# ucmmesa/Lidar-Visual-Odometry

Measured on NVIDIA B200. Metric: scan-to-map scans/sec (HDL-64 synthetic), higher is better.
Workload: dtype f32+f64

## Files before the change

lidar-visual-odometry_b200/csrc/lvo_api.cu:

```cuda
#include "lvo_internal.h"
#include "lvo_prims.cuh"
#include "lvo_extract.cuh"
#include "lvo_voxel.cuh"
#include "lvo_knn.cuh"
#include "lvo_solver.cuh"
#include "lvo_odometry.cuh"
#include "lvo_mapping.cuh"
#include "lvo_depth.cuh"
#include "lvo_outputs.cuh"

#include <algorithm>
#include <cmath>
#include <cstring>
#include <new>
#include <type_traits>
#include <nvtx3/nvToolsExt.h>

#define LVO_PROBE_GATE_EXTRACT 1
#define LVO_PROBE_GATE_ODO 2
#define LVO_PROBE_GATE_MAP 4

struct lvo_ctx {
  lvo_config cfg;
  int lanes, P, cap_sharp, cap_lsharp, cap_flat;
  cudaStream_t st = nullptr;
  cudaStream_t own_st = nullptr;
  std::string err;
  std::vector<void*> allocs, pinned;
  LaneState* d_ls = nullptr;
  LaneState* h_ls = nullptr;
  ExtractArgs ex;
  OdoArgs odo;
  MapArgs map;
  SolveArgs solve;
  GridSet gknn;
  GridProblem* d_knn_prob = nullptr;
  int* d_knn_n = nullptr;
  unsigned char* d_raw = nullptr;
  const lvo_cloud_view* pending_next = nullptr;
  unsigned char* d_raw2 = nullptr;
  cudaStream_t copy_st = nullptr;
  cudaEvent_t copy_ev = nullptr, compute_ev = nullptr;
  std::vector<lvo_cloud_view> prefetched;
  std::vector<const unsigned char*> next_in_ptr;
  int opt_stage_timing = 1;
  int raw_cur = 0;
  size_t raw_lane_bytes = 0;
  const unsigned char** d_in_ptr = nullptr; const unsigned char** h_in_ptr = nullptr;
  int* d_in_n = nullptr; int* h_in_n = nullptr;
  float4* d_upload = nullptr;
  int* d_knn_ind = nullptr; float* d_knn_sq = nullptr;
  double* d_trace[2] = {nullptr, nullptr};
  long long launches = 0;
  std::vector<long long> lane_frame;
  std::vector<lvo_lane_config> lane_cfg;
  LaneConfig* d_lcfg = nullptr; LaneConfig* h_lcfg = nullptr;
  std::vector<char> lane_active;
  std::vector<char> lane_map_update;
  std::vector<char> prefetched_active;
  std::vector<int> lane_status;
  std::vector<char> probe_gate;
  bool odo_grids_stale = false;
  cudaEvent_t ev[8];
  LvoStageTimer stage_tm;
  lvo_timings tim;
  bool pending = false, pending_do_map = false, pending_graph = false;
  struct Span { const unsigned char* host; size_t bytes; size_t dev_off; };
  std::vector<Span> spans;
  std::vector<int> span_order;
  cudaGraphExec_t graph_exec[2][2] = {{nullptr, nullptr}, {nullptr, nullptr}};
  long long graph_launches[2][2] = {{0, 0}, {0, 0}};
  int graph_stride = -1, graph_off = -1;
  int opt_graphs = -1;
  struct DepthArena {
    size_t cap_pts = 0, cap_raw = 0, cap_kp = 0; int cap_slots = 0;
    std::vector<void*> dev, pin;
    unsigned char* raw = nullptr;
    unsigned* flag = nullptr;
    float4* dc = nullptr;
    unsigned char* d_in = nullptr;
    unsigned char* h_in = nullptr;
    unsigned* d_res = nullptr;
    unsigned* h_res = nullptr;
    unsigned* dc_off = nullptr; int* ndc = nullptr;
    int* cnt = nullptr;
    GridSet grid;
  } depth;
  struct MapOutArena {
    std::vector<void*> dev, pin;
    MapOutDesc* d_desc = nullptr; MapOutDesc* h_desc = nullptr;
    unsigned* off = nullptr;
    unsigned* d_tot = nullptr; unsigned* h_tot = nullptr;
    size_t cap_pts = 0;
    float4* d_pts = nullptr;
  } mapout;
  std::vector<size_t> reg_n;
  bool reg_valid = true;
};

void lvo_set_error(lvo_ctx* ctx, const std::string& msg) { if (ctx) ctx->err = msg; }

namespace {

template <class T>
int dalloc(lvo_ctx* c, T** p, size_t n, bool zero = true) {
  void* q = nullptr;
  size_t bytes = std::max<size_t>(n, 1) * sizeof(T);
  cudaError_t e = cudaMalloc(&q, bytes);
  if (e != cudaSuccess) { lvo_set_error(c, std::string("cudaMalloc: ") + cudaGetErrorString(e)); return LVO_E_CUDA; }
  if (zero) { e = cudaMemsetAsync(q, 0, bytes, c->st); if (e != cudaSuccess) { cudaFree(q); lvo_set_error(c, std::string("cudaMemsetAsync: ") + cudaGetErrorString(e)); return LVO_E_CUDA; } }
  c->allocs.push_back(q);
  *p = (T*)q;
  return LVO_OK;
}
template <class T>
int halloc(lvo_ctx* c, T** p, size_t n) {
  void* q = nullptr;
  cudaError_t e = cudaMallocHost(&q, std::max<size_t>(n, 1) * sizeof(T));
  if (e != cudaSuccess) { lvo_set_error(c, std::string("cudaMallocHost: ") + cudaGetErrorString(e)); return LVO_E_CUDA; }
  memset(q, 0, std::max<size_t>(n, 1) * sizeof(T));
  c->pinned.push_back(q);
  *p = (T*)q;
  return LVO_OK;
}
#define LVO_TRY(x) do { int _r = (x); if (_r != LVO_OK) return _r; } while (0)

int alloc_scan(lvo_ctx* c, LvoScanScratch* s, size_t n_cap) {
  s->cap_tiles = lvo_div_up((long long)n_cap, LVO_SCAN_TILE) + 2;
  return dalloc(c, &s->partial, (size_t)s->cap_tiles);
}
int alloc_grid(lvo_ctx* c, GridSet* g, int nprob, int cells_cap, size_t pts_total, int pts_per_problem, size_t table_cells = 0) {
  g->nprob = nprob; g->cells_cap_per_problem = cells_cap; g->pts_cap_per_problem = pts_per_problem;
  if (table_cells == 0) table_cells = (size_t)nprob * cells_cap;
  g->table_cap_total = (long long)table_cells;
  LVO_TRY(dalloc(c, &g->prob, (size_t)nprob));
  LVO_TRY(dalloc(c, &g->table, table_cells + 1));
  LVO_TRY(dalloc(c, &g->d_table_len, 1));
  LVO_TRY(dalloc(c, &g->rank, pts_total));
  LVO_TRY(dalloc(c, &g->pt_off, (size_t)nprob + 1));
  LVO_TRY(dalloc(c, &g->sorted_pts, pts_total));
  LVO_TRY(dalloc(c, &g->sorted_id, pts_total));
  LVO_TRY(alloc_scan(c, &g->scan, table_cells + 1));
  return LVO_OK;
}

__global__ void k_unpack(const unsigned char* raw, int n, int stride, int off_xyz, int off_i, float4* out) {
  for (int i = blockIdx.x * blockDim.x + threadIdx.x; i < n; i += gridDim.x * blockDim.x) {
    const float* p = reinterpret_cast<const float*>(raw + (size_t)i * stride + off_xyz);
    const float w = *reinterpret_cast<const float*>(raw + (size_t)i * stride + off_i);
    out[i] = make_float4(p[0], p[1], p[2], w);
  }
}
struct SetCounts { int what; int v[4]; double pose[7]; };
__global__ void k_set_lane(LaneState* ls, int lane, SetCounts sc) {
  LaneState& s = ls[lane];
  if (sc.what == 0) { s.n_sharp = sc.v[0]; s.n_less_sharp = sc.v[1]; s.n_flat = sc.v[2]; s.n_less_flat = sc.v[3]; }
  else if (sc.what == 1) { s.n_less_sharp = sc.v[0]; s.n_less_flat = sc.v[1]; s.n_kept = sc.v[2]; for (int k = 0; k < 4; ++k) s.q_wodom[k] = sc.pose[k]; for (int k = 0; k < 3; ++k) s.t_wodom[k] = sc.pose[4 + k]; }
  else if (sc.what == 2) { for (int k = 0; k < 4; ++k) s.q_wmap_wodom[k] = sc.pose[k]; for (int k = 0; k < 3; ++k) s.t_wmap_wodom[k] = sc.pose[4 + k]; }
  else if (sc.what == 3) { for (int k = 0; k < 4; ++k) s.para_q[k] = sc.pose[k]; for (int k = 0; k < 3; ++k) s.para_t[k] = sc.pose[4 + k]; }
  else if (sc.what == 4) { for (int k = 0; k < 4; ++k) s.q_w[k] = sc.pose[k]; for (int k = 0; k < 3; ++k) s.t_w[k] = sc.pose[4 + k]; }
  else if (sc.what == 5) { s.n_map[0] = sc.v[0]; s.n_map[1] = sc.v[1]; }
}
__global__ void k_init_lanes(LaneState* ls, int first, int n) {
  const int l = first + blockIdx.x * blockDim.x + threadIdx.x;
  if (l >= first + n) return;
  LaneState& s = ls[l];
  s.para_q[3] = 1.0; s.q_w[3] = 1.0; s.map_x[3] = 1.0; s.q_wmap_wodom[3] = 1.0; s.q_wodom[3] = 1.0;
  s.cen[0] = 10; s.cen[1] = 10; s.cen[2] = 5;
}
__global__ void k_setup_grid_problems(GridProblem* prob, int nprob, const float4* base0, size_t stride0, const float4* base1, size_t stride1,
                                      LaneState* ls, int which, float cell) {
  const int p = blockIdx.x * blockDim.x + threadIdx.x;
  if (p >= nprob) return;
  const int per = which == 0 ? LVO_ODO_GRIDS : 2;
  const int lane = p / per, t = p & 1;
  prob[p].pts = (t ? base1 + (size_t)lane * stride1 : base0 + (size_t)lane * stride0);
  if (which == 0) prob[p].d_n = t ? &ls[lane].n_surf_last : &ls[lane].n_corner_last;
  else prob[p].d_n = &ls[lane].from_off[t][LVO_MAX_VALID];
  const int k = p % per;
  prob[p].want_cell = which == 0 ? (k >= 4 ? 2.0f : (k == 1 ? 0.5f : 1.0f)) : cell;
  prob[p].want_cell_z = which == 0 ? 2.0f : 0.f;
  prob[p].mode = (which == 0 && (k == 2 || k == 3)) ? 1 : 0;
  prob[p].cells_cap = which == 0 ? (k < 2 ? (1 << 22) : (k < 4 ? LVO_AZ_BUCKETS * LVO_AZ_RINGS : (1 << 19))) : 0;
  prob[p].clamp_xy = 0.f;
  prob[p].bbox_from = (which == 0 && k >= 4) ? p - k + (k & 1) : -1;
}
__global__ void k_setup_one_problem(GridProblem* prob, const float4* pts, const int* d_n, float cell) {
  prob[0].pts = pts; prob[0].d_n = d_n; prob[0].want_cell = cell; prob[0].want_cell_z = 0.f; prob[0].mode = 0; prob[0].cells_cap = 0; prob[0].clamp_xy = 0.f; prob[0].bbox_from = -1;
}
__global__ void k_vx_single_setup(VoxelEngine e, int n, float leaf) {
  if (blockIdx.x == 0 && threadIdx.x == 0) { *e.d_n = n; *e.d_nsegs = 1; e.seg_leaf[0] = leaf; }
  for (int i = blockIdx.x * blockDim.x + threadIdx.x; i < n; i += gridDim.x * blockDim.x) { e.in_seg[i] = 0; e.in_aux[i] = 0; }
}

struct PoseArg { double q[4], t[3]; int use; };
__global__ void k_transform_cloud(const LaneState* ls, PoseArg pa, const float4* in, int n, int distortion, int to_end, float4* out) {
  const double* q = pa.use ? pa.q : ls[0].para_q;
  const double* t = pa.use ? pa.t : ls[0].para_t;
  for (int i = blockIdx.x * blockDim.x + threadIdx.x; i < n; i += gridDim.x * blockDim.x)
    out[i] = to_end ? transform_to_end(q, t, in[i]) : transform_to_start(q, t, in[i], distortion);
}
int check_view(lvo_ctx* c, const lvo_cloud_view& v, size_t cap, bool xyz_only = false) {
  if (v.n == 0) return LVO_OK;
  const bool bad_i = !xyz_only && ((v.off_intensity & 3) || v.off_intensity + 4 > v.stride);
  if (!v.data || v.stride < (xyz_only ? 12u : 16u) || v.stride > 64 || (v.stride & 3) || (v.off_xyz & 3) || v.off_xyz + 12 > v.stride || bad_i) {
    lvo_set_error(c, "bad cloud view"); return LVO_E_BADARG;
  }
  if (v.n > cap) { lvo_set_error(c, "input cloud exceeds context capacity"); return LVO_E_CAPACITY; }
  return LVO_OK;
}
int upload_cloud(lvo_ctx* c, const lvo_cloud_view& v, float4* dst) {
  if (v.n == 0) return LVO_OK;
  LVO_CUDA_OK(c, cudaMemcpyAsync(c->d_upload, v.data, v.n * v.stride, cudaMemcpyHostToDevice, c->st));
  k_unpack<<<std::max(1, std::min(lvo_div_up((long long)v.n, 256), 592)), 256, 0, c->st>>>((const unsigned char*)c->d_upload, (int)v.n, (int)v.stride,
                                                                                             (int)v.off_xyz, (int)v.off_intensity, dst);
  c->launches++;
  return LVO_OK;
}
int download_cloud(lvo_ctx* c, const float4* src, size_t n, lvo_cloud_out* out) {
  if (!out) return LVO_OK;
  out->n = n;
  if (n > out->cap || (n && !out->data)) { lvo_set_error(c, "output cloud buffer too small"); return LVO_E_CAPACITY; }
  if (n) LVO_CUDA_OK(c, cudaMemcpyAsync(out->data, src, n * sizeof(float4), cudaMemcpyDeviceToHost, c->st));
  return LVO_OK;
}
int sync_state(lvo_ctx* c) {
  LVO_CUDA_OK(c, cudaMemcpyAsync(c->h_ls, c->d_ls, sizeof(LaneState) * c->lanes, cudaMemcpyDeviceToHost, c->st));
  LVO_CUDA_OK(c, cudaStreamSynchronize(c->st));
  LVO_CUDA_OK(c, cudaGetLastError());
  return LVO_OK;
}
void rebuild_stale_grids(lvo_ctx* c) {
  if (!c->odo_grids_stale) return;
  lvo_grid_build(c->st, c->odo.grid, &c->launches);
  c->odo_grids_stale = false;
}
void pose_out(lvo_pose* p, const double* q, const double* t) {
  if (!p) return;
  for (int k = 0; k < 4; ++k) p->q[k] = q[k];
  for (int k = 0; k < 3; ++k) p->t[k] = t[k];
}
int* lane_flags(lvo_ctx* c) { return c->h_in_n + c->lanes; }
struct FeatureCaps { int sharp, lsharp, flat; };
FeatureCaps feature_caps(int n_scans) { return FeatureCaps{n_scans * LVO_SECTORS * 2, n_scans * LVO_SECTORS * 20, n_scans * LVO_SECTORS * 4}; }
int upload_lane_config(lvo_ctx* c, int lane) {
  const lvo_lane_config& lc = c->lane_cfg[lane];
  c->h_lcfg[lane] = LaneConfig{lc.n_scans, (float)lc.minimum_range, {(float)lc.line_res, (float)lc.plane_res}};
  LVO_CUDA_OK(c, cudaMemcpyAsync(c->d_lcfg + lane, c->h_lcfg + lane, sizeof(LaneConfig), cudaMemcpyHostToDevice, c->st));
  return LVO_OK;
}
void stage_ran_on_all_lanes(lvo_ctx* c, int gate) { for (char& g : c->probe_gate) g &= ~gate; }
int set_inputs(lvo_ctx* c) {
  LVO_CUDA_OK(c, cudaMemcpyAsync(c->d_in_ptr, c->h_in_ptr, sizeof(void*) * c->lanes, cudaMemcpyHostToDevice, c->st));
  LVO_CUDA_OK(c, cudaMemcpyAsync(c->d_in_n, c->h_in_n, sizeof(int) * 2 * c->lanes, cudaMemcpyHostToDevice, c->st));
  return LVO_OK;
}
int flags_all_lanes(lvo_ctx* c, bool upload) {
  for (int l = 0; l < c->lanes; ++l) lane_flags(c)[l] = LVO_LANE_ACTIVE | LVO_LANE_MAPS | (c->lane_map_update[l] ? 0 : LVO_LANE_MAP_FIXED);
  if (upload) LVO_CUDA_OK(c, cudaMemcpyAsync(c->d_in_n + c->lanes, lane_flags(c), sizeof(int) * c->lanes, cudaMemcpyHostToDevice, c->st));
  return LVO_OK;
}
void enqueue_extract(lvo_ctx* c, int stride, int off_xyz, int max_n, LvoStageTimer* tm) {
  ExtractArgs a = c->ex;
  a.in_stride = stride; a.in_off_xyz = off_xyz;
  nvtxRangePushA("scan registration");
  lvo_launch_extract(c->st, a, c->lanes, max_n, &c->launches, tm);
  nvtxRangePop();
}
void enqueue_odometry(lvo_ctx* c, LvoStageTimer* tm) {
  nvtxRangePushA("laserOdometry");
  lvo_launch_odometry(c->st, c->odo, c->solve, c->cfg.outer_iters, c->lanes, &c->launches, tm);
  nvtxRangePop();
}
void enqueue_mapping(lvo_ctx* c, int from_odo, bool want_registered, LvoStageTimer* tm) {
  MapArgs a = c->map;
  a.from_odo = from_odo;
  nvtxRangePushA("laserMapping");
  lvo_launch_mapping(c->st, a, c->solve, c->cfg.outer_iters, c->lanes, want_registered, &c->launches, tm);
  nvtxRangePop();
  c->map.gen ^= 1;
}
LvoStageTimer* stage_timer_begin(lvo_ctx* c, bool on) {
  c->stage_tm.reset();
  c->stage_tm.on = on;
  return on ? &c->stage_tm : nullptr;
}
void collect_stage_timing(lvo_ctx* c, bool mapped) {
  float ms[LVO_ST_COUNT]; int cnt[LVO_ST_COUNT];
  c->stage_tm.collect(ms, cnt);
  lvo_timings& t = c->tim;
  t.reg_prepare_ms = ms[LVO_ST_REG_PREPARE]; t.reg_sort_ms = ms[LVO_ST_REG_SORT]; t.reg_separate_ms = ms[LVO_ST_REG_SEPARATE];
  t.odo_association_ms = ms[LVO_ST_ODO_ASSOC]; t.odo_solver_ms = ms[LVO_ST_ODO_SOLVER]; t.odo_rest_ms = ms[LVO_ST_ODO_REST];
  t.map_prepare_ms = ms[LVO_ST_MAP_PREPARE]; t.map_build_tree_ms = ms[LVO_ST_MAP_TREE];
  t.map_association_ms = ms[LVO_ST_MAP_KNN] + ms[LVO_ST_MAP_FIT]; t.map_solver_ms = ms[LVO_ST_MAP_SOLVER];
  t.map_optimization_ms = ms[LVO_ST_MAP_KNN] + ms[LVO_ST_MAP_FIT] + ms[LVO_ST_MAP_SOLVER];
  t.map_add_points_ms = ms[LVO_ST_MAP_ADD]; t.map_filter_ms = ms[LVO_ST_MAP_FILTER]; t.map_pub_ms = ms[LVO_ST_MAP_PUB];
  t.knn_ms = ms[LVO_ST_MAP_KNN]; t.knn_launches = cnt[LVO_ST_MAP_KNN]; t.knn_bytes = 0;
  if (!mapped || !c->stage_tm.on) return;
  for (int l = 0; l < c->lanes; ++l) {
    const LaneState& s = c->h_ls[l];
    if (s.map_too_small || !(lane_flags(c)[l] & LVO_LANE_MAPS)) continue;
    const double M = (double)s.from_off[0][LVO_MAX_VALID] + (double)s.from_off[1][LVO_MAX_VALID];
    const double Q = (double)s.n_stack[0] + (double)s.n_stack[1];
    t.knn_bytes += s.stats.map_outer_executed * (16.0 * M + 56.0 * Q);
  }
}
int stage_sweeps(lvo_ctx* c, const lvo_cloud_view* sweeps, unsigned char* buf, cudaStream_t st) {
  const int L = c->lanes;
  c->span_order.clear();
  for (int l = 0; l < L; ++l) {
    if (c->lane_active[l]) c->span_order.push_back(l);
    else { c->h_in_n[l] = 0; c->h_in_ptr[l] = buf; }
  }
  std::sort(c->span_order.begin(), c->span_order.end(), [&](int a, int b) { return (uintptr_t)sweeps[a].data < (uintptr_t)sweeps[b].data; });
  c->spans.clear();
  const size_t cap = c->raw_lane_bytes * (size_t)L, max_gap = 64u << 10;
  size_t dev_off = 0;
  for (size_t k = 0; k < c->span_order.size(); ++k) {
    const int l = c->span_order[k];
    const lvo_cloud_view& v = sweeps[l];
    c->h_in_n[l] = (int)v.n;
    if (v.n == 0) { c->h_in_ptr[l] = buf; continue; }
    const unsigned char* h = (const unsigned char*)v.data;
    const size_t bytes = v.n * v.stride;
    bool merged = false;
    if (!c->spans.empty()) {
      lvo_ctx::Span& sp = c->spans.back();
      const unsigned char* end = sp.host + sp.bytes;
      if (h >= end && (size_t)(h - end) <= max_gap && sp.dev_off + (size_t)(h - sp.host) + bytes <= cap) {
        sp.bytes = (size_t)(h - sp.host) + bytes;
        c->h_in_ptr[l] = buf + sp.dev_off + (size_t)(h - sp.host);
        dev_off = sp.dev_off + ((sp.bytes + 255) & ~(size_t)255);
        merged = true;
      }
    }
    if (!merged) {
      if (dev_off + bytes > cap) { lvo_set_error(c, "sweeps exceed the staging buffer"); return LVO_E_CAPACITY; }
      c->spans.push_back(lvo_ctx::Span{h, bytes, dev_off});
      c->h_in_ptr[l] = buf + dev_off;
      dev_off += (bytes + 255) & ~(size_t)255;
    }
  }
  for (const lvo_ctx::Span& sp : c->spans) LVO_CUDA_OK(c, cudaMemcpyAsync(buf + sp.dev_off, sp.host, sp.bytes, cudaMemcpyHostToDevice, st));
  return LVO_OK;
}


struct LvoDeviceGuard {
  int prev = -1; bool switched = false;
  explicit LvoDeviceGuard(const lvo_ctx* c);
  ~LvoDeviceGuard() { if (switched) cudaSetDevice(prev); }
};
}

LvoDeviceGuard::LvoDeviceGuard(const lvo_ctx* c) {
  if (!c) return;
  if (cudaGetDevice(&prev) == cudaSuccess && prev != c->cfg.device) switched = cudaSetDevice(c->cfg.device) == cudaSuccess;
}

static void destroy_graphs(lvo_ctx* c) {
  for (int a = 0; a < 2; ++a) for (int b = 0; b < 2; ++b) if (c->graph_exec[a][b]) { cudaGraphExecDestroy(c->graph_exec[a][b]); c->graph_exec[a][b] = nullptr; }
}

extern "C" {

void lvo_default_config(lvo_config* cfg) {
  if (!cfg) return;
  memset(cfg, 0, sizeof(*cfg));
  cfg->n_scans = 64; cfg->minimum_range = 5.0; cfg->line_res = 0.4; cfg->plane_res = 0.8;
  cfg->skip_frame = 1; cfg->outer_iters = 10; cfg->lm_max_iters = 4; cfg->huber = 0.1; cfg->device = 0; cfg->lanes = 1;
  cfg->max_points = 0; cfg->max_map_corner = 0; cfg->max_map_surf = 0;
  cfg->distortion = 0;
  cfg->debug_probes = 0;
}

int lvo_create(const lvo_config* cfg, lvo_ctx** out) {
  if (!cfg || !out) return LVO_E_BADARG;
  *out = nullptr;
  if (cfg->n_scans != 16 && cfg->n_scans != 32 && cfg->n_scans != 64) return LVO_E_BADARG;
  if (cfg->distortion < 0 || cfg->distortion > 2) return LVO_E_BADARG;
  if (cfg->lanes < 1 || cfg->outer_iters < 1 || cfg->outer_iters > LVO_MAX_OUTER || cfg->lm_max_iters < 0 || cfg->lm_max_iters > LVO_MAX_LM) return LVO_E_BADARG;
  lvo_ctx* c = new (std::nothrow) lvo_ctx();
  if (!c) return LVO_E_CUDA;
  *out = c;
  c->cfg = *cfg;
  if (c->cfg.skip_frame < 1) c->cfg.skip_frame = 1;
  c->lanes = cfg->lanes;
  int ndev = 0;
  if (cudaGetDeviceCount(&ndev) != cudaSuccess || ndev == 0) { lvo_set_error(c, "no CUDA device: liblvo has no CPU fallback"); return LVO_E_CUDA; }
  struct RestoreDevice { int prev = -1; ~RestoreDevice() { if (prev >= 0) cudaSetDevice(prev); } } restore;
  cudaGetDevice(&restore.prev);
  LVO_CUDA_OK(c, cudaSetDevice(cfg->device));
  cudaDeviceProp prop;
  LVO_CUDA_OK(c, cudaGetDeviceProperties(&prop, cfg->device));
  if (prop.major != 10) { lvo_set_error(c, "liblvo is built for sm_100a (B200) only; found sm_" + std::to_string(prop.major) + std::to_string(prop.minor)); return LVO_E_CUDA; }
  LVO_CUDA_OK(c, cudaStreamCreateWithFlags(&c->own_st, cudaStreamNonBlocking));
  c->st = c->own_st;
  for (int i = 0; i < 8; ++i) LVO_CUDA_OK(c, cudaEventCreate(&c->ev[i]));
  memset(&c->tim, 0, sizeof(c->tim));

  const int L = c->lanes;
  const int P = c->P = cfg->max_points > 0 ? cfg->max_points : 262144;
  const FeatureCaps fc = feature_caps(cfg->n_scans);
  c->cap_sharp = fc.sharp; c->cap_lsharp = fc.lsharp; c->cap_flat = fc.flat;
  const int mapc[2] = {cfg->max_map_corner > 0 ? cfg->max_map_corner : (1 << 20), cfg->max_map_surf > 0 ? cfg->max_map_surf : (1 << 21)};
  c->lane_status.assign(L, 0);
  c->lane_frame.assign(L, 0);
  c->lane_active.assign(L, 1);
  c->lane_map_update.assign(L, 1);
  c->probe_gate.assign(L, 0);
  c->reg_n.assign(L, 0);
  c->lane_cfg.assign(L, lvo_lane_config{c->cfg.n_scans, c->cfg.minimum_range, c->cfg.line_res, c->cfg.plane_res, c->cfg.skip_frame});

  LVO_TRY(dalloc(c, &c->d_ls, (size_t)L));
  LVO_TRY(halloc(c, &c->h_ls, (size_t)L));
  k_init_lanes<<<lvo_div_up(L, 64), 64, 0, c->st>>>(c->d_ls, 0, L);
  LVO_TRY(dalloc(c, &c->d_lcfg, (size_t)L, false)); LVO_TRY(halloc(c, &c->h_lcfg, (size_t)L));
  for (int l = 0; l < L; ++l) LVO_TRY(upload_lane_config(c, l));
  c->raw_lane_bytes = (size_t)P * 32;
  LVO_TRY(dalloc(c, &c->d_raw, c->raw_lane_bytes * L, false));
  LVO_TRY(dalloc(c, &c->d_in_ptr, (size_t)L)); LVO_TRY(halloc(c, &c->h_in_ptr, (size_t)L));
  LVO_TRY(dalloc(c, &c->d_in_n, (size_t)2 * L)); LVO_TRY(halloc(c, &c->h_in_n, (size_t)2 * L));
  LVO_TRY(flags_all_lanes(c, true));
  LVO_TRY(dalloc(c, (unsigned char**)&c->d_upload, (size_t)std::max(P, std::max(mapc[0], mapc[1])) * 64, false));

  ExtractArgs& ex = c->ex;
  memset(&ex, 0, sizeof(ex));
  ex.in_ptr = c->d_in_ptr; ex.in_n = c->d_in_n; ex.lane_flags = c->d_in_n + L; ex.lcfg = c->d_lcfg; ex.max_scans = cfg->n_scans;
  ex.P = P; ex.nblk_cap = lvo_div_up(P, LVO_EX_THREADS); ex.ls = c->d_ls;
  LVO_TRY(dalloc(c, &ex.ring, (size_t)L * P)); LVO_TRY(dalloc(c, &ex.ori, (size_t)L * P));
  LVO_TRY(dalloc(c, &ex.blkcnt, (size_t)L * ex.nblk_cap * LVO_MAX_RINGS));
  LVO_TRY(dalloc(c, &ex.full, (size_t)L * P)); LVO_TRY(dalloc(c, &ex.curv, (size_t)L * P)); LVO_TRY(dalloc(c, &ex.gapbig, (size_t)L * P));
  LVO_TRY(dalloc(c, &ex.sort_ind, (size_t)L * P)); LVO_TRY(dalloc(c, &ex.picked, (size_t)L * P)); LVO_TRY(dalloc(c, &ex.label, (size_t)L * P));
  const size_t nsec = (size_t)L * LVO_MAX_RINGS * LVO_SECTORS;
  LVO_TRY(dalloc(c, &ex.slot_sharp, nsec * 2)); LVO_TRY(dalloc(c, &ex.slot_lsharp, nsec * 20)); LVO_TRY(dalloc(c, &ex.slot_flat, nsec * 4));
  LVO_TRY(dalloc(c, &ex.slot_cnt, nsec * 3));
  LVO_TRY(dalloc(c, &ex.lf_ring, (size_t)L * P)); LVO_TRY(dalloc(c, &ex.lf_cnt, (size_t)L * LVO_MAX_RINGS));
  LVO_TRY(dalloc(c, &ex.sort_scratch, (size_t)L * 2 * P, false));
  LVO_TRY(dalloc(c, &ex.ring_done, (size_t)L * LVO_MAX_RINGS));
  LVO_TRY(dalloc(c, &ex.sharp, (size_t)L * c->cap_sharp)); LVO_TRY(dalloc(c, &ex.less_sharp, (size_t)L * c->cap_lsharp));
  LVO_TRY(dalloc(c, &ex.flat, (size_t)L * c->cap_flat)); LVO_TRY(dalloc(c, &ex.less_flat, (size_t)L * P));
  ex.cap_sharp = c->cap_sharp; ex.cap_lsharp = c->cap_lsharp; ex.cap_flat = c->cap_flat;

  SolveArgs& so = c->solve;
  memset(&so, 0, sizeof(so));
  so.ls = c->d_ls; so.max_iters = cfg->lm_max_iters; so.huber = cfg->huber;
  so.n_outer = cfg->outer_iters; so.fixpoint_skip = 1;
  const size_t trace_n = (size_t)L * LVO_MAX_OUTER * (LVO_MAX_LM + 1) * LVO_TRACE_W;
  LVO_TRY(dalloc(c, &c->d_trace[0], trace_n)); LVO_TRY(dalloc(c, &c->d_trace[1], trace_n));

  OdoArgs& od = c->odo;
  memset(&od, 0, sizeof(od));
  od.ls = c->d_ls; od.lanes = L; od.distortion = cfg->distortion; od.full = ex.full; od.lane_flags = ex.lane_flags;
  od.sharp = ex.sharp; od.less_sharp = ex.less_sharp; od.flat = ex.flat; od.less_flat = ex.less_flat;
  od.cap_sharp = c->cap_sharp; od.cap_lsharp = c->cap_lsharp; od.cap_flat = c->cap_flat; od.P = P;
  const int slots = cfg->debug_probes ? LVO_MAX_OUTER : 2;
  od.slots = slots;
  LVO_TRY(dalloc(c, &od.corner_last, (size_t)L * c->cap_lsharp)); LVO_TRY(dalloc(c, &od.surf_last, (size_t)L * P));
  od.factor_cap = std::max(c->cap_sharp + c->cap_flat, c->cap_lsharp + P);
  LVO_TRY(dalloc(c, &od.factors, (size_t)L * od.factor_cap));
  LVO_TRY(dalloc(c, &od.slow_list, (size_t)L * (c->cap_sharp + c->cap_flat))); LVO_TRY(dalloc(c, &od.slow_cnt, (size_t)L));
  od.reuse = 1;
  LVO_TRY(dalloc(c, &od.ref, (size_t)L * (c->cap_sharp + c->cap_flat))); LVO_TRY(dalloc(c, &od.guard, (size_t)L * (c->cap_sharp + c->cap_flat)));
  LVO_TRY(dalloc(c, &od.sel, (size_t)L * (c->cap_sharp + c->cap_flat)));
  LVO_TRY(dalloc(c, &od.corner_corr, (size_t)L * slots * c->cap_sharp * 2));
  LVO_TRY(dalloc(c, &od.plane_corr, (size_t)L * slots * c->cap_flat * 3));
  const size_t odo_cells = 2 * ((size_t)(1 << 22) + (size_t)LVO_AZ_BUCKETS * LVO_AZ_RINGS + (1 << 19));
  LVO_TRY(alloc_grid(c, &od.grid, LVO_ODO_GRIDS * L, 1 << 22, (size_t)3 * L * (c->cap_lsharp + P), P, odo_cells * L));
  k_setup_grid_problems<<<lvo_div_up(LVO_ODO_GRIDS * L, 64), 64, 0, c->st>>>(od.grid.prob, LVO_ODO_GRIDS * L, od.corner_last, (size_t)c->cap_lsharp, od.surf_last, (size_t)P, c->d_ls, 0, 1.0f);

  MapArgs& mp = c->map;
  memset(&mp, 0, sizeof(mp));
  mp.ls = c->d_ls; mp.lanes = L; mp.lane_flags = ex.lane_flags; mp.lcfg = c->d_lcfg;
  mp.in_pts[0] = ex.less_sharp; mp.in_pts[1] = ex.less_flat; mp.in_cap[0] = c->cap_lsharp; mp.in_cap[1] = P;
  mp.full = ex.full; mp.P = P; mp.gen = 0; mp.slots = slots;
  mp.knn_reuse = 1;
  lvo_extract_kernel_attributes();
  for (int t = 0; t < 2; ++t) {
    mp.map_cap[t] = mapc[t];
    for (int g = 0; g < 2; ++g) {
      LVO_TRY(dalloc(c, &mp.map_pts[g][t], (size_t)L * mapc[t], false));
      LVO_TRY(dalloc(c, &mp.cube_start[g][t], (size_t)L * (LVO_NCUBES + 1)));
    }
    LVO_TRY(dalloc(c, &mp.from_map[t], (size_t)L * mapc[t], false));
    LVO_TRY(dalloc(c, &mp.stack[t], (size_t)L * mp.in_cap[t]));
    LVO_TRY(dalloc(c, &mp.knn_ind[t], (size_t)L * slots * mp.in_cap[t] * 5));
    LVO_TRY(dalloc(c, &mp.fac_valid[t], (size_t)L * slots * mp.in_cap[t]));
    LVO_TRY(dalloc(c, &mp.knn_ref[t], (size_t)L * mp.in_cap[t], false));
    LVO_TRY(dalloc(c, &mp.knn_sel[t], (size_t)L * mp.in_cap[t] * 5, false));
    LVO_TRY(dalloc(c, &mp.knn_flag[t], (size_t)L * mp.in_cap[t], false));
  }
  LVO_TRY(alloc_grid(c, &mp.grid, 2 * L, 1 << 21, (size_t)L * ((size_t)mapc[0] + mapc[1]), std::max(mapc[0], mapc[1])));
  k_setup_grid_problems<<<lvo_div_up(2 * L, 64), 64, 0, c->st>>>(mp.grid.prob, 2 * L, mp.from_map[0], (size_t)mapc[0], mp.from_map[1], (size_t)mapc[1], c->d_ls, 1, 1.0f);
  LVO_TRY(dalloc(c, &mp.item_off, (size_t)2 * L + 1));
  LVO_TRY(dalloc(c, &mp.fit_list, (size_t)L * (mp.in_cap[0] + mp.in_cap[1]), false));
  LVO_TRY(dalloc(c, &mp.fit_cnt, (size_t)L * LVO_MAX_OUTER));
  mp.factors = od.factors; mp.factor_cap = od.factor_cap;
  LVO_TRY(dalloc(c, &mp.app_cnt, (size_t)2 * L * LVO_NCUBES)); LVO_TRY(dalloc(c, &mp.app_first, (size_t)2 * L * LVO_NCUBES));
  LVO_TRY(dalloc(c, &mp.new_cnt, (size_t)2 * L * (LVO_NCUBES + 1)));
  LVO_TRY(dalloc(c, &mp.registered, (size_t)L * P, false));
  VoxelEngine& vx = mp.vx;
  vx.cap_items = (int)std::min<size_t>((size_t)L * ((size_t)mapc[0] + mapc[1] + c->cap_lsharp + P), (size_t)INT_MAX - 4096);
  vx.cap_segs = 2 * L * LVO_MSEGS;
  const size_t NI = (size_t)vx.cap_items, NS = (size_t)vx.cap_segs;
  LVO_TRY(dalloc(c, &vx.in_pts, NI, false)); LVO_TRY(dalloc(c, &vx.in_seg, NI)); LVO_TRY(dalloc(c, &vx.in_aux, NI));
  LVO_TRY(dalloc(c, &vx.d_n, 1)); LVO_TRY(dalloc(c, &vx.seg_leaf, NS)); LVO_TRY(dalloc(c, &vx.d_nsegs, 1));
  LVO_TRY(dalloc(c, &vx.seg_mn, 3 * NS)); LVO_TRY(dalloc(c, &vx.seg_mx, 3 * NS)); LVO_TRY(dalloc(c, &vx.seg_minb, 3 * NS));
  LVO_TRY(dalloc(c, &vx.seg_div, 2 * NS)); LVO_TRY(dalloc(c, &vx.seg_mode, NS)); LVO_TRY(dalloc(c, &vx.d_vbits, 1)); LVO_TRY(dalloc(c, &vx.d_bits, 1));
  for (int k = 0; k < 2; ++k) { LVO_TRY(dalloc(c, &vx.sort.keys[k], NI, false)); LVO_TRY(dalloc(c, &vx.sort.vals[k], NI, false)); }
  const size_t tiles = (size_t)lvo_div_up((long long)NI, LVO_SORT_TILE) + 1;
  LVO_TRY(dalloc(c, &vx.sort.ghist, (size_t)LVO_SORT_GHIST_WORDS)); LVO_TRY(dalloc(c, &vx.sort.d_epoch, 1));
  LVO_TRY(dalloc(c, &vx.sort.status, 256 * tiles));
  vx.sort.cap = vx.cap_items;
  LVO_TRY(dalloc(c, &vx.outpos, NI)); LVO_TRY(dalloc(c, &vx.out_pts, NI, false)); LVO_TRY(dalloc(c, &vx.out_aux, NI));
  LVO_TRY(dalloc(c, &vx.seg_out_cnt, NS)); LVO_TRY(dalloc(c, &vx.seg_out_start, NS + 1)); LVO_TRY(dalloc(c, &vx.d_n_out, 1));
  LVO_TRY(alloc_scan(c, &vx.scan, std::max(NI, NS + 1)));

  c->gknn = mp.grid; c->gknn.nprob = 1;
  LVO_TRY(dalloc(c, &c->d_knn_prob, 1)); LVO_TRY(dalloc(c, &c->d_knn_n, 4));
  c->gknn.prob = c->d_knn_prob;
  LVO_TRY(dalloc(c, &c->d_knn_ind, (size_t)P * 5)); LVO_TRY(dalloc(c, &c->d_knn_sq, (size_t)P * 5));

  LVO_CUDA_OK(c, cudaStreamSynchronize(c->st));
  LVO_CUDA_OK(c, cudaGetLastError());
  return LVO_OK;
}

int lvo_destroy(lvo_ctx* c) {
  if (!c) return LVO_E_BADARG;
  LvoDeviceGuard _dev(c);
  if (c->st) cudaStreamSynchronize(c->st);
  for (void* p : c->allocs) cudaFree(p);
  for (void* p : c->pinned) cudaFreeHost(p);
  for (void* p : c->depth.dev) cudaFree(p);
  for (void* p : c->depth.pin) cudaFreeHost(p);
  for (void* p : c->mapout.dev) cudaFree(p);
  for (void* p : c->mapout.pin) cudaFreeHost(p);
  if (c->mapout.d_pts) cudaFree(c->mapout.d_pts);
  destroy_graphs(c);
  if (c->copy_st) { cudaStreamSynchronize(c->copy_st); cudaStreamDestroy(c->copy_st); cudaEventDestroy(c->copy_ev); cudaEventDestroy(c->compute_ev); }
  if (c->own_st) { for (int i = 0; i < 8; ++i) cudaEventDestroy(c->ev[i]); c->stage_tm.destroy(); cudaStreamDestroy(c->own_st); }
  delete c;
  return LVO_OK;
}

const char* lvo_last_error(const lvo_ctx* c) { return c ? c->err.c_str() : "null context"; }

int lvo_get_stats(const lvo_ctx* c, int lane, lvo_stats* out, size_t bytes) {
  if (!c || !out || lane < 0 || lane >= c->lanes) return LVO_E_BADARG;
  memcpy(out, &c->h_ls[lane].stats, std::min(bytes, sizeof(lvo_stats)));
  return LVO_OK;
}
int lvo_lane_status(const lvo_ctx* c, int lane) { return (c && lane >= 0 && lane < c->lanes) ? c->lane_status[lane] : LVO_E_BADARG; }
size_t lvo_state_bytes(void) { return sizeof(LaneState); }
int lvo_set_option(lvo_ctx* c, int option, int value) {
  LvoDeviceGuard _dev(c);
  if (!c) return LVO_E_BADARG;
  if (option == LVO_OPT_GRAPHS) { c->opt_graphs = value; return LVO_OK; }
  if (option == LVO_OPT_STAGE_TIMING) { c->opt_stage_timing = value ? 1 : 0; return LVO_OK; }
  if (option == LVO_OPT_ODO_REUSE) {
    if (c->st) cudaStreamSynchronize(c->st);
    destroy_graphs(c);
    c->odo.reuse = value ? 1 : 0;
    return LVO_OK;
  }
  if (option == LVO_OPT_KNN_REUSE) {
    if (c->st) cudaStreamSynchronize(c->st);
    destroy_graphs(c);
    c->map.knn_reuse = value ? 1 : 0;
    return LVO_OK;
  }
  if (option == LVO_OPT_FIXPOINT_SKIP) {
    if (c->st) cudaStreamSynchronize(c->st);
    destroy_graphs(c);
    c->solve.fixpoint_skip = value ? 1 : 0;
    return LVO_OK;
  }
  return LVO_E_BADARG;
}
int lvo_set_stream(lvo_ctx* c, void* cuda_stream) {
  LvoDeviceGuard _dev(c);
  if (!c) return LVO_E_BADARG;
  cudaStreamSynchronize(c->st);
  destroy_graphs(c);
  c->st = cuda_stream ? (cudaStream_t)cuda_stream : c->own_st;
  return LVO_OK;
}
int lvo_get_timings(const lvo_ctx* c, lvo_timings* out) { if (!c || !out) return LVO_E_BADARG; *out = c->tim; out->kernel_launches = (int)c->launches; return LVO_OK; }

int lvo_extract_features(lvo_ctx* c, lvo_cloud_view sweep, lvo_cloud_out* full, lvo_cloud_out* sharp, lvo_cloud_out* less_sharp, lvo_cloud_out* flat,
                         lvo_cloud_out* less_flat) {
  LvoDeviceGuard _dev(c);
  if (!c) return LVO_E_BADARG;
  LVO_TRY(check_view(c, sweep, (size_t)c->P, true));
  if (c->pending) { lvo_set_error(c, "lvo_wait has not been called for the last *_async step"); return LVO_E_STATE; }
  c->launches = 0;
  cudaEventRecord(c->ev[0], c->st);
  if (sweep.n) LVO_CUDA_OK(c, cudaMemcpyAsync(c->d_raw, sweep.data, sweep.n * sweep.stride, cudaMemcpyHostToDevice, c->st));
  for (int l = 0; l < c->lanes; ++l) { c->h_in_ptr[l] = c->d_raw + c->raw_lane_bytes * l; c->h_in_n[l] = l == 0 ? (int)sweep.n : 0; }
  LVO_TRY(flags_all_lanes(c, false));
  LVO_TRY(set_inputs(c));
  LvoStageTimer* tm = stage_timer_begin(c, true);
  enqueue_extract(c, sweep.n ? (int)sweep.stride : 16, sweep.n ? (int)sweep.off_xyz : 0, (int)sweep.n, tm);
  stage_ran_on_all_lanes(c, LVO_PROBE_GATE_EXTRACT);
  c->stage_tm.stop(c->st);
  cudaEventRecord(c->ev[1], c->st);
  LVO_TRY(sync_state(c));
  cudaEventElapsedTime(&c->tim.extract_ms, c->ev[0], c->ev[1]);
  collect_stage_timing(c, false);
  const LaneState& s = c->h_ls[0];
  int r = LVO_OK, q;
  if ((q = download_cloud(c, c->ex.full, (size_t)s.n_kept, full)) != LVO_OK) r = q;
  if ((q = download_cloud(c, c->ex.sharp, (size_t)s.n_sharp, sharp)) != LVO_OK) r = q;
  if ((q = download_cloud(c, c->ex.less_sharp, (size_t)s.n_less_sharp, less_sharp)) != LVO_OK) r = q;
  if ((q = download_cloud(c, c->ex.flat, (size_t)s.n_flat, flat)) != LVO_OK) r = q;
  if ((q = download_cloud(c, c->ex.less_flat, (size_t)s.n_less_flat, less_flat)) != LVO_OK) r = q;
  LVO_CUDA_OK(c, cudaStreamSynchronize(c->st));
  c->lane_status[0] = r;
  return r;
}

int lvo_scan_to_scan(lvo_ctx* c, lvo_cloud_view sharp, lvo_cloud_view less_sharp, lvo_cloud_view flat, lvo_cloud_view less_flat, lvo_pose* T_last_curr,
                     lvo_pose* T_w_curr) {
  LvoDeviceGuard _dev(c);
  if (!c) return LVO_E_BADARG;
  if (c->pending) { lvo_set_error(c, "lvo_wait has not been called for the last *_async step"); return LVO_E_STATE; }
  const FeatureCaps fc = feature_caps(c->lane_cfg[0].n_scans);
  LVO_TRY(check_view(c, sharp, (size_t)fc.sharp)); LVO_TRY(check_view(c, less_sharp, (size_t)fc.lsharp));
  LVO_TRY(check_view(c, flat, (size_t)fc.flat)); LVO_TRY(check_view(c, less_flat, (size_t)c->P));
  c->launches = 0;
  rebuild_stale_grids(c);
  cudaEventRecord(c->ev[2], c->st);
  LVO_TRY(upload_cloud(c, sharp, c->ex.sharp)); LVO_TRY(upload_cloud(c, less_sharp, c->ex.less_sharp));
  LVO_TRY(upload_cloud(c, flat, c->ex.flat)); LVO_TRY(upload_cloud(c, less_flat, c->ex.less_flat));
  SetCounts sc; memset(&sc, 0, sizeof(sc));
  sc.what = 0; sc.v[0] = (int)sharp.n; sc.v[1] = (int)less_sharp.n; sc.v[2] = (int)flat.n; sc.v[3] = (int)less_flat.n;
  k_set_lane<<<1, 1, 0, c->st>>>(c->d_ls, 0, sc);
  LVO_TRY(flags_all_lanes(c, true));
  c->solve.trace = c->d_trace[0];
  LvoStageTimer* tm = stage_timer_begin(c, true);
  enqueue_odometry(c, tm);
  stage_ran_on_all_lanes(c, LVO_PROBE_GATE_ODO);
  c->stage_tm.stop(c->st);
  cudaEventRecord(c->ev[3], c->st);
  LVO_TRY(sync_state(c));
  cudaEventElapsedTime(&c->tim.odometry_ms, c->ev[2], c->ev[3]);
  collect_stage_timing(c, false);
  const LaneState& s = c->h_ls[0];
  pose_out(T_last_curr, s.para_q, s.para_t);
  pose_out(T_w_curr, s.q_w, s.t_w);
  c->lane_status[0] = s.odo_status;
  return s.odo_status;
}

int lvo_scan_to_map(lvo_ctx* c, lvo_cloud_view corner_last, lvo_cloud_view surf_last, lvo_cloud_view full_or_null, const lvo_pose* T_wodom_curr,
                    lvo_pose* T_wmap_curr, lvo_cloud_out* registered_or_null) {
  LvoDeviceGuard _dev(c);
  if (!c || !T_wodom_curr) return LVO_E_BADARG;
  if (c->pending) { lvo_set_error(c, "lvo_wait has not been called for the last *_async step"); return LVO_E_STATE; }
  LVO_TRY(check_view(c, corner_last, (size_t)feature_caps(c->lane_cfg[0].n_scans).lsharp)); LVO_TRY(check_view(c, surf_last, (size_t)c->P));
  LVO_TRY(check_view(c, full_or_null, (size_t)c->P));
  c->launches = 0;
  c->reg_valid = false;
  cudaEventRecord(c->ev[4], c->st);
  LVO_TRY(upload_cloud(c, corner_last, c->ex.less_sharp)); LVO_TRY(upload_cloud(c, surf_last, c->ex.less_flat));
  const bool want_reg = registered_or_null && full_or_null.n > 0;
  if (full_or_null.n) LVO_TRY(upload_cloud(c, full_or_null, c->ex.full));
  SetCounts sc; memset(&sc, 0, sizeof(sc));
  sc.what = 1; sc.v[0] = (int)corner_last.n; sc.v[1] = (int)surf_last.n; sc.v[2] = (int)full_or_null.n;
  for (int k = 0; k < 4; ++k) sc.pose[k] = T_wodom_curr->q[k];
  for (int k = 0; k < 3; ++k) sc.pose[4 + k] = T_wodom_curr->t[k];
  k_set_lane<<<1, 1, 0, c->st>>>(c->d_ls, 0, sc);
  LVO_TRY(flags_all_lanes(c, true));
  c->solve.trace = c->d_trace[1];
  LvoStageTimer* tm = stage_timer_begin(c, true);
  enqueue_mapping(c, 0, want_reg, tm);
  stage_ran_on_all_lanes(c, LVO_PROBE_GATE_MAP);
  c->stage_tm.stop(c->st);
  cudaEventRecord(c->ev[5], c->st);
  LVO_TRY(sync_state(c));
  cudaEventElapsedTime(&c->tim.mapping_ms, c->ev[4], c->ev[5]);
  collect_stage_timing(c, true);
  const LaneState& s = c->h_ls[0];
  pose_out(T_wmap_curr, s.map_x, s.map_x + 4);
  int r = s.map_status;
  if (registered_or_null) {
    int q = download_cloud(c, c->map.registered, want_reg ? full_or_null.n : 0, registered_or_null);
    if (q != LVO_OK) r = q;
    LVO_CUDA_OK(c, cudaStreamSynchronize(c->st));
  }
  if (r == LVO_E_CAPACITY) lvo_set_error(c, "map capacity exceeded (max_map_corner / max_map_surf)");
  c->lane_status[0] = r;
  return r;
}

static int enqueue_prefetch(lvo_ctx* c) {
  const lvo_cloud_view* next = c->pending_next;
  c->pending_next = nullptr;
  if (!next) return LVO_OK;
  unsigned char* bufs[2] = {c->d_raw, c->d_raw2};
  std::vector<const unsigned char*> keep_ptr(c->h_in_ptr, c->h_in_ptr + c->lanes);
  std::vector<int> keep_n(c->h_in_n, c->h_in_n + c->lanes);
  const int r = stage_sweeps(c, next, bufs[c->raw_cur ^ 1], c->copy_st);
  c->next_in_ptr.assign(c->h_in_ptr, c->h_in_ptr + c->lanes);
  std::copy(keep_ptr.begin(), keep_ptr.end(), c->h_in_ptr);
  std::copy(keep_n.begin(), keep_n.end(), c->h_in_n);
  if (r != LVO_OK) return r;
  LVO_CUDA_OK(c, cudaEventRecord(c->copy_ev, c->copy_st));
  c->prefetched.assign(c->lanes, lvo_cloud_view{});
  for (int l = 0; l < c->lanes; ++l) if (c->lane_active[l]) c->prefetched[l] = next[l];
  c->prefetched_active = c->lane_active;
  return LVO_OK;
}

static int step_enqueue(lvo_ctx* c, int stride, int off_xyz, int max_n) {
  if (c->pending) { lvo_set_error(c, "lvo_wait has not been called for the last *_async step"); return LVO_E_STATE; }
  c->launches = 0;
  LVO_TRY(enqueue_prefetch(c));
  rebuild_stale_grids(c);
  const long long pre_launches = c->launches;
  bool do_map = false;
  for (int l = 0; l < c->lanes; ++l) {
    const bool maps = c->lane_active[l] && (c->lane_frame[l] % c->lane_cfg[l].skip_frame) == 0;
    lane_flags(c)[l] = (c->lane_active[l] ? LVO_LANE_ACTIVE : 0) | (maps ? LVO_LANE_MAPS : 0) | (maps && !c->lane_map_update[l] ? LVO_LANE_MAP_FIXED : 0);
    do_map = do_map || maps;
  }
  LVO_TRY(set_inputs(c));
  const bool want_graph = c->opt_graphs == 1 || (c->opt_graphs < 0 && c->lanes <= 8);
  const bool use_graph = want_graph && c->st != nullptr;
  nvtxRangePushA("lvo_step");
  if (use_graph) {
    if (c->graph_stride != stride || c->graph_off != off_xyz) { destroy_graphs(c); c->graph_stride = stride; c->graph_off = off_xyz; }
    const int gen = c->map.gen;
    stage_timer_begin(c, false);
    cudaEventRecord(c->ev[0], c->st);
    if (!c->graph_exec[do_map][gen]) {
      cudaGraph_t graph = nullptr;
      LVO_CUDA_OK(c, cudaStreamBeginCapture(c->st, cudaStreamCaptureModeThreadLocal));
      enqueue_extract(c, stride, off_xyz, c->P, nullptr);
      c->solve.trace = c->d_trace[0];
      enqueue_odometry(c, nullptr);
      if (do_map) { c->solve.trace = c->d_trace[1]; enqueue_mapping(c, 1, true, nullptr); }
      cudaError_t e = cudaStreamEndCapture(c->st, &graph);
      if (do_map) c->map.gen = gen;
      if (e != cudaSuccess || !graph) { nvtxRangePop(); lvo_set_error(c, std::string("graph capture: ") + cudaGetErrorString(e)); return LVO_E_CUDA; }
      e = cudaGraphInstantiate(&c->graph_exec[do_map][gen], graph, 0);
      cudaGraphDestroy(graph);
      if (e != cudaSuccess) { nvtxRangePop(); lvo_set_error(c, std::string("cudaGraphInstantiate: ") + cudaGetErrorString(e)); return LVO_E_CUDA; }
      c->graph_launches[do_map][gen] = c->launches - pre_launches;
    }
    cudaError_t ge = cudaGraphLaunch(c->graph_exec[do_map][gen], c->st);
    if (ge != cudaSuccess) { nvtxRangePop(); lvo_set_error(c, std::string("cudaGraphLaunch: ") + cudaGetErrorString(ge)); return LVO_E_CUDA; }
    c->launches = pre_launches + c->graph_launches[do_map][gen];
    if (do_map) c->map.gen = gen ^ 1;
    cudaEventRecord(c->ev[3], c->st);
  } else {
    LvoStageTimer* tm = stage_timer_begin(c, c->opt_stage_timing != 0);
    cudaEventRecord(c->ev[0], c->st);
    enqueue_extract(c, stride, off_xyz, max_n, tm);
    cudaEventRecord(c->ev[1], c->st);
    c->solve.trace = c->d_trace[0];
    enqueue_odometry(c, tm);
    cudaEventRecord(c->ev[2], c->st);
    if (do_map) { c->solve.trace = c->d_trace[1]; enqueue_mapping(c, 1, true, tm); }
    c->stage_tm.stop(c->st);
    cudaEventRecord(c->ev[3], c->st);
  }
  nvtxRangePop();
  for (int l = 0; l < c->lanes; ++l) {
    const int f = lane_flags(c)[l];
    if (f & LVO_LANE_ACTIVE) { c->lane_frame[l]++; c->probe_gate[l] &= ~(LVO_PROBE_GATE_EXTRACT | LVO_PROBE_GATE_ODO); }
    if (f & LVO_LANE_MAPS) c->probe_gate[l] = 0;
  }
  LVO_CUDA_OK(c, cudaMemcpyAsync(c->h_ls, c->d_ls, sizeof(LaneState) * c->lanes, cudaMemcpyDeviceToHost, c->st));
  c->pending = true; c->pending_do_map = do_map; c->pending_graph = use_graph;
  return LVO_OK;
}

static int step_finish(lvo_ctx* c, lvo_pose* T_wodom, lvo_pose* T_wmap) {
  if (!c->pending) { lvo_set_error(c, "lvo_wait without a step in flight"); return LVO_E_STATE; }
  c->pending = false;
  const bool do_map = c->pending_do_map;
  LVO_CUDA_OK(c, cudaStreamSynchronize(c->st));
  LVO_CUDA_OK(c, cudaGetLastError());
  for (int l = 0; l < c->lanes; ++l) c->reg_n[l] = (lane_flags(c)[l] & LVO_LANE_MAPS) ? (size_t)c->h_ls[l].n_kept : 0;
  c->reg_valid = true;
  if (c->pending_graph) {
    c->tim.extract_ms = c->tim.odometry_ms = 0.f;
    cudaEventElapsedTime(&c->tim.mapping_ms, c->ev[0], c->ev[3]);
  } else {
    cudaEventElapsedTime(&c->tim.extract_ms, c->ev[0], c->ev[1]);
    cudaEventElapsedTime(&c->tim.odometry_ms, c->ev[1], c->ev[2]);
    cudaEventElapsedTime(&c->tim.mapping_ms, c->ev[2], c->ev[3]);
  }
  collect_stage_timing(c, do_map);
  int worst = LVO_OK;
  for (int l = 0; l < c->lanes; ++l) {
    const int flags = lane_flags(c)[l];
    if (!(flags & LVO_LANE_ACTIVE)) continue;
    const bool mapped = (flags & LVO_LANE_MAPS) != 0;
    const LaneState& s = c->h_ls[l];
    if (T_wodom) pose_out(&T_wodom[l], s.q_w, s.t_w);
    if (T_wmap) {
      if (mapped) pose_out(&T_wmap[l], s.map_x, s.map_x + 4);
      else {
        const double* a = s.q_wmap_wodom; const double* b = s.q_w;
        double q[4] = {a[3] * b[0] + a[0] * b[3] + a[1] * b[2] - a[2] * b[1], a[3] * b[1] + a[1] * b[3] + a[2] * b[0] - a[0] * b[2],
                       a[3] * b[2] + a[2] * b[3] + a[0] * b[1] - a[1] * b[0], a[3] * b[3] - a[0] * b[0] - a[1] * b[1] - a[2] * b[2]};
        const double v[3] = {s.t_w[0], s.t_w[1], s.t_w[2]};
        const double uv[3] = {2 * (a[1] * v[2] - a[2] * v[1]), 2 * (a[2] * v[0] - a[0] * v[2]), 2 * (a[0] * v[1] - a[1] * v[0])};
        const double t[3] = {v[0] + a[3] * uv[0] + (a[1] * uv[2] - a[2] * uv[1]) + s.t_wmap_wodom[0], v[1] + a[3] * uv[1] + (a[2] * uv[0] - a[0] * uv[2]) + s.t_wmap_wodom[1],
                             v[2] + a[3] * uv[2] + (a[0] * uv[1] - a[1] * uv[0]) + s.t_wmap_wodom[2]};
        pose_out(&T_wmap[l], q, t);
      }
    }
// ... 374 lines not shown
  if (!c || lane < 0 || lane >= c->lanes || which < 0 || which > 1 || !pts) return LVO_E_BADARG;
  LVO_CUDA_OK(c, cudaStreamSynchronize(c->st));
  std::vector<unsigned> start(LVO_NCUBES + 1);
  LVO_CUDA_OK(c, cudaMemcpyAsync(start.data(), c->map.cube_start[c->map.gen][which] + (size_t)lane * (LVO_NCUBES + 1), sizeof(unsigned) * (LVO_NCUBES + 1), cudaMemcpyDeviceToHost, c->st));
  LVO_CUDA_OK(c, cudaStreamSynchronize(c->st));
  const size_t n = start[LVO_NCUBES];
  pts->n = n;
  if (n > pts->cap) return LVO_E_CAPACITY;
  if (n) {
    LVO_CUDA_OK(c, cudaMemcpyAsync(pts->data, c->map.map_pts[c->map.gen][which] + (size_t)lane * c->map.map_cap[which], n * sizeof(lvo_point), cudaMemcpyDeviceToHost, c->st));
    LVO_CUDA_OK(c, cudaStreamSynchronize(c->st));
  }
  if (cube_out) for (int k = 0; k < LVO_NCUBES; ++k) for (unsigned i = start[k]; i < start[k + 1]; ++i) cube_out[i] = k;
  return LVO_OK;
}

static int mapout_fail(lvo_ctx* c, cudaError_t e) { lvo_set_error(c, std::string("map outputs: ") + cudaGetErrorString(e)); return LVO_E_CUDA; }
static int mapout_reserve_slots(lvo_ctx* c) {
  lvo_ctx::MapOutArena& m = c->mapout;
  auto fail = [&](cudaError_t e) { return mapout_fail(c, e); };
  if (!m.d_desc) {
    const size_t L = (size_t)c->lanes;
    void* q[5] = {nullptr, nullptr, nullptr, nullptr, nullptr};
    const size_t dev_bytes[3] = {L * sizeof(MapOutDesc), L * LVO_MAPOUT_STRIDE * sizeof(unsigned), L * sizeof(unsigned)};
    for (int k = 0; k < 3; ++k) { cudaError_t e = cudaMalloc(&q[k], dev_bytes[k]); if (e != cudaSuccess) return fail(e); m.dev.push_back(q[k]); }
    for (int k = 3; k < 5; ++k) {
      cudaError_t e = cudaMallocHost(&q[k], k == 3 ? L * sizeof(MapOutDesc) : L * sizeof(unsigned));
      if (e != cudaSuccess) return fail(e);
      m.pin.push_back(q[k]);
    }
    m.d_desc = (MapOutDesc*)q[0]; m.off = (unsigned*)q[1]; m.d_tot = (unsigned*)q[2]; m.h_desc = (MapOutDesc*)q[3]; m.h_tot = (unsigned*)q[4];
  }
  return LVO_OK;
}
static int mapout_reserve_points(lvo_ctx* c, size_t pts) {
  lvo_ctx::MapOutArena& m = c->mapout;
  LVO_TRY(mapout_reserve_slots(c));
  if (m.d_pts && pts <= m.cap_pts) return LVO_OK;
  pts = std::max<size_t>({pts, m.cap_pts + m.cap_pts / 2, 1024});
  if (m.d_pts) { cudaFree(m.d_pts); m.d_pts = nullptr; }
  m.cap_pts = 0;
  cudaError_t e = cudaMalloc(&m.d_pts, pts * sizeof(float4));
  if (e != cudaSuccess) { m.d_pts = nullptr; return mapout_fail(c, e); }
  m.cap_pts = pts;
  return LVO_OK;
}

static MapOutArgs mapout_args(const lvo_ctx* c, int which, int first_lane) {
  MapOutArgs a;
  memset(&a, 0, sizeof(a));
  a.ls = c->d_ls;
  for (int t = 0; t < 2; ++t) { a.cube_start[t] = c->map.cube_start[c->map.gen][t]; a.map_pts[t] = c->map.map_pts[c->map.gen][t]; a.map_cap[t] = c->map.map_cap[t]; }
  a.first_lane = first_lane;
  a.surround = which == LVO_MAP_SURROUND;
  return a;
}

static int mapout_count(lvo_ctx* c, const MapOutArgs& a, int S, size_t* n) {
  lvo_ctx::MapOutArena& m = c->mapout;
  k_mapout_offsets<<<S, 256, 0, c->st>>>(a, m.off, m.d_tot);
  c->launches++;
  LVO_CUDA_OK(c, cudaMemcpyAsync(m.h_tot, m.d_tot, sizeof(unsigned) * S, cudaMemcpyDeviceToHost, c->st));
  LVO_CUDA_OK(c, cudaStreamSynchronize(c->st));
  LVO_CUDA_OK(c, cudaGetLastError());
  for (int s = 0; s < S; ++s) n[s] = m.h_tot[s];
  return LVO_OK;
}

static int mapout_copy(lvo_ctx* c, int which, const MapOutArgs& a, int S) {
  lvo_ctx::MapOutArena& m = c->mapout;
  LVO_CUDA_OK(c, cudaMemcpyAsync(m.d_desc, m.h_desc, sizeof(MapOutDesc) * S, cudaMemcpyHostToDevice, c->st));
  if (which == LVO_MAP_REGISTERED) k_mapout_registered<<<dim3(64, S), 256, 0, c->st>>>(c->map.registered, c->P, m.d_desc);
  else k_mapout_copy<<<dim3(which == LVO_MAP_SURROUND ? LVO_MAX_VALID : 296, S), 256, 0, c->st>>>(a, m.d_desc, m.off);
  c->launches++;
  return LVO_OK;
}

static int mapout_host(lvo_ctx* c, int which, const MapOutArgs& a, int S, const size_t* n, lvo_point* const* dst) {
  lvo_ctx::MapOutArena& m = c->mapout;
  size_t total = 0; bool any = false;
  for (int s = 0; s < S; ++s) if (dst[s]) { total += n[s]; any = true; }
  if (!any) return LVO_OK;
  LVO_TRY(mapout_reserve_points(c, total));
  size_t o = 0;
  for (int s = 0; s < S; ++s) {
    m.h_desc[s] = MapOutDesc{dst[s] ? m.d_pts + o : nullptr, (unsigned)n[s], 0u};
    if (dst[s]) o += n[s];
  }
  LVO_TRY(mapout_copy(c, which, a, S));
  o = 0;
  for (int s = 0; s < S; ++s) {
    if (!dst[s]) continue;
    if (n[s]) LVO_CUDA_OK(c, cudaMemcpyAsync(dst[s], m.d_pts + o, n[s] * sizeof(float4), cudaMemcpyDeviceToHost, c->st));
    o += n[s];
  }
  LVO_CUDA_OK(c, cudaStreamSynchronize(c->st));
  LVO_CUDA_OK(c, cudaGetLastError());
  return LVO_OK;
}

static int mapout_batch_begin(lvo_ctx* c, int which, size_t* n, MapOutArgs* a) {
  if (which < LVO_MAP_SURROUND || which > LVO_MAP_REGISTERED) { lvo_set_error(c, "bad `which`: LVO_MAP_SURROUND, LVO_MAP_WHOLE or LVO_MAP_REGISTERED"); return LVO_E_BADARG; }
  if (c->pending) { lvo_set_error(c, "lvo_wait has not been called for the last *_async step"); return LVO_E_STATE; }
  if (which == LVO_MAP_REGISTERED && !c->reg_valid) {
    lvo_set_error(c, "the registered clouds were overwritten by lvo_scan_to_map, lvo_knn or lvo_depth_associate; the next lvo_step_batch* call makes them available again");
    return LVO_E_STATE;
  }
  c->launches = 0;
  *a = mapout_args(c, which, 0);
  if (which == LVO_MAP_REGISTERED) { for (int l = 0; l < c->lanes; ++l) n[l] = c->reg_n[l]; return LVO_OK; }
  LVO_TRY(mapout_reserve_slots(c));
  return mapout_count(c, *a, c->lanes, n);
}

static int map_cloud_one(lvo_ctx* c, int lane, int which, lvo_cloud_out* pts) {
  LVO_TRY(mapout_reserve_slots(c));
  const MapOutArgs a = mapout_args(c, which, lane);
  size_t n = 0;
  LVO_TRY(mapout_count(c, a, 1, &n));
  pts->n = n;
  if (n > pts->cap || (n && !pts->data)) { lvo_set_error(c, "output cloud buffer too small"); return LVO_E_CAPACITY; }
  lvo_point* dst = pts->data;
  return mapout_host(c, which, a, 1, &n, &dst);
}
int lvo_map_cloud(lvo_ctx* c, int lane, int which, lvo_cloud_out* pts) {
  LvoDeviceGuard _dev(c);
  if (!c || lane < 0 || lane >= c->lanes || which < 0 || which > 1 || !pts) return LVO_E_BADARG;
  const long long launches = c->launches;
  const int r = map_cloud_one(c, lane, which, pts);
  c->launches = launches;
  return r;
}

int lvo_map_cloud_batch(lvo_ctx* c, int which, lvo_cloud_out* outs) {
  LvoDeviceGuard _dev(c);
  if (!c) return LVO_E_BADARG;
  if (!outs) { lvo_set_error(c, "NULL array"); return LVO_E_BADARG; }
  const int L = c->lanes;
  std::vector<size_t> n(L);
  MapOutArgs a;
  LVO_TRY(mapout_batch_begin(c, which, n.data(), &a));
  std::vector<lvo_point*> dst(L);
  int short_lane = -1;
  for (int l = 0; l < L; ++l) {
    outs[l].n = n[l];
    dst[l] = outs[l].data;
    if (dst[l] && outs[l].cap < n[l] && short_lane < 0) short_lane = l;
  }
  if (short_lane >= 0) { lvo_set_error(c, "output buffer of lane " + std::to_string(short_lane) + " too small"); return LVO_E_CAPACITY; }
  return mapout_host(c, which, a, L, n.data(), dst.data());
}

int lvo_map_cloud_batch_dev(lvo_ctx* c, int which, lvo_point* const* d_out, const size_t* cap, size_t* n_out) {
  LvoDeviceGuard _dev(c);
  if (!c) return LVO_E_BADARG;
  if (!d_out || !cap || !n_out) { lvo_set_error(c, "NULL array"); return LVO_E_BADARG; }
  const int L = c->lanes;
  std::vector<size_t> n(L);
  MapOutArgs a;
  LVO_TRY(mapout_batch_begin(c, which, n.data(), &a));
  int short_lane = -1;
  bool any = false;
  for (int l = 0; l < L; ++l) {
    n_out[l] = n[l];
    any = any || d_out[l];
    if (d_out[l] && cap[l] < n[l] && short_lane < 0) short_lane = l;
  }
  if (short_lane >= 0) { lvo_set_error(c, "output buffer of lane " + std::to_string(short_lane) + " too small"); return LVO_E_CAPACITY; }
  if (!any) return LVO_OK;
  LVO_TRY(mapout_reserve_slots(c));
  for (int l = 0; l < L; ++l) c->mapout.h_desc[l] = MapOutDesc{(float4*)d_out[l], (unsigned)n[l], 0u};
  LVO_TRY(mapout_copy(c, which, a, L));
  LVO_CUDA_OK(c, cudaStreamSynchronize(c->st));
  LVO_CUDA_OK(c, cudaGetLastError());
  return LVO_OK;
}

int lvo_transform_cloud(lvo_ctx* c, lvo_cloud_view in, const lvo_pose* T, int to_end, lvo_cloud_out* out) {
  LvoDeviceGuard _dev(c);
  if (!c || !out) return LVO_E_BADARG;
  const size_t cap = (size_t)std::max(c->P, std::max(c->map.map_cap[0], c->map.map_cap[1]));
  LVO_TRY(check_view(c, in, cap));
  if (in.n * in.stride > cap * 32) { lvo_set_error(c, "input cloud exceeds the staging buffer"); return LVO_E_CAPACITY; }
  float4* d_in = (float4*)c->d_upload + 2 * cap;
  float4* d_out = d_in + cap;
  if (in.n) {
    LVO_CUDA_OK(c, cudaMemcpyAsync(c->d_upload, in.data, in.n * in.stride, cudaMemcpyHostToDevice, c->st));
    k_unpack<<<std::max(1, std::min(lvo_div_up((long long)in.n, 256), 592)), 256, 0, c->st>>>((const unsigned char*)c->d_upload, (int)in.n, (int)in.stride,
                                                                                                 (int)in.off_xyz, (int)in.off_intensity, d_in);
    PoseArg pa; memset(&pa, 0, sizeof(pa));
    if (T) { pa.use = 1; for (int k = 0; k < 4; ++k) pa.q[k] = T->q[k]; for (int k = 0; k < 3; ++k) pa.t[k] = T->t[k]; }
    k_transform_cloud<<<std::max(1, std::min(lvo_div_up((long long)in.n, 256), 592)), 256, 0, c->st>>>(c->d_ls, pa, d_in, (int)in.n, c->cfg.distortion, to_end, d_out);
  }
  const int r = download_cloud(c, d_out, in.n, out);
  LVO_CUDA_OK(c, cudaStreamSynchronize(c->st));
  LVO_CUDA_OK(c, cudaGetLastError());
  return r;
}

static int set_pose(lvo_ctx* c, int lane, int what, const lvo_pose* p) {
  if (!c || !p || lane < 0 || lane >= c->lanes) return LVO_E_BADARG;
  SetCounts sc; memset(&sc, 0, sizeof(sc));
  sc.what = what;
  for (int k = 0; k < 4; ++k) sc.pose[k] = p->q[k];
  for (int k = 0; k < 3; ++k) sc.pose[4 + k] = p->t[k];
  k_set_lane<<<1, 1, 0, c->st>>>(c->d_ls, lane, sc);
  LVO_CUDA_OK(c, cudaStreamSynchronize(c->st));
  return LVO_OK;
}
int lvo_set_map_correction(lvo_ctx* c, int lane, const lvo_pose* T) {
  LvoDeviceGuard _dev(c); return set_pose(c, lane, 2, T); }
int lvo_get_map_correction(lvo_ctx* c, int lane, lvo_pose* T) {
  LvoDeviceGuard _dev(c);
  if (!c || !T || lane < 0 || lane >= c->lanes) return LVO_E_BADARG;
  LVO_TRY(sync_state(c));
  pose_out(T, c->h_ls[lane].q_wmap_wodom, c->h_ls[lane].t_wmap_wodom);
  return LVO_OK;
}
int lvo_set_odometry_state(lvo_ctx* c, int lane, const lvo_pose* T_last_curr, const lvo_pose* T_w_curr) {
  LvoDeviceGuard _dev(c);
  int r = LVO_OK;
  if (T_last_curr) r = set_pose(c, lane, 3, T_last_curr);
  if (r == LVO_OK && T_w_curr) r = set_pose(c, lane, 4, T_w_curr);
  return r;
}

int lvo_probe_fetch(lvo_ctx* c, int lane, int what, void* out, size_t cap_bytes, size_t* n_bytes) {
  LvoDeviceGuard _dev(c);
  if (!c || lane < 0 || lane >= c->lanes) return LVO_E_BADARG;
  LVO_TRY(sync_state(c));
  const LaneState& s = c->h_ls[lane];
  const ExtractArgs& ex = c->ex;
  const int P = c->P, O = c->cfg.outer_iters;
  const void* src = nullptr; size_t bytes = 0;
  size_t row_bytes = 0, row_stride = 0; int rows = 1;
  bool per_outer = false;
  switch (what) {
    case LVO_P_FULL: src = ex.full + (size_t)lane * P; bytes = (size_t)s.n_kept * 16; break;
    case LVO_P_CURVATURE: src = ex.curv + (size_t)lane * P; bytes = (size_t)s.n_kept * 4; break;
    case LVO_P_SORT_IND: src = ex.sort_ind + (size_t)lane * P; bytes = (size_t)s.n_kept * 4; break;
    case LVO_P_LABEL: src = ex.label + (size_t)lane * P; bytes = (size_t)s.n_kept * 4; break;
    case LVO_P_PICKED: src = ex.picked + (size_t)lane * P; bytes = (size_t)s.n_kept * 4; break;
    case LVO_P_SCAN_START: src = (const char*)(c->d_ls + lane) + offsetof(LaneState, scan_start); bytes = (size_t)c->lane_cfg[lane].n_scans * 4; break;
    case LVO_P_SCAN_END: src = (const char*)(c->d_ls + lane) + offsetof(LaneState, scan_end); bytes = (size_t)c->lane_cfg[lane].n_scans * 4; break;
    case LVO_P_SHARP: src = ex.sharp + (size_t)lane * c->cap_sharp; bytes = (size_t)s.n_sharp * 16; break;
    case LVO_P_LESS_SHARP: src = ex.less_sharp + (size_t)lane * c->cap_lsharp; bytes = (size_t)s.n_less_sharp * 16; break;
    case LVO_P_FLAT: src = ex.flat + (size_t)lane * c->cap_flat; bytes = (size_t)s.n_flat * 16; break;
    case LVO_P_LESS_FLAT: src = ex.less_flat + (size_t)lane * P; bytes = (size_t)s.n_less_flat * 16; break;
    case LVO_P_ODO_CORNER_CORR: src = c->odo.corner_corr + (size_t)lane * c->odo.slots * c->cap_sharp * 2; rows = O; per_outer = true; row_bytes = (size_t)s.n_sharp * 8; row_stride = (size_t)c->cap_sharp * 8; break;
    case LVO_P_ODO_PLANE_CORR: src = c->odo.plane_corr + (size_t)lane * c->odo.slots * c->cap_flat * 3; rows = O; per_outer = true; row_bytes = (size_t)s.n_flat * 12; row_stride = (size_t)c->cap_flat * 12; break;
    case LVO_P_ODO_LM_TRACE: case LVO_P_MAP_LM_TRACE: {
      const double* base = c->d_trace[what == LVO_P_ODO_LM_TRACE ? 0 : 1] + (size_t)lane * LVO_MAX_OUTER * (LVO_MAX_LM + 1) * LVO_TRACE_W;
      src = base; rows = O; row_bytes = (size_t)(c->cfg.lm_max_iters + 1) * LVO_TRACE_W * 8; row_stride = (size_t)(LVO_MAX_LM + 1) * LVO_TRACE_W * 8; break;
    }
    case LVO_P_MAP_CORNER_STACK: src = c->map.stack[0] + (size_t)lane * c->map.in_cap[0]; bytes = (size_t)s.n_stack[0] * 16; break;
    case LVO_P_MAP_SURF_STACK: src = c->map.stack[1] + (size_t)lane * c->map.in_cap[1]; bytes = (size_t)s.n_stack[1] * 16; break;
    case LVO_P_MAP_CORNER_FROM_MAP: src = c->map.from_map[0] + (size_t)lane * c->map.map_cap[0]; bytes = (size_t)s.from_off[0][LVO_MAX_VALID] * 16; break;
    case LVO_P_MAP_SURF_FROM_MAP: src = c->map.from_map[1] + (size_t)lane * c->map.map_cap[1]; bytes = (size_t)s.from_off[1][LVO_MAX_VALID] * 16; break;
    case LVO_P_MAP_CORNER_KNN: case LVO_P_MAP_SURF_KNN: {
      const int t = what == LVO_P_MAP_CORNER_KNN ? 0 : 1;
      src = c->map.knn_ind[t] + (size_t)lane * c->map.slots * c->map.in_cap[t] * 5; rows = O; per_outer = true; row_bytes = (size_t)s.n_stack[t] * 20; row_stride = (size_t)c->map.in_cap[t] * 20; break;
    }
    case LVO_P_MAP_CORNER_VALID: case LVO_P_MAP_SURF_VALID: {
      const int t = what == LVO_P_MAP_CORNER_VALID ? 0 : 1;
      src = c->map.fac_valid[t] + (size_t)lane * c->map.slots * c->map.in_cap[t]; rows = O; per_outer = true; row_bytes = (size_t)s.n_stack[t] * 4; row_stride = (size_t)c->map.in_cap[t] * 4; break;
    }
    case LVO_P_REGISTERED: src = c->map.registered + (size_t)lane * P; bytes = (size_t)s.n_kept * 16; break;
    default: return LVO_E_BADARG;
  }
  if (per_outer && !c->cfg.debug_probes) { lvo_set_error(c, "per-outer-iteration probes need lvo_config::debug_probes = 1"); return LVO_E_STATE; }
  const int gate = what <= LVO_P_LESS_FLAT ? LVO_PROBE_GATE_EXTRACT : (what <= LVO_P_ODO_LM_TRACE ? LVO_PROBE_GATE_ODO : LVO_PROBE_GATE_MAP);
  if (c->probe_gate[lane] & gate) {
    lvo_set_error(c, "the lane was loaded from a snapshot and the stage that writes this probe has not run for it since");
    return LVO_E_STATE;
  }
  if (rows > 1 || row_bytes) bytes = row_bytes * rows;
  if (n_bytes) *n_bytes = bytes;
  if (!out) return LVO_OK;
  if (cap_bytes < bytes) return LVO_E_CAPACITY;
  if (bytes == 0) return LVO_OK;
  if (row_bytes) {
    LVO_CUDA_OK(c, cudaMemcpy2DAsync(out, row_bytes, src, row_stride, row_bytes, rows, cudaMemcpyDeviceToHost, c->st));
    LVO_CUDA_OK(c, cudaStreamSynchronize(c->st));
    const bool odo = what == LVO_P_ODO_CORNER_CORR || what == LVO_P_ODO_PLANE_CORR || what == LVO_P_ODO_LM_TRACE;
    const int ran = odo ? s.stats.odo_outer_executed : s.stats.map_outer_executed;
    if (ran >= 1 && ran < rows)
      for (int o = ran; o < rows; ++o) memcpy((char*)out + (size_t)o * row_bytes, (const char*)out + (size_t)(ran - 1) * row_bytes, row_bytes);
  } else {
    LVO_CUDA_OK(c, cudaMemcpyAsync(out, src, bytes, cudaMemcpyDeviceToHost, c->st));
    LVO_CUDA_OK(c, cudaStreamSynchronize(c->st));
  }
  return LVO_OK;
}

int lvo_voxel_downsample(lvo_ctx* c, lvo_cloud_view in, float leaf, lvo_cloud_out* out) {
  LvoDeviceGuard _dev(c);
  if (!c || !out || !(leaf > 0.f)) return LVO_E_BADARG;
  LVO_TRY(check_view(c, in, (size_t)c->map.vx.cap_items));
  if (in.n * in.stride > (size_t)std::max(c->P, std::max(c->map.map_cap[0], c->map.map_cap[1])) * 64) return LVO_E_CAPACITY;
  c->launches = 0;
  VoxelEngine& vx = c->map.vx;
  LVO_TRY(upload_cloud(c, in, vx.in_pts));
  k_vx_single_setup<<<std::max(1, std::min(lvo_div_up((long long)in.n, 256), 592)), 256, 0, c->st>>>(vx, (int)in.n, leaf);
  lvo_voxel_run(c->st, vx, (int)std::max<size_t>(in.n, 1), 1, 1, &c->launches);
  unsigned n_out = 0;
  LVO_CUDA_OK(c, cudaMemcpyAsync(&n_out, vx.d_n_out, 4, cudaMemcpyDeviceToHost, c->st));
  LVO_CUDA_OK(c, cudaStreamSynchronize(c->st));
  LVO_CUDA_OK(c, cudaGetLastError());
  if (in.n == 0) n_out = 0;
  int r = download_cloud(c, vx.out_pts, n_out, out);
  LVO_CUDA_OK(c, cudaStreamSynchronize(c->st));
  return r;
}

int lvo_voxel_downsample_dev(lvo_ctx* c, const lvo_point* d_in, size_t n, float leaf, lvo_point* d_out, size_t* n_out, float* ms) {
  LvoDeviceGuard _dev(c);
  if (!c || !d_in || !d_out || !n_out || !(leaf > 0.f)) return LVO_E_BADARG;
  if (n > (size_t)c->map.vx.cap_items) { lvo_set_error(c, "input cloud exceeds the voxel engine capacity"); return LVO_E_CAPACITY; }
  c->launches = 0;
  VoxelEngine& vx = c->map.vx;
  LVO_CUDA_OK(c, cudaMemcpyAsync(vx.in_pts, d_in, n * sizeof(lvo_point), cudaMemcpyDeviceToDevice, c->st));
  k_vx_single_setup<<<std::max(1, std::min(lvo_div_up((long long)n, 256), 592)), 256, 0, c->st>>>(vx, (int)n, leaf);
  cudaEventRecord(c->ev[6], c->st);
  lvo_voxel_run(c->st, vx, (int)std::max<size_t>(n, 1), 1, 1, &c->launches);
  cudaEventRecord(c->ev[7], c->st);
  unsigned cnt = 0;
  LVO_CUDA_OK(c, cudaMemcpyAsync(&cnt, vx.d_n_out, 4, cudaMemcpyDeviceToHost, c->st));
  LVO_CUDA_OK(c, cudaStreamSynchronize(c->st));
  LVO_CUDA_OK(c, cudaGetLastError());
  if (n == 0) cnt = 0;
  *n_out = cnt;
  if (cnt) LVO_CUDA_OK(c, cudaMemcpyAsync(d_out, vx.out_pts, (size_t)cnt * sizeof(lvo_point), cudaMemcpyDeviceToDevice, c->st));
  LVO_CUDA_OK(c, cudaStreamSynchronize(c->st));
  if (ms) cudaEventElapsedTime(ms, c->ev[6], c->ev[7]);
  return LVO_OK;
}

int lvo_knn(lvo_ctx* c, lvo_cloud_view cloud, lvo_cloud_view queries, int K, float max_sq, int* ind, float* sq) {
  LvoDeviceGuard _dev(c);
  if (!c || !ind || !sq || (K != 1 && K != 5)) return LVO_E_BADARG;
  LVO_TRY(check_view(c, cloud, (size_t)c->map.map_cap[1])); LVO_TRY(check_view(c, queries, (size_t)c->P));
  c->launches = 0;
  float4* d_cloud = c->map.from_map[1];
  float4* d_q = c->map.registered;
  c->reg_valid = false;
  LVO_TRY(upload_cloud(c, cloud, d_cloud)); LVO_TRY(upload_cloud(c, queries, d_q));
  const int n = (int)cloud.n;
  LVO_CUDA_OK(c, cudaMemcpyAsync(c->d_knn_n, &n, 4, cudaMemcpyHostToDevice, c->st));
  float cell = 0.0625f;
  while (cell * cell < max_sq && cell < 64.f) cell *= 2.f;
  if (K == 1 && cell > 2.f) cell = 2.f;
  k_setup_one_problem<<<1, 1, 0, c->st>>>(c->d_knn_prob, d_cloud, c->d_knn_n, cell);
  lvo_grid_build(c->st, c->gknn, &c->launches);
  const int nq = (int)queries.n;
  const int blocks = std::max(1, std::min(lvo_div_up((long long)nq, 8), 1184));
  if (K == 5) k_knn_queries<5><<<blocks, 256, 0, c->st>>>(c->gknn, d_q, nq, max_sq, c->d_knn_ind, c->d_knn_sq);
  else k_knn_queries<1><<<blocks, 256, 0, c->st>>>(c->gknn, d_q, nq, max_sq, c->d_knn_ind, c->d_knn_sq);
  c->launches += 2;
  if (nq) {
    LVO_CUDA_OK(c, cudaMemcpyAsync(ind, c->d_knn_ind, (size_t)nq * K * 4, cudaMemcpyDeviceToHost, c->st));
    LVO_CUDA_OK(c, cudaMemcpyAsync(sq, c->d_knn_sq, (size_t)nq * K * 4, cudaMemcpyDeviceToHost, c->st));
  }
  LVO_CUDA_OK(c, cudaStreamSynchronize(c->st));
  LVO_CUDA_OK(c, cudaGetLastError());
  return LVO_OK;
}

__global__ void k_setup_batch_problems(GridProblem* prob, int S, const float4* maps, const unsigned* m_off, const int* m_cnt, float cell) {
  const int p = blockIdx.x * blockDim.x + threadIdx.x;
  if (p >= S) return;
  prob[p].pts = maps + m_off[p]; prob[p].d_n = m_cnt + p; prob[p].want_cell = cell; prob[p].want_cell_z = 0.f; prob[p].mode = 0; prob[p].cells_cap = 0; prob[p].clamp_xy = 0.f; prob[p].bbox_from = -1;
}

int lvo_depth_associate(lvo_ctx* c, lvo_cloud_view sweep, const lvo_camera* cam, const float* keypoints_uv, size_t n_kp, float* depth_out, int* valid_out,
                        int* nn_out, lvo_cloud_out* depth_cloud_or_null) {
  LvoDeviceGuard _dev(c);
  if (!c || !cam || (n_kp && (!keypoints_uv || !depth_out || !valid_out))) return LVO_E_BADARG;
  LVO_TRY(check_view(c, sweep, (size_t)c->P));
  if (n_kp > (size_t)c->P) { lvo_set_error(c, "too many keypoints"); return LVO_E_CAPACITY; }
  c->launches = 0;
  float4* d_sweep = c->ex.lf_ring;
  float4* d_dc = c->map.registered;
  unsigned* d_flag = (unsigned*)c->ex.sort_ind;
  float* d_uv = (float*)c->ex.curv;
  if (2 * n_kp > (size_t)c->P) { lvo_set_error(c, "too many keypoints"); return LVO_E_CAPACITY; }
  if ((size_t)std::max(c->P, std::max(c->map.map_cap[0], c->map.map_cap[1])) * 64 < sizeof(DepthSlot)) { lvo_set_error(c, "context too small for lvo_depth_associate"); return LVO_E_CAPACITY; }
  c->reg_valid = false;
  LVO_TRY(upload_cloud(c, sweep, d_sweep));
  if (n_kp) LVO_CUDA_OK(c, cudaMemcpyAsync(d_uv, keypoints_uv, 2 * n_kp * sizeof(float), cudaMemcpyHostToDevice, c->st));
  DepthSlot slot;
  memset(&slot, 0, sizeof(slot));
  slot.pts = (const unsigned char*)d_sweep; slot.n = (int)sweep.n;
  slot.uv = d_uv; slot.nkp = (int)n_kp;
  slot.depth = c->d_knn_sq; slot.valid = c->d_knn_ind; slot.nn = c->d_knn_ind + c->P;
  for (int k = 0; k < 12; ++k) slot.extr[k] = cam->extrinsic[k];
  DepthSlot* d_slot = (DepthSlot*)c->d_upload;
  LVO_CUDA_OK(c, cudaMemcpyAsync(d_slot, &slot, sizeof(slot), cudaMemcpyHostToDevice, c->st));
  DepthArgs a;
  memset(&a, 0, sizeof(a));
  a.slot = d_slot; a.nslot = 1; a.stride = 16; a.off_xyz = 0; a.n_total = (int)sweep.n; a.kp_total = (int)n_kp;
  a.flag = d_flag; a.d_n = c->d_knn_n; a.d_total = c->map.vx.d_n_out; a.dc_off = (unsigned*)(c->d_knn_n + 2); a.ndc = c->d_knn_n + 1; a.dc = d_dc;
  a.grid = c->gknn;
  lvo_launch_depth(c->st, a, (int)sweep.n, c->map.vx.scan, &c->launches);
  int ndc = 0;
  LVO_CUDA_OK(c, cudaMemcpyAsync(&ndc, a.ndc, 4, cudaMemcpyDeviceToHost, c->st));
  if (n_kp) {
    LVO_CUDA_OK(c, cudaMemcpyAsync(depth_out, slot.depth, n_kp * 4, cudaMemcpyDeviceToHost, c->st));
    LVO_CUDA_OK(c, cudaMemcpyAsync(valid_out, slot.valid, n_kp * 4, cudaMemcpyDeviceToHost, c->st));
    if (nn_out) LVO_CUDA_OK(c, cudaMemcpyAsync(nn_out, slot.nn, n_kp * 12, cudaMemcpyDeviceToHost, c->st));
  }
  LVO_CUDA_OK(c, cudaStreamSynchronize(c->st));
  LVO_CUDA_OK(c, cudaGetLastError());
  if (sweep.n == 0) ndc = 0;
  int r = download_cloud(c, d_dc, (size_t)ndc, depth_cloud_or_null);
  LVO_CUDA_OK(c, cudaStreamSynchronize(c->st));
  return r;
}

static size_t depth_slot_bytes(int slots) { return ((size_t)slots * sizeof(DepthSlot) + 15) & ~(size_t)15; }

static int depth_reserve(lvo_ctx* c, size_t pts, size_t raw, size_t kp, int slots) {
  lvo_ctx::DepthArena& d = c->depth;
  if (d.cnt && pts <= d.cap_pts && raw <= d.cap_raw && kp <= d.cap_kp && slots <= d.cap_slots) return LVO_OK;
  pts = std::max(pts, d.cap_pts); raw = std::max(raw, d.cap_raw); kp = std::max(kp, d.cap_kp); slots = std::max(slots, d.cap_slots);
  for (void* p : d.dev) cudaFree(p);
  for (void* p : d.pin) cudaFreeHost(p);
  d.dev.clear(); d.pin.clear(); d.cnt = nullptr;
  d.cap_pts = d.cap_raw = d.cap_kp = 0; d.cap_slots = 0;
  bool ok = true;
  auto dev = [&](auto** p, size_t bytes) {
    void* q = nullptr;
    if (ok && cudaMalloc(&q, std::max<size_t>(bytes, 16)) == cudaSuccess) d.dev.push_back(q);
    else ok = false;
    *p = (std::remove_reference_t<decltype(**p)>*)q;
  };
  auto pin = [&](auto** p, size_t bytes) {
    void* q = nullptr;
    if (ok && cudaMallocHost(&q, std::max<size_t>(bytes, 16)) == cudaSuccess) d.pin.push_back(q);
    else ok = false;
    *p = (std::remove_reference_t<decltype(**p)>*)q;
  };
  const size_t cells = (size_t)slots * LVO_DEPTH_CELLS + 1;
  dev(&d.raw, raw); dev(&d.flag, 4 * pts); dev(&d.dc, 16 * pts);
  dev(&d.d_in, depth_slot_bytes(slots) + 8 * kp); pin(&d.h_in, depth_slot_bytes(slots) + 8 * kp);
  dev(&d.d_res, 20 * kp); pin(&d.h_res, 20 * kp);
  dev(&d.dc_off, 4 * (size_t)slots); dev(&d.ndc, 4 * (size_t)slots);
  GridSet& g = d.grid;
  memset(&g, 0, sizeof(g));
  g.cells_cap_per_problem = LVO_DEPTH_CELLS;
  dev(&g.prob, sizeof(GridProblem) * slots); dev(&g.table, 4 * cells); dev(&g.d_table_len, 4);
  dev(&g.rank, 4 * pts); dev(&g.pt_off, 4 * ((size_t)slots + 1)); dev(&g.sorted_pts, 16 * pts);
  g.scan.cap_tiles = lvo_div_up((long long)std::max(pts, cells), LVO_SCAN_TILE) + 2;
  dev(&g.scan.partial, 4 * (size_t)g.scan.cap_tiles);
  int* cnt = nullptr;
  dev(&cnt, 8);
  if (!ok) {
    for (void* p : d.dev) cudaFree(p);
    for (void* p : d.pin) cudaFreeHost(p);
    d.dev.clear(); d.pin.clear();
    lvo_set_error(c, "lvo_depth_associate_batch: out of memory");
    return LVO_E_CUDA;
  }
  d.cnt = cnt;
  d.cap_pts = pts; d.cap_raw = raw; d.cap_kp = kp; d.cap_slots = slots;
  return LVO_OK;
}

static int depth_check_keypoints(lvo_ctx* c, const void* const* kp, const size_t* n_kp, const void* const* depth, const void* const* valid, const void* const* nn) {
  for (int l = 0; l < c->lanes; ++l) {
    if (!c->lane_active[l] || n_kp[l] == 0) continue;
    if (2 * n_kp[l] > (size_t)c->P) { lvo_set_error(c, "too many keypoints"); return LVO_E_CAPACITY; }
    if (!kp[l] || !depth[l] || !valid[l] || (nn && !nn[l])) { lvo_set_error(c, "NULL keypoint or output pointer of an active lane"); return LVO_E_BADARG; }
  }
  return LVO_OK;
}

static int depth_enqueue(lvo_ctx* c, int nslot, size_t n_total, size_t kp_total, int max_n, int stride, int off_xyz, size_t in_bytes) {
  lvo_ctx::DepthArena& d = c->depth;
  LVO_CUDA_OK(c, cudaMemcpyAsync(d.d_in, d.h_in, in_bytes, cudaMemcpyHostToDevice, c->st));
  DepthArgs a;
  memset(&a, 0, sizeof(a));
  a.slot = (const DepthSlot*)d.d_in; a.nslot = nslot; a.stride = stride; a.off_xyz = off_xyz;
  a.n_total = (int)n_total; a.kp_total = (int)kp_total;
  a.flag = d.flag; a.d_n = d.cnt; a.d_total = (unsigned*)(d.cnt + 1); a.dc_off = d.dc_off; a.ndc = d.ndc; a.dc = d.dc;
  a.grid = d.grid;
  a.grid.nprob = nslot; a.grid.table_cap_total = (long long)nslot * LVO_DEPTH_CELLS; a.grid.pts_cap_per_problem = std::max(max_n, 1);
  lvo_launch_depth(c->st, a, max_n, d.grid.scan, &c->launches);
  return LVO_OK;
}

static void depth_slot_camera(DepthSlot& s, const lvo_camera& cam) { for (int k = 0; k < 12; ++k) s.extr[k] = cam.extrinsic[k]; }

int lvo_depth_associate_batch(lvo_ctx* c, const lvo_camera* cams, const lvo_cloud_view* sweeps, const float* const* keypoints_uv, const size_t* n_kp,
                              float* const* depth_out, int* const* valid_out, int* const* nn_out_or_null) {
  LvoDeviceGuard _dev(c);
  if (!c) return LVO_E_BADARG;
  if (c->pending) { lvo_set_error(c, "lvo_wait has not been called for the last *_async step"); return LVO_E_STATE; }
  if (!cams || !sweeps || !keypoints_uv || !n_kp || !depth_out || !valid_out) { lvo_set_error(c, "NULL array"); return LVO_E_BADARG; }
  int max_n = 0, stride = 16, off_xyz = 0;
  LVO_TRY(check_sweeps(c, sweeps, &max_n, &stride, &off_xyz));
  LVO_TRY(depth_check_keypoints(c, (const void* const*)keypoints_uv, n_kp, (const void* const*)depth_out, (const void* const*)valid_out,
                                (const void* const*)nn_out_or_null));
  int A = 0; size_t N = 0, K = 0;
  for (int l = 0; l < c->lanes; ++l) if (c->lane_active[l]) { A++; N += sweeps[l].n; K += n_kp[l]; }
  if (N > INT_MAX || K > INT_MAX) { lvo_set_error(c, "too many points or keypoints in one call"); return LVO_E_CAPACITY; }
  c->launches = 0;
  if (A == 0) return LVO_OK;
  LVO_TRY(depth_reserve(c, N, N * stride, K, A));
  lvo_ctx::DepthArena& d = c->depth;
  DepthSlot* hs = (DepthSlot*)d.h_in;
  float* huv = (float*)(d.h_in + depth_slot_bytes(A));
  const float* d_uv = (const float*)(d.d_in + depth_slot_bytes(A));
  float* r_depth = (float*)d.d_res; int* r_valid = (int*)d.d_res + K; int* r_nn = (int*)d.d_res + 2 * K;
  struct Run { const unsigned char* host; size_t bytes; size_t dev_off; };
  std::vector<Run> runs;
  int s = 0; size_t po = 0, ko = 0;
  for (int l = 0; l < c->lanes; ++l) {
    if (!c->lane_active[l]) continue;
    const lvo_cloud_view& v = sweeps[l];
    DepthSlot& t = hs[s++];
    memset(&t, 0, sizeof(t));
    t.pts = d.raw + po * stride; t.n = (int)v.n; t.pt_off = (unsigned)po;
    t.uv = d_uv + 2 * ko; t.nkp = (int)n_kp[l]; t.kp_off = (unsigned)ko;
    t.depth = r_depth + ko; t.valid = r_valid + ko; t.nn = nn_out_or_null ? r_nn + 3 * ko : nullptr;
    depth_slot_camera(t, cams[l]);
    if (n_kp[l]) memcpy(huv + 2 * ko, keypoints_uv[l], 8 * n_kp[l]);
    if (v.n) {
      const unsigned char* h = (const unsigned char*)v.data;
      const size_t bytes = v.n * stride;
      if (!runs.empty() && runs.back().host + runs.back().bytes == h) runs.back().bytes += bytes;
      else runs.push_back(Run{h, bytes, po * stride});
    }
    po += v.n; ko += n_kp[l];
  }
  for (const Run& r : runs) LVO_CUDA_OK(c, cudaMemcpyAsync(d.raw + r.dev_off, r.host, r.bytes, cudaMemcpyHostToDevice, c->st));
  LVO_TRY(depth_enqueue(c, A, N, K, max_n, stride, off_xyz, depth_slot_bytes(A) + 8 * K));
  const size_t res_words = (nn_out_or_null ? 5 : 2) * K;
  if (res_words) LVO_CUDA_OK(c, cudaMemcpyAsync(d.h_res, d.d_res, 4 * res_words, cudaMemcpyDeviceToHost, c->st));
  LVO_CUDA_OK(c, cudaStreamSynchronize(c->st));
  LVO_CUDA_OK(c, cudaGetLastError());
  const float* h_depth = (const float*)d.h_res; const int* h_valid = (const int*)d.h_res + K; const int* h_nn = (const int*)d.h_res + 2 * K;
  ko = 0;
  for (int l = 0; l < c->lanes; ++l) {
    if (!c->lane_active[l] || n_kp[l] == 0) continue;
    memcpy(depth_out[l], h_depth + ko, 4 * n_kp[l]);
    memcpy(valid_out[l], h_valid + ko, 4 * n_kp[l]);
    if (nn_out_or_null) memcpy(nn_out_or_null[l], h_nn + 3 * ko, 12 * n_kp[l]);
    ko += n_kp[l];
  }
  return LVO_OK;
}

int lvo_depth_associate_batch_dev(lvo_ctx* c, const lvo_camera* cams, const lvo_point* const* d_sweeps, const size_t* n, const float* const* d_keypoints_uv,
                                  const size_t* n_kp, float* const* d_depth_out, int* const* d_valid_out, int* const* d_nn_out_or_null) {
  LvoDeviceGuard _dev(c);
  if (!c) return LVO_E_BADARG;
  if (c->pending) { lvo_set_error(c, "lvo_wait has not been called for the last *_async step"); return LVO_E_STATE; }
  if (!cams || !d_sweeps || !n || !d_keypoints_uv || !n_kp || !d_depth_out || !d_valid_out) { lvo_set_error(c, "NULL array"); return LVO_E_BADARG; }
  int A = 0, max_n = 0; size_t N = 0, K = 0;
  for (int l = 0; l < c->lanes; ++l) {
    if (!c->lane_active[l]) continue;
    if (n[l] > (size_t)c->P) { lvo_set_error(c, "input cloud exceeds context capacity"); return LVO_E_CAPACITY; }
    if (n[l] && !d_sweeps[l]) { lvo_set_error(c, "NULL sweep of an active lane"); return LVO_E_BADARG; }
    A++; N += n[l]; K += n_kp[l]; max_n = std::max(max_n, (int)n[l]);
  }
  LVO_TRY(depth_check_keypoints(c, (const void* const*)d_keypoints_uv, n_kp, (const void* const*)d_depth_out, (const void* const*)d_valid_out,
                                (const void* const*)d_nn_out_or_null));
  if (N > INT_MAX || K > INT_MAX) { lvo_set_error(c, "too many points or keypoints in one call"); return LVO_E_CAPACITY; }
  c->launches = 0;
  if (A == 0) return LVO_OK;
  LVO_TRY(depth_reserve(c, N, 0, 0, A));
  DepthSlot* hs = (DepthSlot*)c->depth.h_in;
  int s = 0; size_t po = 0, ko = 0;
  for (int l = 0; l < c->lanes; ++l) {
    if (!c->lane_active[l]) continue;
    DepthSlot& t = hs[s++];
    memset(&t, 0, sizeof(t));
    t.pts = (const unsigned char*)d_sweeps[l]; t.n = (int)n[l]; t.pt_off = (unsigned)po;
    t.uv = d_keypoints_uv[l]; t.nkp = (int)n_kp[l]; t.kp_off = (unsigned)ko;
    t.depth = d_depth_out[l]; t.valid = d_valid_out[l]; t.nn = d_nn_out_or_null ? d_nn_out_or_null[l] : nullptr;
    depth_slot_camera(t, cams[l]);
    po += n[l]; ko += n_kp[l];
  }
  LVO_TRY(depth_enqueue(c, A, N, K, max_n, 16, 0, depth_slot_bytes(A)));
  LVO_CUDA_OK(c, cudaStreamSynchronize(c->st));
  LVO_CUDA_OK(c, cudaGetLastError());
  return LVO_OK;
}

int lvo_knn5_throughput(lvo_ctx* c, const lvo_point* d_maps, const int* map_counts, const lvo_point* d_queries, const int* query_counts, int S, int reps,
                        int* d_ind_out, float* d_sq_out, float* ms) {
  LvoDeviceGuard _dev(c);
  if (!c || !d_maps || !map_counts || !d_queries || !query_counts || S < 1 || reps < 1 || !d_ind_out || !d_sq_out || !ms) return LVO_E_BADARG;
  std::vector<unsigned> moff(S + 1, 0), qoff(S + 1, 0);
  int maxm = 1, maxq = 1;
  for (int p = 0; p < S; ++p) {
    if (map_counts[p] < 0 || query_counts[p] < 0) return LVO_E_BADARG;
    moff[p + 1] = moff[p] + (unsigned)map_counts[p]; qoff[p + 1] = qoff[p] + (unsigned)query_counts[p];
    maxm = std::max(maxm, map_counts[p]); maxq = std::max(maxq, query_counts[p]);
  }
  std::vector<void*> tmp;
  auto talloc = [&](void** p, size_t bytes) { cudaError_t e = cudaMalloc(p, std::max<size_t>(bytes, 16)); if (e == cudaSuccess) { tmp.push_back(*p); cudaMemsetAsync(*p, 0, std::max<size_t>(bytes, 16), c->st); } return e; };
  auto cleanup = [&]() { cudaStreamSynchronize(c->st); for (void* p : tmp) cudaFree(p); };
  GridSet g; memset(&g, 0, sizeof(g));
  const int cells_cap = 1 << 21;
  g.nprob = S; g.cells_cap_per_problem = cells_cap; g.pts_cap_per_problem = maxm;
  unsigned* d_moff = nullptr; unsigned* d_qoff = nullptr; int* d_mcnt = nullptr;
  const size_t total_m = moff[S];
  const size_t table_n = (size_t)S * cells_cap + 1;
  bool ok = talloc((void**)&g.prob, sizeof(GridProblem) * S) == cudaSuccess && talloc((void**)&g.table, 4 * table_n) == cudaSuccess &&
            talloc((void**)&g.d_table_len, 4) == cudaSuccess && talloc((void**)&g.rank, 4 * total_m) == cudaSuccess &&
            talloc((void**)&g.pt_off, 4 * (size_t)(S + 1)) == cudaSuccess && talloc((void**)&g.sorted_pts, 16 * total_m) == cudaSuccess &&
            talloc((void**)&g.sorted_id, 4 * total_m) == cudaSuccess &&
            talloc((void**)&g.scan.partial, 4 * (size_t)(lvo_div_up((long long)table_n, LVO_SCAN_TILE) + 2)) == cudaSuccess &&
            talloc((void**)&d_moff, 4 * (size_t)(S + 1)) == cudaSuccess && talloc((void**)&d_qoff, 4 * (size_t)(S + 1)) == cudaSuccess &&
            talloc((void**)&d_mcnt, 4 * (size_t)S) == cudaSuccess;
  if (!ok) { cleanup(); lvo_set_error(c, "lvo_knn5_throughput: out of device memory"); return LVO_E_CUDA; }
  g.scan.cap_tiles = lvo_div_up((long long)table_n, LVO_SCAN_TILE) + 2;
  cudaError_t ce = cudaMemcpyAsync(d_moff, moff.data(), 4 * (size_t)(S + 1), cudaMemcpyHostToDevice, c->st);
  if (ce == cudaSuccess) ce = cudaMemcpyAsync(d_qoff, qoff.data(), 4 * (size_t)(S + 1), cudaMemcpyHostToDevice, c->st);
  if (ce == cudaSuccess) ce = cudaMemcpyAsync(d_mcnt, map_counts, 4 * (size_t)S, cudaMemcpyHostToDevice, c->st);
  if (ce == cudaSuccess) ce = cudaStreamSynchronize(c->st);
  if (ce != cudaSuccess) { cleanup(); lvo_set_error(c, std::string("lvo_knn5_throughput: ") + cudaGetErrorString(ce)); return LVO_E_CUDA; }
  k_setup_batch_problems<<<lvo_div_up(S, 64), 64, 0, c->st>>>(g.prob, S, (const float4*)d_maps, d_moff, d_mcnt, 1.0f);
  c->launches = 0;
  lvo_grid_build(c->st, g, &c->launches);
  dim3 grid(std::max(1, std::min(lvo_div_up(maxq, 128), 256)), S);
// ... 24 lines not shown
```

lidar-visual-odometry_b200/csrc/lvo_mapping.cuh:

```cuda
#pragma once
#include "lvo_internal.h"
#include "lvo_knn.cuh"
#include "lvo_solver.cuh"
#include "lvo_voxel.cuh"

#define LVO_SEG_NONVALID 75
#define LVO_SEG_TRASH 76
#define LVO_MSEGS 77

struct MapArgs {
  LaneState* ls;
  int lanes, outer, from_odo;
  const int* lane_flags;
  const LaneConfig* lcfg;
  const float4* in_pts[2]; int in_cap[2];
  const float4* full; int P;
  float4* map_pts[2][2];
  unsigned* cube_start[2][2];
  int map_cap[2];
  int gen;
  float4* from_map[2];
  float4* stack[2];
  GridSet grid;
  VoxelEngine vx;
  unsigned* item_off;
  LvoFactor* factors; int factor_cap;
  unsigned* app_cnt;
  unsigned* app_first;
  unsigned* new_cnt;
  int* knn_ind[2];
  int* fac_valid[2];
  int slots;
  int knn_reuse;
  float4* knn_ref[2];
  int* knn_sel[2];
  int* knn_flag[2];
  int* fit_list;
  int* fit_cnt;
  float4* registered;
};

__device__ __forceinline__ int cube_index(int i, int j, int k) { return i + LVO_CUBE_W * j + LVO_CUBE_W * LVO_CUBE_H * k; }

__global__ void k_map_begin(MapArgs a) {
  const int lane = blockIdx.x * blockDim.x + threadIdx.x;
  if (lane >= a.lanes) return;
  LaneState& s = a.ls[lane];
  if (!lane_maps(a.lane_flags, lane)) { s.map_done = 1; return; }
  if (a.from_odo) { for (int k = 0; k < 4; ++k) s.q_wodom[k] = s.q_w[k]; for (int k = 0; k < 3; ++k) s.t_wodom[k] = s.t_w[k]; }
  quat_mul(s.q_wmap_wodom, s.q_wodom, s.map_x);
  const d3 r = quat_rotate(s.q_wmap_wodom, d3{s.t_wodom[0], s.t_wodom[1], s.t_wodom[2]});
  s.map_x[4] = r.x + s.t_wmap_wodom[0]; s.map_x[5] = r.y + s.t_wmap_wodom[1]; s.map_x[6] = r.z + s.t_wmap_wodom[2];
  const int dims[3] = {LVO_CUBE_W, LVO_CUBE_H, LVO_CUBE_D};
  for (int c = 0; c < 3; ++c) {
    int center = cube_coord(s.map_x[4 + c], s.cen[c]);
    int sh = 0;
    while (center < 3) { center++; sh++; }
    while (center >= dims[c] - 3) { center--; sh--; }
    s.center[c] = center; s.cen[c] += sh; s.shift[c] = sh;
  }
  int nv = 0;
  for (int i = s.center[0] - 2; i <= s.center[0] + 2; i++)
    for (int j = s.center[1] - 2; j <= s.center[1] + 2; j++)
      for (int k = s.center[2] - 1; k <= s.center[2] + 1; k++)
        if (i >= 0 && i < LVO_CUBE_W && j >= 0 && j < LVO_CUBE_H && k >= 0 && k < LVO_CUBE_D) s.valid_cube[nv++] = cube_index(i, j, k);
  s.n_valid = nv;
  for (int t = 0; t < 2; ++t) {
    const unsigned* cs = a.cube_start[a.gen][t] + (size_t)lane * (LVO_NCUBES + 1);
    int acc = 0;
    for (int v = 0; v < nv; ++v) {
      const int c = s.valid_cube[v];
      const int i = c % LVO_CUBE_W - s.shift[0], j = (c / LVO_CUBE_W) % LVO_CUBE_H - s.shift[1], k = c / (LVO_CUBE_W * LVO_CUBE_H) - s.shift[2];
      int cnt = 0;
      if (i >= 0 && i < LVO_CUBE_W && j >= 0 && j < LVO_CUBE_H && k >= 0 && k < LVO_CUBE_D) { const int oc = cube_index(i, j, k); cnt = (int)(cs[oc + 1] - cs[oc]); }
      s.from_off[t][v] = acc;
      acc += cnt;
    }
    for (int v = nv; v <= LVO_MAX_VALID; ++v) s.from_off[t][v] = acc;
  }
  s.stats.map_corner_from_map = s.from_off[0][LVO_MAX_VALID];
  s.stats.map_surf_from_map = s.from_off[1][LVO_MAX_VALID];
  s.map_too_small = !(s.from_off[0][LVO_MAX_VALID] > 10 && s.from_off[1][LVO_MAX_VALID] > 50);
  s.map_status = s.map_too_small ? LVO_W_MAP_TOO_SMALL : LVO_OK;
  s.map_done = 0; s.stats.map_outer_executed = 0;
  for (int o = 0; o < LVO_MAX_OUTER; ++o) { s.stats.map_corner_corr[o] = 0; s.stats.map_surf_corr[o] = 0; s.stats.map_lm_iters[o] = 0; s.stats.map_final_cost[o] = 0; s.stats.map_knn_full[o] = 0; if (a.fit_cnt) a.fit_cnt[lane * LVO_MAX_OUTER + o] = 0; }
  for (int c = 0; c < 3; ++c) { s.stats.center_cube[c] = s.center[c]; s.stats.cen[c] = s.cen[c]; }
}

__global__ void k_map_gather(MapArgs a) {
  const int v = blockIdx.x, lt = blockIdx.y, lane = lt >> 1, t = lt & 1;
  const LaneState& s = a.ls[lane];
  const bool maps = lane_maps(a.lane_flags, lane);
  if (v >= s.n_valid || !maps) return;
  const int c = s.valid_cube[v];
  const int i = c % LVO_CUBE_W - s.shift[0], j = (c / LVO_CUBE_W) % LVO_CUBE_H - s.shift[1], k = c / (LVO_CUBE_W * LVO_CUBE_H) - s.shift[2];
  if (!(i >= 0 && i < LVO_CUBE_W && j >= 0 && j < LVO_CUBE_H && k >= 0 && k < LVO_CUBE_D)) return;
  const int oc = cube_index(i, j, k);
  const unsigned* cs = a.cube_start[a.gen][t] + (size_t)lane * (LVO_NCUBES + 1);
  const unsigned b = cs[oc], e = cs[oc + 1];
  const float4* src = a.map_pts[a.gen][t] + (size_t)lane * a.map_cap[t];
  float4* dst = a.from_map[t] + (size_t)lane * a.map_cap[t] + s.from_off[t][v];
  for (unsigned x = b + threadIdx.x; x < e; x += blockDim.x) dst[x - b] = src[x];
}

__global__ void __launch_bounds__(256) k_stack_offsets(MapArgs a) {
  __shared__ unsigned sm[33];
  const int L2 = 2 * a.lanes;
  unsigned acc = 0;
  for (int base = 0; base < L2; base += blockDim.x) {
    const int lt = base + threadIdx.x;
    unsigned v = 0;
    if (lt < L2) {
      const LaneState& s = a.ls[lt >> 1];
      if (lane_maps(a.lane_flags, lt >> 1)) v = (unsigned)((lt & 1) ? s.n_less_flat : s.n_less_sharp);
      a.vx.seg_leaf[lt] = a.lcfg[lt >> 1].leaf[lt & 1];
    }
    unsigned tot;
    const unsigned ex = block_excl_scan(v, sm, &tot);
    if (lt < L2) a.item_off[lt] = acc + ex;
    acc += tot;
  }
  if (threadIdx.x == 0) { a.item_off[L2] = acc; *a.vx.d_n = (int)acc; *a.vx.d_nsegs = L2; }
}
__global__ void k_stack_gather(MapArgs a) {
  const int lt = blockIdx.y, lane = lt >> 1, t = lt & 1;
  const LaneState& s = a.ls[lane];
  const int n = t ? s.n_less_flat : s.n_less_sharp;
  if (!lane_maps(a.lane_flags, lane)) return;
  const float4* src = a.in_pts[t] + (size_t)lane * a.in_cap[t];
  const unsigned off = a.item_off[lt];
  for (int i = blockIdx.x * blockDim.x + threadIdx.x; i < n; i += gridDim.x * blockDim.x) {
    a.vx.in_pts[off + i] = src[i];
    a.vx.in_seg[off + i] = lt;
    a.vx.in_aux[off + i] = 0;
  }
}
__global__ void k_stack_scatter(MapArgs a) {
  const int lt = blockIdx.y, lane = lt >> 1, t = lt & 1;
  LaneState& s = a.ls[lane];
  const unsigned b = a.vx.seg_out_start[lt], n = a.vx.seg_out_cnt[lt];
  if (!lane_maps(a.lane_flags, lane)) return;
  float4* dst = a.stack[t] + (size_t)lane * a.in_cap[t];
  for (unsigned i = blockIdx.x * blockDim.x + threadIdx.x; i < n; i += gridDim.x * blockDim.x) dst[i] = a.vx.out_pts[b + i];
  if (blockIdx.x == 0 && threadIdx.x == 0) {
    s.n_stack[t] = (int)n;
    if (t == 0) s.stats.map_corner_stack = (int)n; else s.stats.map_surf_stack = (int)n;
  }
}

__device__ __forceinline__ void fit_factor(int t, const float4 ori, const float4* __restrict__ M, const int* id, LvoFactor& fac) {
  float4 nb[5];
#pragma unroll
  for (int j = 0; j < 5; ++j) nb[j] = M[id[j]];
  if (t == 0) {
    d3 center{0, 0, 0};
#pragma unroll
    for (int j = 0; j < 5; ++j) { center.x = center.x + (double)nb[j].x; center.y = center.y + (double)nb[j].y; center.z = center.z + (double)nb[j].z; }
    center.x = center.x / 5.0; center.y = center.y / 5.0; center.z = center.z / 5.0;
    double cov[9] = {0, 0, 0, 0, 0, 0, 0, 0, 0};
#pragma unroll
    for (int j = 0; j < 5; ++j) {
      const double z[3] = {(double)nb[j].x - center.x, (double)nb[j].y - center.y, (double)nb[j].z - center.z};
#pragma unroll
      for (int r = 0; r < 3; ++r)
#pragma unroll
        for (int c = 0; c < 3; ++c) cov[r * 3 + c] = cov[r * 3 + c] + z[r] * z[c];
    }
    double w[3], V[9];
    sym_eigen3_dev(cov, w, V);
    if (w[2] > 3 * w[1]) {
      const double ux = V[0 * 3 + 2], uy = V[1 * 3 + 2], uz = V[2 * 3 + 2];
      fac.type = 0; fac.d = 1.0;
      fac.c[0] = ori.x; fac.c[1] = ori.y; fac.c[2] = ori.z;
      fac.a[0] = 0.1 * ux + center.x; fac.a[1] = 0.1 * uy + center.y; fac.a[2] = 0.1 * uz + center.z;
      const double lb[3] = {-0.1 * ux + center.x, -0.1 * uy + center.y, -0.1 * uz + center.z};
      lvo_edge_direction(fac.a, lb, fac.b);
    }
  } else {
    double A[15], b[5] = {-1, -1, -1, -1, -1}, n[3];
#pragma unroll
    for (int j = 0; j < 5; ++j) { A[j * 3 + 0] = nb[j].x; A[j * 3 + 1] = nb[j].y; A[j * 3 + 2] = nb[j].z; }
    if (!lsq_qr_5x3(A, b, n)) return;
    const double nn = sqrt(n[0] * n[0] + n[1] * n[1] + n[2] * n[2]);
    if (!(nn > 0.0) || !isfinite(nn)) return;
    const double negOA = 1 / nn;
    n[0] /= nn; n[1] /= nn; n[2] /= nn;
    bool planeValid = true;
#pragma unroll
    for (int j = 0; j < 5; ++j)
      if (!(fabs(n[0] * nb[j].x + n[1] * nb[j].y + n[2] * nb[j].z + negOA) <= 0.2)) { planeValid = false; }
    if (planeValid) {
      fac.type = 2;
      fac.c[0] = ori.x; fac.c[1] = ori.y; fac.c[2] = ori.z;
      fac.a[0] = n[0]; fac.a[1] = n[1]; fac.a[2] = n[2];
      fac.b[0] = fac.b[1] = fac.b[2] = 0;
      fac.d = negOA;
    }
  }
}

__global__ void __launch_bounds__(128) k_map_knn(MapArgs a) {
  const int lane = blockIdx.y;
  const LaneState& s = a.ls[lane];
  if (s.map_too_small || s.map_done) return;
  const int n0 = s.n_stack[0], ntot = n0 + s.n_stack[1];
  const GridView g0 = grid_view(a.grid, 2 * lane), g1 = grid_view(a.grid, 2 * lane + 1);
  for (int f = blockIdx.x * blockDim.x + threadIdx.x; f < ntot; f += gridDim.x * blockDim.x) {
    const int t = f >= n0 ? 1 : 0;
    const int i = t ? f - n0 : f;
    const float4 ori = a.stack[t][(size_t)lane * a.in_cap[t] + i];
    const float4 sel = transform_point(s.map_x, s.map_x + 4, ori);
    TopK<5> tk;
    const bool ok = thread_knn<5>(t ? g1 : g0, sel.x, sel.y, sel.z, 1.0f, tk);
    int* ki = a.knn_ind[t] + (((size_t)lane * a.slots + a.outer % a.slots) * a.in_cap[t] + i) * 5;
#pragma unroll
    for (int k = 0; k < 5; ++k) ki[k] = ok ? tk.id[k] : -1;
  }
}
#define LVO_KNN_PRUNE_SQ 1.21f
#define LVO_KF_ROW 1
#define LVO_KF_FACTOR 2
#define LVO_KF_CHANGED 4

__device__ __forceinline__ float knn_guard(const GridView& g, float qx, float qy, float qz, const TopK<6>& tk) {
  const float fx = floorf(qx * g.inv_cell), fy = floorf(qy * g.inv_cell), fz = floorf(qz * g.inv_cell_z);
  if (!(g.dim[0] > 0 && fabsf(fx) < 8.0e6f && fabsf(fy) < 8.0e6f && fabsf(fz) < 8.0e6f)) return 0.f;
  const float cz_size = 1.0f / g.inv_cell_z;
  const float lx = qx - fx * g.cell, ly = qy - fy * g.cell, lz = qz - fz * cz_size;
  const float bx = fminf(lx, g.cell - lx) + g.cell, by = fminf(ly, g.cell - ly) + g.cell, bz = fminf(lz, cz_size - lz) + cz_size;
  float gd = fminf(fminf(bx, by), bz);
  gd = fminf(gd, sqrtf(tk.d[5]));
  return fmaxf(gd * 0.9999f - 1e-5f, 0.f);
}

__device__ __forceinline__ void thread_knn6_block(const GridView& g, float qx, float qy, float qz, TopK<6>& tk) {
  tk.init(LVO_KNN_PRUNE_SQ);
  if (g.dim[0] <= 0) return;
  const int cx = cell_coord(qx, g.inv_cell) - g.org[0], cy = cell_coord(qy, g.inv_cell) - g.org[1], cz = cell_coord(qz, g.inv_cell_z) - g.org[2];
  unsigned rb[9], re[9];
  const int x0 = max(cx - 1, 0), x1 = min(cx + 1, g.dim[0] - 1);
#pragma unroll
  for (int k = 0; k < 9; ++k) {
    const int z = cz + k / 3 - 1, y = cy + k % 3 - 1;
    rb[k] = re[k] = 0;
    if (z >= 0 && z < g.dim[2] && y >= 0 && y < g.dim[1] && x0 <= x1) {
      const int rowbase = (z * g.dim[1] + y) * g.dim[0];
      rb[k] = __ldg(g.cell_start + rowbase + x0); re[k] = __ldg(g.cell_start + rowbase + x1 + 1);
    }
  }
#pragma unroll 1
  for (int k = 0; k < 9; ++k) {
    unsigned t = rb[k];
    const unsigned e = re[k];
    for (; t + 4 <= e; t += 4) {
      const float4 p0 = __ldg(g.pts + t), p1 = __ldg(g.pts + t + 1), p2 = __ldg(g.pts + t + 2), p3 = __ldg(g.pts + t + 3);
      tk.insert(sqdist3(p0, qx, qy, qz), __float_as_int(p0.w));
      tk.insert(sqdist3(p1, qx, qy, qz), __float_as_int(p1.w));
      tk.insert(sqdist3(p2, qx, qy, qz), __float_as_int(p2.w));
      tk.insert(sqdist3(p3, qx, qy, qz), __float_as_int(p3.w));
    }
    if (t < e) {
      const float4 p0 = __ldg(g.pts + t);
      const float4 p1 = t + 1 < e ? __ldg(g.pts + t + 1) : p0;
      const float4 p2 = t + 2 < e ? __ldg(g.pts + t + 2) : p0;
      tk.insert(sqdist3(p0, qx, qy, qz), __float_as_int(p0.w));
      if (t + 1 < e) tk.insert(sqdist3(p1, qx, qy, qz), __float_as_int(p1.w));
      if (t + 2 < e) tk.insert(sqdist3(p2, qx, qy, qz), __float_as_int(p2.w));
    }
  }
}

template <int K, int TW>
__device__ __forceinline__ void tile_merge(TopK<K>& tk) {
  float rd[K]; int ri[K];
  int ptr = 0;
#pragma unroll
  for (int k = 0; k < K; ++k) {
    float cd = FLT_MAX; int ci = INT_MAX;
#pragma unroll
    for (int j = 0; j < K; ++j) if (j == ptr) { cd = tk.d[j]; ci = tk.id[j]; }
    float bd = cd; int bi = ci;
#pragma unroll
    for (int o = TW / 2; o > 0; o >>= 1) {
      const float od = __shfl_xor_sync(0xffffffffu, bd, o, TW);
      const int oi = __shfl_xor_sync(0xffffffffu, bi, o, TW);
      if (TopK<K>::less(od, oi, bd, bi)) { bd = od; bi = oi; }
    }
    rd[k] = bd; ri[k] = bi;
    if (bi == ci && bd == cd && ci != INT_MAX) ptr++;
  }
#pragma unroll
  for (int k = 0; k < K; ++k) { tk.d[k] = rd[k]; tk.id[k] = ri[k]; }
}

__device__ __forceinline__ void tile8_knn6_block(const GridView& g, bool active, float qx, float qy, float qz, TopK<6>& tk, float& guard) {
  const int tl = (int)tile_lane<8>();
  tk.init(LVO_KNN_PRUNE_SQ);
  guard = 0.f;
  const int cx = cell_coord(qx, g.inv_cell) - g.org[0], cy = cell_coord(qy, g.inv_cell) - g.org[1], cz = cell_coord(qz, g.inv_cell_z) - g.org[2];
  auto consider = [&](float4 p, int) { tk.insert(sqdist3(p, qx, qy, qz), __float_as_int(p.w)); };
#pragma unroll 1
  for (int base = 0; base < 9; base += 8) {
    const int row = base + tl;
    unsigned b = 0, e = 0;
    if (active && g.dim[0] > 0 && row < 9) row_bounds(g, cz + row / 3 - 1, cy + row % 3 - 1, cx - 1, cx + 1, b, e);
    tile_scan_ranges<8, 8>(g.pts, b, e, consider);
  }
  tile_merge<6, 8>(tk);
  guard = knn_guard(g, qx, qy, qz, tk);
}

__global__ void __launch_bounds__(128) k_map_knn_reuse(MapArgs a) {
  __shared__ float4 s_sel[128];
  __shared__ int s_list[128], s_fit[128];
  __shared__ int s_n, s_nfit, s_off;
  const int lane = blockIdx.y;
  const LaneState& s = a.ls[lane];
  if (s.map_too_small || s.map_done) return;
  const int n0 = s.n_stack[0], ntot = n0 + s.n_stack[1];
  int nc = 0, nsf = 0;
  __shared__ GridView gv[2];
  if (threadIdx.x < 2) gv[threadIdx.x] = grid_view(a.grid, 2 * lane + threadIdx.x);
  const float4* M0 = a.from_map[0] + (size_t)lane * a.map_cap[0];
  const float4* M1 = a.from_map[1] + (size_t)lane * a.map_cap[1];
  const int slot = a.outer % a.slots;
  for (int base = blockIdx.x * blockDim.x; base < ntot; base += gridDim.x * blockDim.x) {
    if (threadIdx.x == 0) { s_n = 0; s_nfit = 0; }
    __syncthreads();
    const int f = base + threadIdx.x;
    bool need_full = false, refit = false;
    if (f < ntot) {
      need_full = true;
      const int t = f >= n0 ? 1 : 0;
      const int i = t ? f - n0 : f;
      const size_t qi = (size_t)lane * a.in_cap[t] + i;
      const float4 ori = a.stack[t][qi];
      const float4 sel = transform_point(s.map_x, s.map_x + 4, ori);
      s_sel[threadIdx.x] = sel;
      if (a.outer > 0) {
        const float4 ref = a.knn_ref[t][qi];
        const int flag = a.knn_flag[t][qi];
        int id[5], old[5];
#pragma unroll
        for (int k = 0; k < 5; ++k) old[k] = id[k] = a.knn_sel[t][qi * 5 + k];
        const float4* M = t ? M1 : M0;
        float d[5];
#pragma unroll
        for (int k = 0; k < 5; ++k) d[k] = id[k] != INT_MAX ? sqdist3(M[id[k]], sel.x, sel.y, sel.z) : FLT_MAX;
#pragma unroll
        for (int k = 1; k < 5; ++k)
#pragma unroll
          for (int j = k; j > 0; --j)
            if (TopK<5>::less(d[j], id[j], d[j - 1], id[j - 1])) {
              const float td = d[j]; d[j] = d[j - 1]; d[j - 1] = td;
              const int ti = id[j]; id[j] = id[j - 1]; id[j - 1] = ti;
            }
        const float dx = sel.x - ref.x, dy = sel.y - ref.y, dz = sel.z - ref.z;
        const float delta = sqrtf(dx * dx + dy * dy + dz * dz) * 1.0001f + 1e-5f;
        const float B = ref.w - delta;
        const bool full_set = id[4] != INT_MAX;
        bool decided = false, row_ok = false;
        if (full_set && sqrtf(d[4]) * 1.0001f + 1e-5f < B) { decided = true; row_ok = (double)d[4] < 1.0; }
        else if (B > 1.0002f) { decided = true; row_ok = full_set && (double)d[4] < 1.0; }
        if (decided) {
          need_full = false;
          bool reordered = false;
#pragma unroll
          for (int k = 0; k < 5; ++k) if (old[k] != id[k]) { reordered = true; a.knn_sel[t][qi * 5 + k] = id[k]; }
          if (a.slots > 2) {
            int* ki = a.knn_ind[t] + (((size_t)lane * a.slots + slot) * a.in_cap[t] + i) * 5;
#pragma unroll
            for (int k = 0; k < 5; ++k) ki[k] = row_ok ? id[k] : -1;
          }
          const bool changed = row_ok != ((flag & LVO_KF_ROW) != 0) || (row_ok && reordered);
          a.knn_flag[t][qi] = (flag & LVO_KF_FACTOR) | (row_ok ? LVO_KF_ROW : 0) | (changed ? LVO_KF_CHANGED : 0);
          refit = changed;
          if (!changed) {
            const int v = (flag & LVO_KF_FACTOR) ? 1 : 0;
            if (a.slots > 2) a.fac_valid[t][((size_t)lane * a.slots + slot) * a.in_cap[t] + i] = v;
            if (v) { if (t == 0) nc++; else nsf++; }
          }
        }
      }
    }
    {
      const unsigned m = __ballot_sync(0xffffffffu, need_full);
      int off = 0;
      if ((threadIdx.x & 31) == 0 && m) off = atomicAdd(&s_n, __popc(m));
      off = __shfl_sync(0xffffffffu, off, 0);
      if (need_full) s_list[off + __popc(m & ((1u << (threadIdx.x & 31)) - 1u))] = (int)threadIdx.x;
      const unsigned m2 = __ballot_sync(0xffffffffu, refit);
      int off2 = 0;
      if ((threadIdx.x & 31) == 0 && m2) off2 = atomicAdd(&s_nfit, __popc(m2));
      off2 = __shfl_sync(0xffffffffu, off2, 0);
      if (refit) s_fit[off2 + __popc(m2 & ((1u << (threadIdx.x & 31)) - 1u))] = (int)threadIdx.x;
    }
    __syncthreads();
    const int nfull = s_n;
    const int nfit = s_nfit + nfull;
    if (a.outer > 0 && nfit > 0) {
      if (threadIdx.x == 0) s_off = atomicAdd(&a.fit_cnt[lane * LVO_MAX_OUTER + a.outer], nfit);
      __syncthreads();
      int* fl = a.fit_list + (size_t)lane * (a.in_cap[0] + a.in_cap[1]) + s_off;
      if ((int)threadIdx.x < nfit) fl[threadIdx.x] = base + ((int)threadIdx.x < s_nfit ? s_fit[threadIdx.x] : s_list[threadIdx.x - s_nfit]);
    }
    if (threadIdx.x == 0 && nfull) atomicAdd(&a.ls[lane].stats.map_knn_full[a.outer], nfull);
    if (a.outer == 0) {
      if (f < ntot) {
        const int t = f >= n0 ? 1 : 0;
        const int i = t ? f - n0 : f;
        const size_t qi = (size_t)lane * a.in_cap[t] + i;
        const float4 sel = s_sel[threadIdx.x];
        TopK<6> tk;
        thread_knn6_block(gv[t], sel.x, sel.y, sel.z, tk);
        const float guard = knn_guard(gv[t], sel.x, sel.y, sel.z, tk);
        const bool row_ok = tk.id[4] != INT_MAX && (double)tk.d[4] < 1.0;
#pragma unroll
        for (int k = 0; k < 5; ++k) a.knn_sel[t][qi * 5 + k] = tk.id[k];
        if (a.slots > 2) {
          int* ki = a.knn_ind[t] + (((size_t)lane * a.slots + slot) * a.in_cap[t] + i) * 5;
#pragma unroll
          for (int k = 0; k < 5; ++k) ki[k] = row_ok ? tk.id[k] : -1;
        }
        a.knn_ref[t][qi] = make_float4(sel.x, sel.y, sel.z, guard);
        a.knn_flag[t][qi] = (row_ok ? LVO_KF_ROW : 0) | LVO_KF_CHANGED;
      }
      __syncthreads();
      continue;
    }
    const int w = threadIdx.x >> 5, tile = (threadIdx.x & 31) >> 3;
    for (int e0 = 4 * w; e0 < nfull; e0 += 16) {
      const int e = e0 + tile;
      const bool active = e < nfull;
      const int src = active ? s_list[e] : 0;
      const int f2 = base + src;
      const int t = (active && f2 >= n0) ? 1 : 0;
      const float4 sel = s_sel[src];
      TopK<6> tk;
      float guard;
      tile8_knn6_block(gv[t], active, sel.x, sel.y, sel.z, tk, guard);
      if (active && tile_lane<8>() == 0) {
        const int i = t ? f2 - n0 : f2;
        const size_t qi = (size_t)lane * a.in_cap[t] + i;
        const bool row_ok = tk.id[4] != INT_MAX && (double)tk.d[4] < 1.0;
#pragma unroll
        for (int k = 0; k < 5; ++k) a.knn_sel[t][qi * 5 + k] = tk.id[k];
        if (a.slots > 2) {
          int* ki = a.knn_ind[t] + (((size_t)lane * a.slots + slot) * a.in_cap[t] + i) * 5;
#pragma unroll
          for (int k = 0; k < 5; ++k) ki[k] = row_ok ? tk.id[k] : -1;
        }
        a.knn_ref[t][qi] = make_float4(sel.x, sel.y, sel.z, guard);
        const int oldf = a.knn_flag[t][qi];
        a.knn_flag[t][qi] = (oldf & LVO_KF_FACTOR) | (row_ok ? LVO_KF_ROW : 0) | LVO_KF_CHANGED;
      }
    }
    __syncthreads();
  }
  nc = __reduce_add_sync(0xffffffffu, nc);
  nsf = __reduce_add_sync(0xffffffffu, nsf);
  if ((threadIdx.x & 31) == 0) {
    if (nc) atomicAdd(&a.ls[lane].stats.map_corner_corr[a.outer], nc);
    if (nsf) atomicAdd(&a.ls[lane].stats.map_surf_corr[a.outer], nsf);
  }
}

__global__ void __launch_bounds__(128) k_map_fit_reuse(MapArgs a) {
  const int lane = blockIdx.y;
  LaneState& s = a.ls[lane];
  if (s.map_too_small || s.map_done) return;
  const int n0 = s.n_stack[0], ntot = n0 + s.n_stack[1];
  const int n = a.outer > 0 ? a.fit_cnt[lane * LVO_MAX_OUTER + a.outer] : ntot;
  const int* fl = a.fit_list + (size_t)lane * (a.in_cap[0] + a.in_cap[1]);
  const float4* M0 = a.from_map[0] + (size_t)lane * a.map_cap[0];
  const float4* M1 = a.from_map[1] + (size_t)lane * a.map_cap[1];
  const int slot = a.outer % a.slots;
  int nc = 0, nsf = 0;
  for (int base = blockIdx.x * blockDim.x; base < n; base += gridDim.x * blockDim.x) {
    const int e = base + threadIdx.x;
    if (e < n) {
      const int f2 = a.outer > 0 ? fl[e] : e;
      const int t = f2 >= n0 ? 1 : 0;
      const int i = t ? f2 - n0 : f2;
      const size_t qi = (size_t)lane * a.in_cap[t] + i;
      const int flag = a.knn_flag[t][qi];
      LvoFactor fac;
      fac.type = -1; fac.pad = 0; fac.d = 0;
      if (flag & LVO_KF_ROW) {
        int id[5];
#pragma unroll
        for (int k = 0; k < 5; ++k) id[k] = a.knn_sel[t][qi * 5 + k];
        fit_factor(t, a.stack[t][qi], t ? M1 : M0, id, fac);
      }
      a.factors[(size_t)lane * a.factor_cap + f2] = fac;
      const int v = fac.type >= 0 ? 1 : 0;
      if (a.slots > 2) a.fac_valid[t][((size_t)lane * a.slots + slot) * a.in_cap[t] + i] = v;
      a.knn_flag[t][qi] = (flag & LVO_KF_ROW) | (v ? LVO_KF_FACTOR : 0);
      if (v) { if (t == 0) nc++; else nsf++; }
    }
  }
  nc = __reduce_add_sync(0xffffffffu, nc);
  nsf = __reduce_add_sync(0xffffffffu, nsf);
  if ((threadIdx.x & 31) == 0) {
    if (nc) atomicAdd(&s.stats.map_corner_corr[a.outer], nc);
    if (nsf) atomicAdd(&s.stats.map_surf_corr[a.outer], nsf);
  }
}

__global__ void __launch_bounds__(128) k_map_fit(MapArgs a) {
  const int lane = blockIdx.y;
  LaneState& s = a.ls[lane];
  if (s.map_too_small || s.map_done) return;
  const int n0 = s.n_stack[0], ntot = n0 + s.n_stack[1];
  const float4* M0 = a.from_map[0] + (size_t)lane * a.map_cap[0];
  const float4* M1 = a.from_map[1] + (size_t)lane * a.map_cap[1];
  int nc = 0, nsf = 0;
  for (int base = blockIdx.x * blockDim.x; base < ntot; base += gridDim.x * blockDim.x) {
    const int f = base + threadIdx.x;
    if (f < ntot) {
      const int t = f >= n0 ? 1 : 0;
      const int i = t ? f - n0 : f;
      const int* ki = a.knn_ind[t] + (((size_t)lane * a.slots + a.outer % a.slots) * a.in_cap[t] + i) * 5;
      int id[5];
#pragma unroll
      for (int k = 0; k < 5; ++k) id[k] = ki[k];
      LvoFactor fac;
      fac.type = -1; fac.pad = 0; fac.d = 0;
      if (id[0] >= 0) fit_factor(t, a.stack[t][(size_t)lane * a.in_cap[t] + i], t ? M1 : M0, id, fac);
      a.factors[(size_t)lane * a.factor_cap + f] = fac;
      a.fac_valid[t][((size_t)lane * a.slots + a.outer % a.slots) * a.in_cap[t] + i] = fac.type >= 0 ? 1 : 0;
      if (fac.type >= 0) { if (t == 0) nc++; else nsf++; }
    }
  }
  nc = __reduce_add_sync(0xffffffffu, nc);
  nsf = __reduce_add_sync(0xffffffffu, nsf);
  if ((threadIdx.x & 31) == 0) {
    if (nc) atomicAdd(&s.stats.map_corner_corr[a.outer], nc);
    if (nsf) atomicAdd(&s.stats.map_surf_corr[a.outer], nsf);
  }
}

__global__ void k_map_finish(MapArgs a) {
  const int lane = blockIdx.x * blockDim.x + threadIdx.x;
  if (lane >= a.lanes || !lane_maps(a.lane_flags, lane)) return;
  LaneState& s = a.ls[lane];
  const double* q = s.q_wodom;
  const double n2 = q[0] * q[0] + q[1] * q[1] + q[2] * q[2] + q[3] * q[3];
  const double qi[4] = {-q[0] / n2, -q[1] / n2, -q[2] / n2, q[3] / n2};
  quat_mul(s.map_x, qi, s.q_wmap_wodom);
  const d3 r = quat_rotate(s.q_wmap_wodom, d3{s.t_wodom[0], s.t_wodom[1], s.t_wodom[2]});
  s.t_wmap_wodom[0] = s.map_x[4] - r.x; s.t_wmap_wodom[1] = s.map_x[5] - r.y; s.t_wmap_wodom[2] = s.map_x[6] - r.z;
}

__global__ void __launch_bounds__(256) k_refilter_offsets(MapArgs a) {
  __shared__ unsigned sm[33];
  const int L2 = 2 * a.lanes;
  const int nw = blockDim.x >> 5, ln = threadIdx.x & 31;
  for (int r0 = threadIdx.x >> 5; r0 < L2; r0 += 32 * nw) {
    const int mine = r0 + ln * nw;
    const float my_leaf = mine < L2 ? a.lcfg[mine >> 1].leaf[mine & 1] : 0.f;
    for (int j = 0; j < 32; ++j) {
      const float leaf = __shfl_sync(0xffffffffu, my_leaf, j);
      const int lt = r0 + j * nw;
      if (lt >= L2) break;
      for (int k = ln; k < LVO_MSEGS; k += 32) a.vx.seg_leaf[lt * LVO_MSEGS + k] = k < LVO_MAX_VALID ? leaf : 0.f;
    }
  }
  unsigned acc = 0;
  for (int base = 0; base < L2; base += blockDim.x) {
    const int lt = base + threadIdx.x;
    unsigned v = 0;
    if (lt < L2 && lane_updates_map(a.lane_flags, lt >> 1)) { const LaneState& s = a.ls[lt >> 1]; v = (unsigned)(s.from_off[lt & 1][LVO_MAX_VALID] + s.n_stack[lt & 1]); }
    unsigned tot;
    const unsigned ex = block_excl_scan(v, sm, &tot);
    if (lt < L2) a.item_off[lt] = acc + ex;
    acc += tot;
  }
  if (threadIdx.x == 0) { a.item_off[L2] = acc; *a.vx.d_n = (int)acc; *a.vx.d_nsegs = L2 * LVO_MSEGS; }
}
__global__ void k_refilter_gather(MapArgs a) {
  const int lt = blockIdx.y, lane = lt >> 1, t = lt & 1;
  const LaneState& s = a.ls[lane];
  const int nfrom = s.from_off[t][LVO_MAX_VALID], nst = s.n_stack[t];
  if (!lane_updates_map(a.lane_flags, lane)) return;
  const unsigned off = a.item_off[lt];
  const float4* FM = a.from_map[t] + (size_t)lane * a.map_cap[t];
  const float4* ST = a.stack[t] + (size_t)lane * a.in_cap[t];
  for (int i = blockIdx.x * blockDim.x + threadIdx.x; i < nfrom + nst; i += gridDim.x * blockDim.x) {
    float4 p; int seg; unsigned aux = 0;
    if (i < nfrom) {
      p = FM[i];
      int lo = 0, hi = s.n_valid - 1;
      while (lo < hi) { const int mid = (lo + hi + 1) >> 1; if (s.from_off[t][mid] <= i) lo = mid; else hi = mid - 1; }
      seg = lo;
    } else {
      p = transform_point(s.map_x, s.map_x + 4, ST[i - nfrom]);
      const int ci = cube_coord((double)p.x, s.cen[0]), cj = cube_coord((double)p.y, s.cen[1]), ck = cube_coord((double)p.z, s.cen[2]);
      if (ci >= 0 && ci < LVO_CUBE_W && cj >= 0 && cj < LVO_CUBE_H && ck >= 0 && ck < LVO_CUBE_D) {
        const int di = ci - (s.center[0] - 2), dj = cj - (s.center[1] - 2), dk = ck - (s.center[2] - 1);
        aux = (unsigned)cube_index(ci, cj, ck);
        if (di >= 0 && di < 5 && dj >= 0 && dj < 5 && dk >= 0 && dk < 3) seg = (di * 5 + dj) * 3 + dk;
        else seg = LVO_SEG_NONVALID;
      } else seg = LVO_SEG_TRASH;
    }
    a.vx.in_pts[off + i] = p;
    a.vx.in_seg[off + i] = lt * LVO_MSEGS + seg;
    a.vx.in_aux[off + i] = aux;
  }
}
__global__ void k_rebuild_reset(MapArgs a) {
  const int n = 2 * a.lanes * LVO_NCUBES;
  for (int i = blockIdx.x * blockDim.x + threadIdx.x; i < n; i += gridDim.x * blockDim.x) { a.app_cnt[i] = 0; a.app_first[i] = 0xffffffffu; }
}
__global__ void k_rebuild_appended(MapArgs a) {
  const int lt = blockIdx.y;
  const int seg = lt * LVO_MSEGS + LVO_SEG_NONVALID;
  const unsigned b = a.vx.seg_out_start[seg], n = a.vx.seg_out_cnt[seg];
  for (unsigned i = blockIdx.x * blockDim.x + threadIdx.x; i < n; i += gridDim.x * blockDim.x) {
    const unsigned cube = a.vx.out_aux[b + i];
    atomicAdd(&a.app_cnt[(size_t)lt * LVO_NCUBES + cube], 1u);
    atomicMin(&a.app_first[(size_t)lt * LVO_NCUBES + cube], b + i);
  }
}
__global__ void __launch_bounds__(256) k_rebuild_offsets(MapArgs a) {
  __shared__ unsigned sm[33];
  __shared__ signed char vrank[LVO_NCUBES];
  const int lt = blockIdx.x, lane = lt >> 1, t = lt & 1;
  LaneState& s = a.ls[lane];
  const bool maps = lane_maps(a.lane_flags, lane), updates = lane_updates_map(a.lane_flags, lane);
  for (int c = threadIdx.x; c < LVO_NCUBES; c += blockDim.x) vrank[c] = -1;
  __syncthreads();
  if (updates && threadIdx.x < s.n_valid) vrank[s.valid_cube[threadIdx.x]] = (signed char)threadIdx.x;
  __syncthreads();
  const unsigned* cs = a.cube_start[a.gen][t] + (size_t)lane * (LVO_NCUBES + 1);
  unsigned* ncs = a.cube_start[a.gen ^ 1][t] + (size_t)lane * (LVO_NCUBES + 1);
  unsigned carry = 0;
  for (int base = 0; base < LVO_NCUBES; base += blockDim.x) {
    const int c = base + threadIdx.x;
    unsigned cnt = 0;
    if (c < LVO_NCUBES) {
      const int v = vrank[c];
      if (v >= 0) cnt = a.vx.seg_out_cnt[lt * LVO_MSEGS + v];
      else {
        const int i = c % LVO_CUBE_W - s.shift[0], j = (c / LVO_CUBE_W) % LVO_CUBE_H - s.shift[1], k = c / (LVO_CUBE_W * LVO_CUBE_H) - s.shift[2];
        if (i >= 0 && i < LVO_CUBE_W && j >= 0 && j < LVO_CUBE_H && k >= 0 && k < LVO_CUBE_D) { const int oc = cube_index(i, j, k); cnt = cs[oc + 1] - cs[oc]; }
        cnt += a.app_cnt[(size_t)lt * LVO_NCUBES + c];
      }
    }
    unsigned tot;
    const unsigned ex = block_excl_scan(cnt, sm, &tot);
    if (c < LVO_NCUBES) ncs[c] = min(carry + ex, (unsigned)a.map_cap[t]);
    carry += tot;
  }
  if (threadIdx.x == 0) {
    const unsigned kept = min(carry, (unsigned)a.map_cap[t]);
    ncs[LVO_NCUBES] = kept;
    if (!maps) return;
    s.n_map[t] = (int)kept;
    if (t == 0) s.stats.map_corner_total = (int)kept; else s.stats.map_surf_total = (int)kept;
    if (carry > (unsigned)a.map_cap[t]) s.map_status = LVO_E_CAPACITY;
  }
}
__global__ void __launch_bounds__(256) k_rebuild_copy(MapArgs a) {
  __shared__ signed char vrank[LVO_NCUBES];
  const int lt = blockIdx.y, lane = lt >> 1, t = lt & 1;
  const LaneState& s = a.ls[lane];
  const bool updates = lane_updates_map(a.lane_flags, lane);
  for (int c = threadIdx.x; c < LVO_NCUBES; c += blockDim.x) vrank[c] = -1;
  __syncthreads();
  if (updates && threadIdx.x < s.n_valid) vrank[s.valid_cube[threadIdx.x]] = (signed char)threadIdx.x;
  __syncthreads();
  const unsigned* cs = a.cube_start[a.gen][t] + (size_t)lane * (LVO_NCUBES + 1);
  const unsigned* ncs = a.cube_start[a.gen ^ 1][t] + (size_t)lane * (LVO_NCUBES + 1);
  const float4* src = a.map_pts[a.gen][t] + (size_t)lane * a.map_cap[t];
  float4* dst = a.map_pts[a.gen ^ 1][t] + (size_t)lane * a.map_cap[t];
  const unsigned n = min(ncs[LVO_NCUBES], (unsigned)a.map_cap[t]);
  for (unsigned d = blockIdx.x * blockDim.x + threadIdx.x; d < n; d += gridDim.x * blockDim.x) {
    int lo = 0, hi = LVO_NCUBES - 1;
    while (lo < hi) { const int mid = (lo + hi + 1) >> 1; if (ncs[mid] <= d) lo = mid; else hi = mid - 1; }
    const int c = lo;
    const unsigned r = d - ncs[c];
    const int v = vrank[c];
    float4 p;
    if (v >= 0) p = a.vx.out_pts[a.vx.seg_out_start[lt * LVO_MSEGS + v] + r];
    else {
      const int i = c % LVO_CUBE_W - s.shift[0], j = (c / LVO_CUBE_W) % LVO_CUBE_H - s.shift[1], k = c / (LVO_CUBE_W * LVO_CUBE_H) - s.shift[2];
      unsigned ocnt = 0, ob = 0;
      if (i >= 0 && i < LVO_CUBE_W && j >= 0 && j < LVO_CUBE_H && k >= 0 && k < LVO_CUBE_D) { const int oc = cube_index(i, j, k); ob = cs[oc]; ocnt = cs[oc + 1] - ob; }
      if (r < ocnt) p = src[ob + r];
      else p = a.vx.out_pts[a.app_first[(size_t)lt * LVO_NCUBES + c] + (r - ocnt)];
    }
    dst[d] = p;
  }
}
__global__ void k_map_end(MapArgs a) {
  const int lane = blockIdx.x * blockDim.x + threadIdx.x;
  if (lane >= a.lanes) return;
  LaneState& s = a.ls[lane];
  s.shift[0] = s.shift[1] = s.shift[2] = 0;
}
__global__ void k_register(MapArgs a) {
  const int lane = blockIdx.y;
  const LaneState& s = a.ls[lane];
  const int n = s.n_kept;
  if (!lane_maps(a.lane_flags, lane)) return;
  for (int i = blockIdx.x * blockDim.x + threadIdx.x; i < n; i += gridDim.x * blockDim.x)
    a.registered[(size_t)lane * a.P + i] = transform_point(s.map_x, s.map_x + 4, a.full[(size_t)lane * a.P + i]);
}

static inline void lvo_launch_mapping(cudaStream_t st, MapArgs a, const SolveArgs& solve_proto, int outer_iters, int lanes, bool want_registered,
                                      long long* launches, LvoStageTimer* tm = nullptr) {
  const int L2 = 2 * lanes;
  LVO_MARK(tm, LVO_ST_MAP_PREPARE, st);
  k_map_begin<<<lvo_div_up(lanes, 64), 64, 0, st>>>(a);
  k_map_gather<<<dim3(LVO_MAX_VALID, L2), 128, 0, st>>>(a);
  k_stack_offsets<<<1, 256, 0, st>>>(a);
  k_stack_gather<<<dim3(16, L2), 256, 0, st>>>(a);
  if (launches) *launches += 4;
  int seg_bits = 1; while ((1 << seg_bits) < L2) seg_bits++;
  lvo_voxel_run(st, a.vx, lanes * (a.in_cap[0] + a.in_cap[1]), L2, seg_bits, launches);
  k_stack_scatter<<<dim3(8, L2), 256, 0, st>>>(a);
  if (launches) *launches += 1;
  LVO_MARK(tm, LVO_ST_MAP_TREE, st);
  lvo_grid_build(st, a.grid, launches);
  const int nstack_cap = a.in_cap[0] + a.in_cap[1];
  dim3 ga(max(1, min(lvo_div_up(nstack_cap, 128), 128)), lanes);
  dim3 gr(max(1, min(lvo_div_up(nstack_cap, 128), 32)), lanes), gf(max(1, min(lvo_div_up(nstack_cap, 128), 8)), lanes), gf2(max(1, min(lvo_div_up(nstack_cap, 128), 16)), lanes);
  for (int o = 0; o < outer_iters; ++o) {
    a.outer = o;
    LVO_MARK(tm, LVO_ST_MAP_KNN, st);
    if (a.knn_reuse) k_map_knn_reuse<<<gr, 128, 0, st>>>(a);
    else k_map_knn<<<ga, 128, 0, st>>>(a);
    LVO_MARK(tm, LVO_ST_MAP_FIT, st);
    if (a.knn_reuse) k_map_fit_reuse<<<o == 0 ? gr : (o <= 2 ? gf2 : gf), 128, 0, st>>>(a);
    else k_map_fit<<<ga, 128, 0, st>>>(a);
    if (launches) *launches += 1;
    SolveArgs sa = solve_proto;
    sa.which = 1; sa.outer = o; sa.n_outer = outer_iters; sa.factors = a.factors; sa.factor_cap = a.factor_cap; sa.distort = 0; sa.reset_cnt = nullptr;
    LVO_MARK(tm, LVO_ST_MAP_SOLVER, st);
    lvo_launch_lm(st, sa, lanes, 16384);
    if (launches) *launches += 2;
  }
  LVO_MARK(tm, LVO_ST_MAP_ADD, st);
  k_map_finish<<<lvo_div_up(lanes, 64), 64, 0, st>>>(a);
  k_refilter_offsets<<<1, 256, 0, st>>>(a);
  k_refilter_gather<<<dim3(64, L2), 256, 0, st>>>(a);
  if (launches) *launches += 3;
  LVO_MARK(tm, LVO_ST_MAP_FILTER, st);
  int seg_bits2 = 1; while ((1 << seg_bits2) < L2 * LVO_MSEGS) seg_bits2++;
  lvo_voxel_run(st, a.vx, a.vx.cap_items, L2 * LVO_MSEGS, seg_bits2, launches);
  k_rebuild_reset<<<148, 256, 0, st>>>(a);
  k_rebuild_appended<<<dim3(4, L2), 256, 0, st>>>(a);
  k_rebuild_offsets<<<L2, 256, 0, st>>>(a);
  k_rebuild_copy<<<dim3(64, L2), 256, 0, st>>>(a);
  k_map_end<<<lvo_div_up(lanes, 64), 64, 0, st>>>(a);
  if (launches) *launches += 5;
  LVO_MARK(tm, LVO_ST_MAP_PUB, st);
  if (want_registered && a.registered) { k_register<<<dim3(64, lanes), 256, 0, st>>>(a); if (launches) *launches += 1; }
}
```

lidar-visual-odometry_b200/csrc/lvo_prims.cuh:

```cuda
#pragma once
#include "lvo_internal.h"

#define LVO_SCAN_THREADS 256
#define LVO_SCAN_ITEMS 8
#define LVO_SCAN_TILE (LVO_SCAN_THREADS * LVO_SCAN_ITEMS)

#define LVO_SORT_THREADS 256
#define LVO_SORT_ITEMS 16
#define LVO_SORT_TILE (LVO_SORT_THREADS * LVO_SORT_ITEMS)
#define LVO_SORT_WARPS (LVO_SORT_THREADS / 32)

__device__ __forceinline__ unsigned warp_incl_scan(unsigned v) {
  const unsigned lane = threadIdx.x & 31;
#pragma unroll
  for (int o = 1; o < 32; o <<= 1) {
    unsigned t = __shfl_up_sync(0xffffffffu, v, o);
    if (lane >= (unsigned)o) v += t;
  }
  return v;
}
__device__ __forceinline__ unsigned block_excl_scan(unsigned v, unsigned* sm, unsigned* total) {
  const unsigned lane = threadIdx.x & 31, w = threadIdx.x >> 5, nw = blockDim.x >> 5;
  unsigned inc = warp_incl_scan(v);
  if (lane == 31) sm[w] = inc;
  __syncthreads();
  if (w == 0) {
    unsigned x = lane < nw ? sm[lane] : 0;
    unsigned xi = warp_incl_scan(x);
    sm[lane] = xi - x;
    if (lane == 31) sm[32] = xi;
  }
  __syncthreads();
  unsigned r = sm[w] + inc - v;
  *total = sm[32];
  __syncthreads();
  return r;
}

__device__ __forceinline__ unsigned block_flag_rank(bool flag, unsigned* sm, int phase, unsigned* total) {
  const unsigned lane = threadIdx.x & 31, w = threadIdx.x >> 5, nw = blockDim.x >> 5;
  const unsigned m = __ballot_sync(0xffffffffu, flag);
  unsigned* cnt = sm + 32 * (phase & 1);
  if (lane == 0) cnt[w] = __popc(m);
  __syncthreads();
  unsigned pre = 0, tot = 0;
  for (unsigned ww = 0; ww < nw; ++ww) { const unsigned c = cnt[ww]; tot += c; if (ww < w) pre += c; }
  *total = tot;
  return pre + __popc(m & ((1u << lane) - 1u));
}

__global__ void k_scan_reduce(const unsigned* __restrict__ data, const int* __restrict__ d_n, unsigned* __restrict__ partial) {
  __shared__ unsigned sm[33];
  const int n = *d_n;
  const int ntiles = (n + LVO_SCAN_TILE - 1) / LVO_SCAN_TILE;
  for (int tile = blockIdx.x; tile < ntiles; tile += gridDim.x) {
    unsigned s = 0;
    const int base = tile * LVO_SCAN_TILE;
#pragma unroll
    for (int k = 0; k < LVO_SCAN_ITEMS; ++k) {
      int i = base + k * LVO_SCAN_THREADS + threadIdx.x;
      if (i < n) s += data[i];
    }
    unsigned tot;
    block_excl_scan(s, sm, &tot);
    if (threadIdx.x == 0) partial[tile] = tot;
  }
}
__global__ void k_scan_partials(unsigned* __restrict__ partial, const int* __restrict__ d_n, unsigned* __restrict__ d_total) {
  __shared__ unsigned sm[33];
  const int n = *d_n;
  const int ntiles = (n + LVO_SCAN_TILE - 1) / LVO_SCAN_TILE;
  unsigned carry = 0;
  for (int base = 0; base < ntiles; base += blockDim.x) {
    int i = base + threadIdx.x;
    unsigned v = i < ntiles ? partial[i] : 0;
    unsigned tot;
    unsigned ex = block_excl_scan(v, sm, &tot);
    if (i < ntiles) partial[i] = carry + ex;
    carry += tot;
  }
  if (threadIdx.x == 0 && d_total) *d_total = carry;
}
__global__ void k_scan_apply(unsigned* __restrict__ data, const int* __restrict__ d_n, const unsigned* __restrict__ partial) {
  __shared__ unsigned sm[33];
  const int n = *d_n;
  const int ntiles = (n + LVO_SCAN_TILE - 1) / LVO_SCAN_TILE;
  for (int tile = blockIdx.x; tile < ntiles; tile += gridDim.x) {
    const int base = tile * LVO_SCAN_TILE + threadIdx.x * LVO_SCAN_ITEMS;
    unsigned v[LVO_SCAN_ITEMS];
    unsigned s = 0;
#pragma unroll
    for (int k = 0; k < LVO_SCAN_ITEMS; ++k) {
      v[k] = (base + k < n) ? data[base + k] : 0;
      s += v[k];
    }
    unsigned tot;
    unsigned ex = block_excl_scan(s, sm, &tot) + partial[tile];
#pragma unroll
    for (int k = 0; k < LVO_SCAN_ITEMS; ++k) {
      if (base + k < n) data[base + k] = ex;
      ex += v[k];
    }
  }
}

struct LvoScanScratch { unsigned* partial; int cap_tiles; };

static inline void lvo_scan_exclusive(cudaStream_t st, unsigned* data, const int* d_n, int n_cap, unsigned* d_total, const LvoScanScratch& sc,
                                      long long* launches) {
  int tiles = lvo_div_up(n_cap, LVO_SCAN_TILE);
  int grid = tiles < 1184 ? (tiles < 1 ? 1 : tiles) : 1184;
  k_scan_reduce<<<grid, LVO_SCAN_THREADS, 0, st>>>(data, d_n, sc.partial);
  k_scan_partials<<<1, 1024, 0, st>>>(sc.partial, d_n, d_total);
  k_scan_apply<<<grid, LVO_SCAN_THREADS, 0, st>>>(data, d_n, sc.partial);
  if (launches) *launches += 3;
}

struct LvoSortBufs {
  unsigned long long* keys[2];
  unsigned* vals[2];
  unsigned* ghist;
  unsigned long long* status;
  unsigned* d_epoch;
  int cap;
};
#define LVO_SORT_GHIST_WORDS (8 * 256 + 8)

__device__ __forceinline__ int lvo_sort_passes(int bits) { return (bits + 7) >> 3; }

__global__ void __launch_bounds__(256) k_sort_ghist(const unsigned long long* __restrict__ keys, const int* __restrict__ d_n, const int* __restrict__ d_bits,
                                                    unsigned* __restrict__ ghist, unsigned* __restrict__ d_epoch) {
  __shared__ unsigned h[8][256];
  const int passes = min(lvo_sort_passes(*d_bits), 8);
  const int n = *d_n;
  if (blockIdx.x == 0 && threadIdx.x == 0) *d_epoch = *d_epoch + 1u;
  for (int k = threadIdx.x; k < 8 * 256; k += blockDim.x) (&h[0][0])[k] = 0;
  __syncthreads();
  for (int i = blockIdx.x * blockDim.x + threadIdx.x; i < n; i += gridDim.x * blockDim.x) {
    const unsigned long long key = keys[i];
    for (int p = 0; p < passes; ++p) atomicAdd(&h[p][(unsigned)(key >> (8 * p)) & 255u], 1u);
  }
  __syncthreads();
  for (int k = threadIdx.x; k < passes * 256; k += blockDim.x) { const unsigned v = (&h[0][0])[k]; if (v) atomicAdd(&ghist[k], v); }
}

__global__ void __launch_bounds__(LVO_SORT_THREADS, 2)
k_sort_onesweep(unsigned long long* __restrict__ keys0, unsigned long long* __restrict__ keys1, unsigned* __restrict__ vals0,
                unsigned* __restrict__ vals1, const int* __restrict__ d_n, const int* __restrict__ d_bits, int pass,
                unsigned* __restrict__ ghist, unsigned long long* status, const unsigned* __restrict__ d_epoch) {
  __shared__ unsigned wcnt[LVO_SORT_WARPS][256];
  __shared__ unsigned gbase[256];
  __shared__ unsigned sm_scan[33];
  __shared__ int s_tile;
  const int bits = *d_bits;
  if (pass * 8 >= bits) return;
  const int n = *d_n;
  const int ntiles = (n + LVO_SORT_TILE - 1) / LVO_SORT_TILE;
  const unsigned long long* kin = (pass & 1) ? keys1 : keys0;
  unsigned long long* kout = (pass & 1) ? keys0 : keys1;
  const unsigned* vin = (pass & 1) ? vals1 : vals0;
  unsigned* vout = (pass & 1) ? vals0 : vals1;
  const int shift = pass * 8;
  const unsigned lane = threadIdx.x & 31, w = threadIdx.x >> 5;
  const unsigned lt = (1u << lane) - 1u;
  const unsigned tag = 2u * (8u * (*d_epoch) + (unsigned)pass);
  unsigned* ticket = ghist + 8 * 256 + pass;
  unsigned tot_unused;
  const unsigned digit_base = block_excl_scan(ghist[pass * 256 + threadIdx.x], sm_scan, &tot_unused);
  while (true) {
    if (threadIdx.x == 0) s_tile = (int)atomicAdd(ticket, 1u);
    for (int k = threadIdx.x; k < LVO_SORT_WARPS * 256; k += LVO_SORT_THREADS) (&wcnt[0][0])[k] = 0;
    __syncthreads();
    const int tile = s_tile;
    if (tile >= ntiles) break;
    unsigned long long key[LVO_SORT_ITEMS];
    unsigned val[LVO_SORT_ITEMS];
    unsigned short lpos[LVO_SORT_ITEMS];
    const int wbase = tile * LVO_SORT_TILE + w * (32 * LVO_SORT_ITEMS);
#pragma unroll
    for (int r = 0; r < LVO_SORT_ITEMS; ++r) {
      const int i = wbase + r * 32 + lane;
      const bool valid = i < n;
      key[r] = valid ? kin[i] : 0ull;
      val[r] = valid ? vin[i] : 0u;
      const unsigned digit = (unsigned)(key[r] >> shift) & 255u;
      const unsigned m = __match_any_sync(0xffffffffu, valid ? digit : 256u);
      const unsigned rank = __popc(m & lt);
      unsigned base = 0;
      if (valid) base = wcnt[w][digit];
      __syncwarp();
      if (valid && rank == 0) wcnt[w][digit] = base + __popc(m);
      __syncwarp();
      lpos[r] = (unsigned short)(base + rank);
    }
    __syncthreads();
    {
      const unsigned d = threadIdx.x;
      unsigned run = 0;
#pragma unroll
      for (int ww = 0; ww < LVO_SORT_WARPS; ++ww) {
        unsigned t = wcnt[ww][d];
        wcnt[ww][d] = run;
        run += t;
      }
      volatile unsigned long long* st = status;
      unsigned excl = 0;
      if (tile > 0) {
        st[(size_t)tile * 256 + d] = ((unsigned long long)tag << 32) | run;
        for (int t = tile - 1; t >= 0; --t) {
          unsigned long long v;
          do { v = st[(size_t)t * 256 + d]; } while (((unsigned)(v >> 32) | 1u) != (tag | 1u));
          excl += (unsigned)v;
          if ((unsigned)(v >> 32) & 1u) break;
        }
      }
      st[(size_t)tile * 256 + d] = ((unsigned long long)(tag | 1u) << 32) | (excl + run);
      gbase[d] = digit_base + excl;
    }
    __syncthreads();
#pragma unroll
    for (int r = 0; r < LVO_SORT_ITEMS; ++r) {
      const int i = wbase + r * 32 + lane;
      if (i < n) {
        const unsigned digit = (unsigned)(key[r] >> shift) & 255u;
        const unsigned pos = gbase[digit] + wcnt[w][digit] + lpos[r];
        kout[pos] = key[r];
        vout[pos] = val[r];
      }
    }
    __syncthreads();
  }
}

static inline void lvo_sort_pairs(cudaStream_t st, const LvoSortBufs& b, const int* d_n, int n_cap, const int* d_bits, int max_bits,
                                  long long* launches) {
  int tiles = lvo_div_up(n_cap, LVO_SORT_TILE);
  int grid = tiles < 592 ? (tiles < 1 ? 1 : tiles) : 592;
  int passes = (max_bits + 7) / 8;
  if (passes > 8) passes = 8;
  cudaMemsetAsync(b.ghist, 0, sizeof(unsigned) * LVO_SORT_GHIST_WORDS, st);
  k_sort_ghist<<<max(1, min(lvo_div_up(n_cap, 256 * 16), 592)), 256, 0, st>>>(b.keys[0], d_n, d_bits, b.ghist, b.d_epoch);
  for (int p = 0; p < passes; ++p)
    k_sort_onesweep<<<grid, LVO_SORT_THREADS, 0, st>>>(b.keys[0], b.keys[1], b.vals[0], b.vals[1], d_n, d_bits, p, b.ghist, b.status, b.d_epoch);
  if (launches) *launches += 1 + passes;
}
```

lidar-visual-odometry_b200/csrc/lvo_voxel.cuh:

```cuda
#pragma once
#include "lvo_internal.h"
#include "lvo_prims.cuh"
#include <float.h>
#include <limits.h>

struct VoxelEngine {
  int cap_items, cap_segs;
  float4* in_pts;
  int* in_seg;
  unsigned* in_aux;
  int* d_n;
  float* seg_leaf;
  int* d_nsegs;
  int* seg_mn;
  int* seg_mx;
  int* seg_minb;
  int* seg_div;
  int* seg_mode;
  int* d_vbits;
  int* d_bits;
  LvoSortBufs sort;
  unsigned* outpos;
  float4* out_pts;
  unsigned* out_aux;
  unsigned* seg_out_cnt;
  unsigned* seg_out_start;
  unsigned* d_n_out;
  LvoScanScratch scan;
};

__device__ __forceinline__ int f2ord(float f) { int i = __float_as_int(f); return i >= 0 ? i : i ^ 0x7fffffff; }
__device__ __forceinline__ float ord2f(int i) { return __int_as_float(i >= 0 ? i : i ^ 0x7fffffff); }
__device__ __forceinline__ int bitlen64(unsigned long long v) { return v ? 64 - __clzll((long long)v) : 0; }

__global__ void k_vx_reset(VoxelEngine e) {
  const int nsegs = *e.d_nsegs;
  for (int s = blockIdx.x * blockDim.x + threadIdx.x; s < nsegs; s += gridDim.x * blockDim.x) {
    for (int c = 0; c < 3; ++c) { e.seg_mn[c * e.cap_segs + s] = INT_MAX; e.seg_mx[c * e.cap_segs + s] = INT_MIN; }
    e.seg_out_cnt[s] = 0;
  }
  if (blockIdx.x == 0 && threadIdx.x == 0) { *e.d_vbits = 0; *e.d_n_out = 0; }
}

__global__ void k_vx_bbox(VoxelEngine e) {
  const int n = *e.d_n;
  const int stride = gridDim.x * blockDim.x;
  for (int base = blockIdx.x * blockDim.x; base < n; base += stride) {
    const int i = base + threadIdx.x;
    const bool valid = i < n;
    int seg = -1;
    int mn[3] = {INT_MAX, INT_MAX, INT_MAX}, mx[3] = {INT_MIN, INT_MIN, INT_MIN};
    if (valid) {
      seg = e.in_seg[i];
      const float4 p = e.in_pts[i];
      mn[0] = mx[0] = f2ord(p.x); mn[1] = mx[1] = f2ord(p.y); mn[2] = mx[2] = f2ord(p.z);
    }
    const unsigned m = __match_any_sync(0xffffffffu, seg);
    if (m == 0xffffffffu) {
      if (seg >= 0) {
#pragma unroll
        for (int c = 0; c < 3; ++c) { mn[c] = __reduce_min_sync(0xffffffffu, mn[c]); mx[c] = __reduce_max_sync(0xffffffffu, mx[c]); }
        if ((threadIdx.x & 31) == 0)
          for (int c = 0; c < 3; ++c) { atomicMin(&e.seg_mn[c * e.cap_segs + seg], mn[c]); atomicMax(&e.seg_mx[c * e.cap_segs + seg], mx[c]); }
      }
    } else if (valid) {
      for (int c = 0; c < 3; ++c) { atomicMin(&e.seg_mn[c * e.cap_segs + seg], mn[c]); atomicMax(&e.seg_mx[c * e.cap_segs + seg], mx[c]); }
    }
  }
}

__global__ void k_vx_prepare(VoxelEngine e) {
  const int nsegs = *e.d_nsegs;
  const int n = *e.d_n;
  int vb = 0;
  for (int s = blockIdx.x * blockDim.x + threadIdx.x; s < nsegs; s += gridDim.x * blockDim.x) {
    const float leaf = e.seg_leaf[s];
    int mode = 0, bits = 0;
    if (leaf == 0.f) {
      mode = 2; bits = 13;
    } else if (e.seg_mn[s] != INT_MAX) {
      const float inv = 1.0f / leaf;
      float mn[3], mx[3];
      for (int c = 0; c < 3; ++c) { mn[c] = ord2f(e.seg_mn[c * e.cap_segs + s]); mx[c] = ord2f(e.seg_mx[c * e.cap_segs + s]); }
      const long long dx = (long long)((mx[0] - mn[0]) * inv) + 1, dy = (long long)((mx[1] - mn[1]) * inv) + 1, dz = (long long)((mx[2] - mn[2]) * inv) + 1;
      if (dx * dy * dz > (long long)INT_MAX) {
        mode = 1; bits = bitlen64((unsigned long long)(n > 0 ? n - 1 : 0));
      } else {
        int minb[3], maxb[3];
        for (int c = 0; c < 3; ++c) { minb[c] = (int)floorf(mn[c] * inv); maxb[c] = (int)floorf(mx[c] * inv); e.seg_minb[c * e.cap_segs + s] = minb[c]; }
        const int d0 = maxb[0] - minb[0] + 1, d1 = maxb[1] - minb[1] + 1, d2 = maxb[2] - minb[2] + 1;
        e.seg_div[s] = d0; e.seg_div[e.cap_segs + s] = d1;
        unsigned long long prod = (unsigned long long)d0 * (unsigned long long)d1 * (unsigned long long)d2;
        bits = bitlen64(prod - 1);
        if (bits > 32) bits = 32;
      }
    }
    e.seg_mode[s] = mode;
    vb = max(vb, bits);
  }
  vb = __reduce_max_sync(0xffffffffu, vb);
  if ((threadIdx.x & 31) == 0 && vb > 0) atomicMax(e.d_vbits, vb);
}

__global__ void k_vx_keys(VoxelEngine e) {
  const int n = *e.d_n;
  const int vb = *e.d_vbits;
  if (blockIdx.x == 0 && threadIdx.x == 0) {
    const int nsegs = *e.d_nsegs;
    *e.d_bits = vb + bitlen64((unsigned long long)(nsegs > 0 ? nsegs - 1 : 0));
  }
  for (int i = blockIdx.x * blockDim.x + threadIdx.x; i < n; i += gridDim.x * blockDim.x) {
    const int s = e.in_seg[i];
    const int mode = e.seg_mode[s];
    unsigned idx;
    if (mode == 2) idx = e.in_aux[i];
    else if (mode == 1) idx = (unsigned)i;
    else {
      const float inv = 1.0f / e.seg_leaf[s];
      const float4 p = e.in_pts[i];
      const int ijk0 = (int)(floorf(p.x * inv) - (float)e.seg_minb[s]);
      const int ijk1 = (int)(floorf(p.y * inv) - (float)e.seg_minb[e.cap_segs + s]);
      const int ijk2 = (int)(floorf(p.z * inv) - (float)e.seg_minb[2 * e.cap_segs + s]);
      const int d0 = e.seg_div[s], d1 = e.seg_div[e.cap_segs + s];
      idx = (unsigned)(ijk0 + ijk1 * d0 + ijk2 * d0 * d1);
    }
    e.sort.keys[0][i] = ((unsigned long long)(unsigned)s << vb) | (unsigned long long)idx;
    e.sort.vals[0][i] = (unsigned)i;
  }
}

__global__ void k_vx_heads(VoxelEngine e) {
  const int n = *e.d_n;
  const int vb = *e.d_vbits;
  const int p = lvo_sort_passes(*e.d_bits) & 1;
  const unsigned long long* keys = e.sort.keys[p];
  for (int t = blockIdx.x * blockDim.x + threadIdx.x; t < n; t += gridDim.x * blockDim.x) {
    const unsigned long long k = keys[t];
    bool head = (t == 0) || (k != keys[t - 1]);
    if (!head && e.seg_mode[(int)(k >> vb)] == 2) head = true;
    e.outpos[t] = head ? 1u : 0u;
  }
}

__global__ void k_vx_centroid(VoxelEngine e) {
  const int n = *e.d_n;
  const int vb = *e.d_vbits;
  const int p = lvo_sort_passes(*e.d_bits) & 1;
  const unsigned long long* keys = e.sort.keys[p];
  const unsigned* vals = e.sort.vals[p];
  const unsigned lane = threadIdx.x & 31;
  for (int base = (blockIdx.x * blockDim.x + threadIdx.x) & ~31; base < n; base += gridDim.x * blockDim.x) {
    const int t = base + (int)lane;
    const bool in = t < n;
    const unsigned long long k = in ? keys[t] : 0ull;
    const unsigned v = in ? vals[t] : 0u;
    float4 q = make_float4(0.f, 0.f, 0.f, 0.f);
    if (in) q = e.in_pts[v];
    unsigned long long kprev = __shfl_up_sync(0xffffffffu, k, 1);
    if (lane == 0 && in && t > 0) kprev = keys[t - 1];
    const int seg = (int)(k >> vb);
    const bool pseudo = in && e.seg_mode[seg] == 2;
    const bool head = in && (t == 0 || k != kprev || pseudo);
    const unsigned stops = __ballot_sync(0xffffffffu, head || !in);
    const unsigned above = stops & ~((2u << lane) - 1u);
    const int end = above ? __ffs(above) - 1 : 32;
    const int len = head ? end - (int)lane : 0;
    const int maxlen = __reduce_max_sync(0xffffffffu, len);
    float sx = 0.f + q.x, sy = 0.f + q.y, sz = 0.f + q.z, si = 0.f + q.w;
    for (int d = 1; d < maxlen; ++d) {
      const float nx = __shfl_down_sync(0xffffffffu, q.x, d), ny = __shfl_down_sync(0xffffffffu, q.y, d);
      const float nz = __shfl_down_sync(0xffffffffu, q.z, d), ni = __shfl_down_sync(0xffffffffu, q.w, d);
      if (d < len) { sx += nx; sy += ny; sz += nz; si += ni; }
    }
    if (head) {
      int cnt = len;
      if (end == 32 && !pseudo) {
        int u = base + 32;
        while (u < n && keys[u] == k) {
          const float4 r = e.in_pts[vals[u]];
          sx += r.x; sy += r.y; sz += r.z; si += r.w;
          ++u;
        }
        cnt = u - t;
      }
      const float c = (float)cnt;
      const unsigned o = e.outpos[t];
      e.out_pts[o] = make_float4(sx / c, sy / c, sz / c, si / c);
      e.out_aux[o] = e.in_aux[v];
      const unsigned same = __match_any_sync(__activemask(), seg);
      if (lane == (unsigned)(__ffs(same) - 1)) atomicAdd(&e.seg_out_cnt[seg], (unsigned)__popc(same));
    }
  }
}

__global__ void __launch_bounds__(1024) k_vx_seg_offsets(VoxelEngine e) {
  __shared__ unsigned sm[33];
  const int nsegs = *e.d_nsegs;
  unsigned carry = 0;
  for (int base = 0; base < nsegs; base += blockDim.x) {
    const int s = base + threadIdx.x;
    const unsigned v = s < nsegs ? e.seg_out_cnt[s] : 0u;
    unsigned tot;
    const unsigned ex = block_excl_scan(v, sm, &tot);
    if (s < nsegs) e.seg_out_start[s] = carry + ex;
    carry += tot;
  }
}

static inline void lvo_voxel_run(cudaStream_t st, const VoxelEngine& e, int n_items_cap, int n_segs_cap, int max_seg_bits, long long* launches) {
  const int gi = max(1, min(lvo_div_up(n_items_cap, 256), 1184));
  const int gs = max(1, min(lvo_div_up(n_segs_cap, 256), 148));
  k_vx_reset<<<gs, 256, 0, st>>>(e);
  k_vx_bbox<<<gi, 256, 0, st>>>(e);
  k_vx_prepare<<<gs, 256, 0, st>>>(e);
  k_vx_keys<<<gi, 256, 0, st>>>(e);
  lvo_sort_pairs(st, e.sort, e.d_n, n_items_cap, e.d_bits, 32 + max_seg_bits, launches);
  k_vx_heads<<<gi, 256, 0, st>>>(e);
  lvo_scan_exclusive(st, e.outpos, e.d_n, n_items_cap, e.d_n_out, e.scan, launches);
  k_vx_centroid<<<gi, 256, 0, st>>>(e);
  k_vx_seg_offsets<<<1, 1024, 0, st>>>(e);
  if (launches) *launches += 7;
}
```

Measured before the change: 23640.

## Sort voxel keys per lane-group segment instead of one global radix sort

The voxel engine now partitions items by group (lane/type) using precomputed group offsets. The onesweep radix sort runs per group, with per-group histograms, tiles that never cross a group boundary, and lookback limited to the group's own tiles. The group index moves into high key bits that are never sorted, so fewer radix passes are needed (segment bits become per-group rather than global). The bbox kernel is also reworked to use shared-memory slot reduction. The trade-off is extra tiles at group boundaries, a binary search per tile, and larger histogram buffers.

```diff
diff --git a/lidar-visual-odometry_b200/csrc/lvo_api.cu b/lidar-visual-odometry_b200/csrc/lvo_api.cu
--- a/lidar-visual-odometry_b200/csrc/lvo_api.cu
+++ b/lidar-visual-odometry_b200/csrc/lvo_api.cu
@@ -189,7 +189,7 @@
   prob[0].pts = pts; prob[0].d_n = d_n; prob[0].want_cell = cell; prob[0].want_cell_z = 0.f; prob[0].mode = 0; prob[0].cells_cap = 0; prob[0].clamp_xy = 0.f; prob[0].bbox_from = -1;
 }
 __global__ void k_vx_single_setup(VoxelEngine e, int n, float leaf) {
-  if (blockIdx.x == 0 && threadIdx.x == 0) { *e.d_n = n; *e.d_nsegs = 1; e.seg_leaf[0] = leaf; }
+  if (blockIdx.x == 0 && threadIdx.x == 0) { *e.d_n = n; *e.d_nsegs = 1; e.seg_leaf[0] = leaf; e.grp_off[0] = 0; e.grp_off[1] = (unsigned)n; }
   for (int i = blockIdx.x * blockDim.x + threadIdx.x; i < n; i += gridDim.x * blockDim.x) { e.in_seg[i] = 0; e.in_aux[i] = 0; }
 }
 
@@ -492,7 +492,6 @@
   }
   LVO_TRY(alloc_grid(c, &mp.grid, 2 * L, 1 << 21, (size_t)L * ((size_t)mapc[0] + mapc[1]), std::max(mapc[0], mapc[1])));
   k_setup_grid_problems<<<lvo_div_up(2 * L, 64), 64, 0, c->st>>>(mp.grid.prob, 2 * L, mp.from_map[0], (size_t)mapc[0], mp.from_map[1], (size_t)mapc[1], c->d_ls, 1, 1.0f);
-  LVO_TRY(dalloc(c, &mp.item_off, (size_t)2 * L + 1));
   LVO_TRY(dalloc(c, &mp.fit_list, (size_t)L * (mp.in_cap[0] + mp.in_cap[1]), false));
   LVO_TRY(dalloc(c, &mp.fit_cnt, (size_t)L * LVO_MAX_OUTER));
   mp.factors = od.factors; mp.factor_cap = od.factor_cap;
@@ -502,15 +501,18 @@
   VoxelEngine& vx = mp.vx;
   vx.cap_items = (int)std::min<size_t>((size_t)L * ((size_t)mapc[0] + mapc[1] + c->cap_lsharp + P), (size_t)INT_MAX - 4096);
   vx.cap_segs = 2 * L * LVO_MSEGS;
+  vx.cap_groups = 2 * L;
   const size_t NI = (size_t)vx.cap_items, NS = (size_t)vx.cap_segs;
+  LVO_TRY(dalloc(c, &vx.grp_off, (size_t)vx.cap_groups + 1));
   LVO_TRY(dalloc(c, &vx.in_pts, NI, false)); LVO_TRY(dalloc(c, &vx.in_seg, NI)); LVO_TRY(dalloc(c, &vx.in_aux, NI));
   LVO_TRY(dalloc(c, &vx.d_n, 1)); LVO_TRY(dalloc(c, &vx.seg_leaf, NS)); LVO_TRY(dalloc(c, &vx.d_nsegs, 1));
   LVO_TRY(dalloc(c, &vx.seg_mn, 3 * NS)); LVO_TRY(dalloc(c, &vx.seg_mx, 3 * NS)); LVO_TRY(dalloc(c, &vx.seg_minb, 3 * NS));
   LVO_TRY(dalloc(c, &vx.seg_div, 2 * NS)); LVO_TRY(dalloc(c, &vx.seg_mode, NS)); LVO_TRY(dalloc(c, &vx.d_vbits, 1)); LVO_TRY(dalloc(c, &vx.d_bits, 1));
   for (int k = 0; k < 2; ++k) { LVO_TRY(dalloc(c, &vx.sort.keys[k], NI, false)); LVO_TRY(dalloc(c, &vx.sort.vals[k], NI, false)); }
-  const size_t tiles = (size_t)lvo_div_up((long long)NI, LVO_SORT_TILE) + 1;
-  LVO_TRY(dalloc(c, &vx.sort.ghist, (size_t)LVO_SORT_GHIST_WORDS)); LVO_TRY(dalloc(c, &vx.sort.d_epoch, 1));
+  const size_t tiles = lvo_sort_tiles((long long)NI, vx.cap_groups);
+  LVO_TRY(dalloc(c, &vx.sort.ghist, lvo_sort_ghist_words(vx.cap_groups))); LVO_TRY(dalloc(c, &vx.sort.d_epoch, 1));
   LVO_TRY(dalloc(c, &vx.sort.status, 256 * tiles));
+  LVO_TRY(dalloc(c, &vx.sort.grp_tile, (size_t)vx.cap_groups + 1));
   vx.sort.cap = vx.cap_items;
   LVO_TRY(dalloc(c, &vx.outpos, NI)); LVO_TRY(dalloc(c, &vx.out_pts, NI, false)); LVO_TRY(dalloc(c, &vx.out_aux, NI));
   LVO_TRY(dalloc(c, &vx.seg_out_cnt, NS)); LVO_TRY(dalloc(c, &vx.seg_out_start, NS + 1)); LVO_TRY(dalloc(c, &vx.d_n_out, 1));
@@ -1491,7 +1493,7 @@
   VoxelEngine& vx = c->map.vx;
   LVO_TRY(upload_cloud(c, in, vx.in_pts));
   k_vx_single_setup<<<std::max(1, std::min(lvo_div_up((long long)in.n, 256), 592)), 256, 0, c->st>>>(vx, (int)in.n, leaf);
-  lvo_voxel_run(c->st, vx, (int)std::max<size_t>(in.n, 1), 1, 1, &c->launches);
+  lvo_voxel_run(c->st, vx, (int)std::max<size_t>(in.n, 1), 1, 1, 1, &c->launches);
   unsigned n_out = 0;
   LVO_CUDA_OK(c, cudaMemcpyAsync(&n_out, vx.d_n_out, 4, cudaMemcpyDeviceToHost, c->st));
   LVO_CUDA_OK(c, cudaStreamSynchronize(c->st));
@@ -1511,7 +1513,7 @@
   LVO_CUDA_OK(c, cudaMemcpyAsync(vx.in_pts, d_in, n * sizeof(lvo_point), cudaMemcpyDeviceToDevice, c->st));
   k_vx_single_setup<<<std::max(1, std::min(lvo_div_up((long long)n, 256), 592)), 256, 0, c->st>>>(vx, (int)n, leaf);
   cudaEventRecord(c->ev[6], c->st);
-  lvo_voxel_run(c->st, vx, (int)std::max<size_t>(n, 1), 1, 1, &c->launches);
+  lvo_voxel_run(c->st, vx, (int)std::max<size_t>(n, 1), 1, 1, 1, &c->launches);
   cudaEventRecord(c->ev[7], c->st);
   unsigned cnt = 0;
   LVO_CUDA_OK(c, cudaMemcpyAsync(&cnt, vx.d_n_out, 4, cudaMemcpyDeviceToHost, c->st));
diff --git a/lidar-visual-odometry_b200/csrc/lvo_mapping.cuh b/lidar-visual-odometry_b200/csrc/lvo_mapping.cuh
--- a/lidar-visual-odometry_b200/csrc/lvo_mapping.cuh
+++ b/lidar-visual-odometry_b200/csrc/lvo_mapping.cuh
@@ -23,7 +23,6 @@
   float4* stack[2];
   GridSet grid;
   VoxelEngine vx;
-  unsigned* item_off;
   LvoFactor* factors; int factor_cap;
   unsigned* app_cnt;
   unsigned* app_first;
@@ -117,10 +116,10 @@
     }
     unsigned tot;
     const unsigned ex = block_excl_scan(v, sm, &tot);
-    if (lt < L2) a.item_off[lt] = acc + ex;
+    if (lt < L2) a.vx.grp_off[lt] = acc + ex;
     acc += tot;
   }
-  if (threadIdx.x == 0) { a.item_off[L2] = acc; *a.vx.d_n = (int)acc; *a.vx.d_nsegs = L2; }
+  if (threadIdx.x == 0) { a.vx.grp_off[L2] = acc; *a.vx.d_n = (int)acc; *a.vx.d_nsegs = L2; }
 }
 __global__ void k_stack_gather(MapArgs a) {
   const int lt = blockIdx.y, lane = lt >> 1, t = lt & 1;
@@ -128,7 +127,7 @@
   const int n = t ? s.n_less_flat : s.n_less_sharp;
   if (!lane_maps(a.lane_flags, lane)) return;
   const float4* src = a.in_pts[t] + (size_t)lane * a.in_cap[t];
-  const unsigned off = a.item_off[lt];
+  const unsigned off = a.vx.grp_off[lt];
   for (int i = blockIdx.x * blockDim.x + threadIdx.x; i < n; i += gridDim.x * blockDim.x) {
     a.vx.in_pts[off + i] = src[i];
     a.vx.in_seg[off + i] = lt;
@@ -573,17 +572,17 @@
     if (lt < L2 && lane_updates_map(a.lane_flags, lt >> 1)) { const LaneState& s = a.ls[lt >> 1]; v = (unsigned)(s.from_off[lt & 1][LVO_MAX_VALID] + s.n_stack[lt & 1]); }
     unsigned tot;
     const unsigned ex = block_excl_scan(v, sm, &tot);
-    if (lt < L2) a.item_off[lt] = acc + ex;
+    if (lt < L2) a.vx.grp_off[lt] = acc + ex;
     acc += tot;
   }
-  if (threadIdx.x == 0) { a.item_off[L2] = acc; *a.vx.d_n = (int)acc; *a.vx.d_nsegs = L2 * LVO_MSEGS; }
+  if (threadIdx.x == 0) { a.vx.grp_off[L2] = acc; *a.vx.d_n = (int)acc; *a.vx.d_nsegs = L2 * LVO_MSEGS; }
 }
 __global__ void k_refilter_gather(MapArgs a) {
   const int lt = blockIdx.y, lane = lt >> 1, t = lt & 1;
   const LaneState& s = a.ls[lane];
   const int nfrom = s.from_off[t][LVO_MAX_VALID], nst = s.n_stack[t];
   if (!lane_updates_map(a.lane_flags, lane)) return;
-  const unsigned off = a.item_off[lt];
+  const unsigned off = a.vx.grp_off[lt];
   const float4* FM = a.from_map[t] + (size_t)lane * a.map_cap[t];
   const float4* ST = a.stack[t] + (size_t)lane * a.in_cap[t];
   for (int i = blockIdx.x * blockDim.x + threadIdx.x; i < nfrom + nst; i += gridDim.x * blockDim.x) {
@@ -717,8 +716,7 @@
   k_stack_offsets<<<1, 256, 0, st>>>(a);
   k_stack_gather<<<dim3(16, L2), 256, 0, st>>>(a);
   if (launches) *launches += 4;
-  int seg_bits = 1; while ((1 << seg_bits) < L2) seg_bits++;
-  lvo_voxel_run(st, a.vx, lanes * (a.in_cap[0] + a.in_cap[1]), L2, seg_bits, launches);
+  lvo_voxel_run(st, a.vx, lanes * (a.in_cap[0] + a.in_cap[1]), L2, L2, 1, launches);
   k_stack_scatter<<<dim3(8, L2), 256, 0, st>>>(a);
   if (launches) *launches += 1;
   LVO_MARK(tm, LVO_ST_MAP_TREE, st);
@@ -747,8 +745,7 @@
   k_refilter_gather<<<dim3(64, L2), 256, 0, st>>>(a);
   if (launches) *launches += 3;
   LVO_MARK(tm, LVO_ST_MAP_FILTER, st);
-  int seg_bits2 = 1; while ((1 << seg_bits2) < L2 * LVO_MSEGS) seg_bits2++;
-  lvo_voxel_run(st, a.vx, a.vx.cap_items, L2 * LVO_MSEGS, seg_bits2, launches);
+  lvo_voxel_run(st, a.vx, a.vx.cap_items, L2 * LVO_MSEGS, L2, LVO_MSEGS, launches);
   k_rebuild_reset<<<148, 256, 0, st>>>(a);
   k_rebuild_appended<<<dim3(4, L2), 256, 0, st>>>(a);
   k_rebuild_offsets<<<L2, 256, 0, st>>>(a);
diff --git a/lidar-visual-odometry_b200/csrc/lvo_prims.cuh b/lidar-visual-odometry_b200/csrc/lvo_prims.cuh
--- a/lidar-visual-odometry_b200/csrc/lvo_prims.cuh
+++ b/lidar-visual-odometry_b200/csrc/lvo_prims.cuh
@@ -116,46 +116,75 @@
   if (launches) *launches += 3;
 }
 
+#define LVO_SORT_MAX_PASSES 8
 struct LvoSortBufs {
   unsigned long long* keys[2];
   unsigned* vals[2];
   unsigned* ghist;
   unsigned long long* status;
   unsigned* d_epoch;
+  unsigned* grp_tile;
   int cap;
 };
-#define LVO_SORT_GHIST_WORDS (8 * 256 + 8)
+static inline size_t lvo_sort_tiles(long long n_cap, int groups) { return (size_t)lvo_div_up(n_cap, LVO_SORT_TILE) + (size_t)groups + 1; }
+static inline size_t lvo_sort_ghist_words(int groups) { return (size_t)LVO_SORT_MAX_PASSES + (size_t)groups * LVO_SORT_MAX_PASSES * 256; }
 
 __device__ __forceinline__ int lvo_sort_passes(int bits) { return (bits + 7) >> 3; }
 
-__global__ void __launch_bounds__(256) k_sort_ghist(const unsigned long long* __restrict__ keys, const int* __restrict__ d_n, const int* __restrict__ d_bits,
+__device__ __forceinline__ void lvo_sort_group_tiles(const unsigned* __restrict__ grp_off, int ngroups, unsigned* __restrict__ grp_tile, unsigned* sm33) {
+  unsigned carry = 0;
+  for (int base = 0; base <= ngroups; base += blockDim.x) {
+    const int g = base + threadIdx.x;
+    const unsigned v = g < ngroups ? (grp_off[g + 1] - grp_off[g] + LVO_SORT_TILE - 1) / LVO_SORT_TILE : 0u;
+    unsigned tot;
+    const unsigned ex = block_excl_scan(v, sm33, &tot);
+    if (g <= ngroups) grp_tile[g] = carry + ex;
+    carry += tot;
+  }
+}
+__device__ __forceinline__ int lvo_sort_tile_group(const unsigned* __restrict__ grp_tile, int ngroups, int tile) {
+  int lo = 0, hi = ngroups - 1;
+  while (lo < hi) { const int mid = (lo + hi + 1) >> 1; if ((int)grp_tile[mid] <= tile) lo = mid; else hi = mid - 1; }
+  return lo;
+}
+
+__global__ void __launch_bounds__(256) k_sort_ghist(const unsigned long long* __restrict__ keys, const unsigned* __restrict__ grp_off,
+                                                    const unsigned* __restrict__ grp_tile, int ngroups, int hpasses, const int* __restrict__ d_bits,
                                                     unsigned* __restrict__ ghist, unsigned* __restrict__ d_epoch) {
-  __shared__ unsigned h[8][256];
-  const int passes = min(lvo_sort_passes(*d_bits), 8);
-  const int n = *d_n;
+  __shared__ unsigned h[LVO_SORT_MAX_PASSES][256];
+  __shared__ int s_g;
+  const int passes = min(lvo_sort_passes(*d_bits), hpasses);
+  const int ntiles = (int)grp_tile[ngroups];
   if (blockIdx.x == 0 && threadIdx.x == 0) *d_epoch = *d_epoch + 1u;
-  for (int k = threadIdx.x; k < 8 * 256; k += blockDim.x) (&h[0][0])[k] = 0;
-  __syncthreads();
-  for (int i = blockIdx.x * blockDim.x + threadIdx.x; i < n; i += gridDim.x * blockDim.x) {
-    const unsigned long long key = keys[i];
-    for (int p = 0; p < passes; ++p) atomicAdd(&h[p][(unsigned)(key >> (8 * p)) & 255u], 1u);
-  }
-  __syncthreads();
-  for (int k = threadIdx.x; k < passes * 256; k += blockDim.x) { const unsigned v = (&h[0][0])[k]; if (v) atomicAdd(&ghist[k], v); }
+  if (passes == 0) return;
+  for (int tile = blockIdx.x; tile < ntiles; tile += gridDim.x) {
+    for (int k = threadIdx.x; k < passes * 256; k += blockDim.x) (&h[0][0])[k] = 0;
+    if (threadIdx.x == 0) s_g = lvo_sort_tile_group(grp_tile, ngroups, tile);
+    __syncthreads();
+    const int g = s_g;
+    const unsigned b = grp_off[g] + (unsigned)(tile - (int)grp_tile[g]) * LVO_SORT_TILE, e = min(b + LVO_SORT_TILE, grp_off[g + 1]);
+    for (unsigned i = b + threadIdx.x; i < e; i += blockDim.x) {
+      const unsigned long long key = keys[i];
+      for (int p = 0; p < passes; ++p) atomicAdd(&h[p][(unsigned)(key >> (8 * p)) & 255u], 1u);
+    }
+    __syncthreads();
+    unsigned* gh = ghist + LVO_SORT_MAX_PASSES + (size_t)g * hpasses * 256;
+    for (int k = threadIdx.x; k < passes * 256; k += blockDim.x) { const unsigned v = (&h[0][0])[k]; if (v) atomicAdd(&gh[k], v); }
+    __syncthreads();
+  }
 }
 
 __global__ void __launch_bounds__(LVO_SORT_THREADS, 2)
 k_sort_onesweep(unsigned long long* __restrict__ keys0, unsigned long long* __restrict__ keys1, unsigned* __restrict__ vals0,
-                unsigned* __restrict__ vals1, const int* __restrict__ d_n, const int* __restrict__ d_bits, int pass,
-                unsigned* __restrict__ ghist, unsigned long long* status, const unsigned* __restrict__ d_epoch) {
+                unsigned* __restrict__ vals1, const unsigned* __restrict__ grp_off, const unsigned* __restrict__ grp_tile, int ngroups, int hpasses,
+                const int* __restrict__ d_bits, int pass, unsigned* __restrict__ ghist, unsigned long long* status, const unsigned* __restrict__ d_epoch) {
   __shared__ unsigned wcnt[LVO_SORT_WARPS][256];
   __shared__ unsigned gbase[256];
   __shared__ unsigned sm_scan[33];
-  __shared__ int s_tile;
+  __shared__ int s_tile, s_g;
   const int bits = *d_bits;
   if (pass * 8 >= bits) return;
-  const int n = *d_n;
-  const int ntiles = (n + LVO_SORT_TILE - 1) / LVO_SORT_TILE;
+  const int ntiles = (int)grp_tile[ngroups];
   const unsigned long long* kin = (pass & 1) ? keys1 : keys0;
   unsigned long long* kout = (pass & 1) ? keys0 : keys1;
   const unsigned* vin = (pass & 1) ? vals1 : vals0;
@@ -164,23 +193,31 @@
   const unsigned lane = threadIdx.x & 31, w = threadIdx.x >> 5;
   const unsigned lt = (1u << lane) - 1u;
   const unsigned tag = 2u * (8u * (*d_epoch) + (unsigned)pass);
-  unsigned* ticket = ghist + 8 * 256 + pass;
-  unsigned tot_unused;
-  const unsigned digit_base = block_excl_scan(ghist[pass * 256 + threadIdx.x], sm_scan, &tot_unused);
+  unsigned* ticket = ghist + pass;
   while (true) {
-    if (threadIdx.x == 0) s_tile = (int)atomicAdd(ticket, 1u);
+    if (threadIdx.x == 0) {
+      const int t = (int)atomicAdd(ticket, 1u);
+      s_tile = t;
+      s_g = t < ntiles ? lvo_sort_tile_group(grp_tile, ngroups, t) : 0;
+    }
     for (int k = threadIdx.x; k < LVO_SORT_WARPS * 256; k += LVO_SORT_THREADS) (&wcnt[0][0])[k] = 0;
     __syncthreads();
     const int tile = s_tile;
     if (tile >= ntiles) break;
+    const int g = s_g;
+    const int first = (int)grp_tile[g];
+    const unsigned gb = grp_off[g];
+    const unsigned end = grp_off[g + 1];
+    unsigned tot_unused;
+    const unsigned digit_base = gb + block_excl_scan(ghist[LVO_SORT_MAX_PASSES + ((size_t)g * hpasses + pass) * 256 + threadIdx.x], sm_scan, &tot_unused);
     unsigned long long key[LVO_SORT_ITEMS];
     unsigned val[LVO_SORT_ITEMS];
     unsigned short lpos[LVO_SORT_ITEMS];
-    const int wbase = tile * LVO_SORT_TILE + w * (32 * LVO_SORT_ITEMS);
+    const unsigned wbase = gb + (unsigned)(tile - first) * LVO_SORT_TILE + w * (32 * LVO_SORT_ITEMS);
 #pragma unroll
     for (int r = 0; r < LVO_SORT_ITEMS; ++r) {
-      const int i = wbase + r * 32 + lane;
-      const bool valid = i < n;
+      const unsigned i = wbase + r * 32 + lane;
+      const bool valid = i < end;
       key[r] = valid ? kin[i] : 0ull;
       val[r] = valid ? vin[i] : 0u;
       const unsigned digit = (unsigned)(key[r] >> shift) & 255u;
@@ -205,9 +242,9 @@
       }
       volatile unsigned long long* st = status;
       unsigned excl = 0;
-      if (tile > 0) {
+      if (tile > first) {
         st[(size_t)tile * 256 + d] = ((unsigned long long)tag << 32) | run;
-        for (int t = tile - 1; t >= 0; --t) {
+        for (int t = tile - 1; t >= first; --t) {
           unsigned long long v;
           do { v = st[(size_t)t * 256 + d]; } while (((unsigned)(v >> 32) | 1u) != (tag | 1u));
           excl += (unsigned)v;
@@ -220,8 +257,8 @@
     __syncthreads();
 #pragma unroll
     for (int r = 0; r < LVO_SORT_ITEMS; ++r) {
-      const int i = wbase + r * 32 + lane;
-      if (i < n) {
+      const unsigned i = wbase + r * 32 + lane;
+      if (i < end) {
         const unsigned digit = (unsigned)(key[r] >> shift) & 255u;
         const unsigned pos = gbase[digit] + wcnt[w][digit] + lpos[r];
         kout[pos] = key[r];
@@ -232,15 +269,16 @@
   }
 }
 
-static inline void lvo_sort_pairs(cudaStream_t st, const LvoSortBufs& b, const int* d_n, int n_cap, const int* d_bits, int max_bits,
+static inline void lvo_sort_pairs(cudaStream_t st, const LvoSortBufs& b, const unsigned* grp_off, int ngroups, int n_cap, const int* d_bits, int max_bits,
                                   long long* launches) {
-  int tiles = lvo_div_up(n_cap, LVO_SORT_TILE);
-  int grid = tiles < 592 ? (tiles < 1 ? 1 : tiles) : 592;
+  const int tiles = (int)lvo_sort_tiles(n_cap, ngroups);
+  const int grid = tiles < 592 ? tiles : 592;
   int passes = (max_bits + 7) / 8;
-  if (passes > 8) passes = 8;
-  cudaMemsetAsync(b.ghist, 0, sizeof(unsigned) * LVO_SORT_GHIST_WORDS, st);
-  k_sort_ghist<<<max(1, min(lvo_div_up(n_cap, 256 * 16), 592)), 256, 0, st>>>(b.keys[0], d_n, d_bits, b.ghist, b.d_epoch);
+  if (passes > LVO_SORT_MAX_PASSES) passes = LVO_SORT_MAX_PASSES;
+  cudaMemsetAsync(b.ghist, 0, sizeof(unsigned) * (LVO_SORT_MAX_PASSES + (size_t)ngroups * passes * 256), st);
+  k_sort_ghist<<<grid, 256, 0, st>>>(b.keys[0], grp_off, b.grp_tile, ngroups, passes, d_bits, b.ghist, b.d_epoch);
   for (int p = 0; p < passes; ++p)
-    k_sort_onesweep<<<grid, LVO_SORT_THREADS, 0, st>>>(b.keys[0], b.keys[1], b.vals[0], b.vals[1], d_n, d_bits, p, b.ghist, b.status, b.d_epoch);
+    k_sort_onesweep<<<grid, LVO_SORT_THREADS, 0, st>>>(b.keys[0], b.keys[1], b.vals[0], b.vals[1], grp_off, b.grp_tile, ngroups, passes, d_bits, p, b.ghist,
+                                                       b.status, b.d_epoch);
   if (launches) *launches += 1 + passes;
 }
diff --git a/lidar-visual-odometry_b200/csrc/lvo_voxel.cuh b/lidar-visual-odometry_b200/csrc/lvo_voxel.cuh
--- a/lidar-visual-odometry_b200/csrc/lvo_voxel.cuh
+++ b/lidar-visual-odometry_b200/csrc/lvo_voxel.cuh
@@ -5,11 +5,13 @@
 #include <limits.h>
 
 struct VoxelEngine {
-  int cap_items, cap_segs;
+  int cap_items, cap_segs, cap_groups;
   float4* in_pts;
   int* in_seg;
   unsigned* in_aux;
   int* d_n;
+  unsigned* grp_off;
+  int ngroups, segs_per_group;
   float* seg_leaf;
   int* d_nsegs;
   int* seg_mn;
@@ -34,20 +36,41 @@
 __device__ __forceinline__ int bitlen64(unsigned long long v) { return v ? 64 - __clzll((long long)v) : 0; }
 
 __global__ void k_vx_reset(VoxelEngine e) {
+  __shared__ unsigned sm[33];
   const int nsegs = *e.d_nsegs;
   for (int s = blockIdx.x * blockDim.x + threadIdx.x; s < nsegs; s += gridDim.x * blockDim.x) {
     for (int c = 0; c < 3; ++c) { e.seg_mn[c * e.cap_segs + s] = INT_MAX; e.seg_mx[c * e.cap_segs + s] = INT_MIN; }
     e.seg_out_cnt[s] = 0;
   }
-  if (blockIdx.x == 0 && threadIdx.x == 0) { *e.d_vbits = 0; *e.d_n_out = 0; }
-}
-
-__global__ void k_vx_bbox(VoxelEngine e) {
-  const int n = *e.d_n;
-  const int stride = gridDim.x * blockDim.x;
-  for (int base = blockIdx.x * blockDim.x; base < n; base += stride) {
-    const int i = base + threadIdx.x;
-    const bool valid = i < n;
+  if (blockIdx.x == 0) {
+    if (threadIdx.x == 0) { *e.d_vbits = 0; *e.d_n_out = 0; }
+    lvo_sort_group_tiles(e.grp_off, e.ngroups, e.sort.grp_tile, sm);
+  }
+}
+
+#define LVO_VX_BBOX_SLOTS 256
+__device__ __forceinline__ void vx_bbox_add(const VoxelEngine& e, int (*smn)[LVO_VX_BBOX_SLOTS], int (*smx)[LVO_VX_BBOX_SLOTS], int base, int seg,
+                                            const int* mn, const int* mx) {
+  const int sl = seg - base;
+  if ((unsigned)sl < LVO_VX_BBOX_SLOTS)
+    for (int c = 0; c < 3; ++c) { atomicMin(&smn[c][sl], mn[c]); atomicMax(&smx[c][sl], mx[c]); }
+  else
+    for (int c = 0; c < 3; ++c) { atomicMin(&e.seg_mn[c * e.cap_segs + seg], mn[c]); atomicMax(&e.seg_mx[c * e.cap_segs + seg], mx[c]); }
+}
+__global__ void __launch_bounds__(256) k_vx_bbox(VoxelEngine e) {
+  __shared__ int smn[3][LVO_VX_BBOX_SLOTS], smx[3][LVO_VX_BBOX_SLOTS];
+  __shared__ int s_base;
+  const int n = *e.d_n;
+  const int per = ((n + (int)gridDim.x - 1) / (int)gridDim.x + 255) & ~255;
+  const int b0 = (int)blockIdx.x * per, b1 = min(n, b0 + per);
+  if (b0 >= b1) return;
+  for (int k = threadIdx.x; k < 3 * LVO_VX_BBOX_SLOTS; k += blockDim.x) { (&smn[0][0])[k] = INT_MAX; (&smx[0][0])[k] = INT_MIN; }
+  if (threadIdx.x == 0) { const int s0 = e.in_seg[b0]; s_base = s0 - s0 % e.segs_per_group; }
+  __syncthreads();
+  const int base = s_base;
+  for (int i0 = b0; i0 < b1; i0 += blockDim.x) {
+    const int i = i0 + threadIdx.x;
+    const bool valid = i < b1;
     int seg = -1;
     int mn[3] = {INT_MAX, INT_MAX, INT_MAX}, mx[3] = {INT_MIN, INT_MIN, INT_MIN};
     if (valid) {
@@ -60,12 +83,17 @@
       if (seg >= 0) {
 #pragma unroll
         for (int c = 0; c < 3; ++c) { mn[c] = __reduce_min_sync(0xffffffffu, mn[c]); mx[c] = __reduce_max_sync(0xffffffffu, mx[c]); }
-        if ((threadIdx.x & 31) == 0)
-          for (int c = 0; c < 3; ++c) { atomicMin(&e.seg_mn[c * e.cap_segs + seg], mn[c]); atomicMax(&e.seg_mx[c * e.cap_segs + seg], mx[c]); }
+        if ((threadIdx.x & 31) == 0) vx_bbox_add(e, smn, smx, base, seg, mn, mx);
       }
     } else if (valid) {
-      for (int c = 0; c < 3; ++c) { atomicMin(&e.seg_mn[c * e.cap_segs + seg], mn[c]); atomicMax(&e.seg_mx[c * e.cap_segs + seg], mx[c]); }
-    }
+      vx_bbox_add(e, smn, smx, base, seg, mn, mx);
+    }
+  }
+  __syncthreads();
+  for (int sl = threadIdx.x; sl < LVO_VX_BBOX_SLOTS; sl += blockDim.x) {
+    if (smn[0][sl] == INT_MAX) continue;
+    const int seg = base + sl;
+    for (int c = 0; c < 3; ++c) { atomicMin(&e.seg_mn[c * e.cap_segs + seg], smn[c][sl]); atomicMax(&e.seg_mx[c * e.cap_segs + seg], smx[c][sl]); }
   }
 }
 
@@ -102,13 +130,14 @@
   if ((threadIdx.x & 31) == 0 && vb > 0) atomicMax(e.d_vbits, vb);
 }
 
+#define LVO_VX_GROUP_SHIFT 40
+__device__ __forceinline__ int vx_key_seg(const VoxelEngine& e, unsigned long long k, int vb) {
+  return (int)(k >> LVO_VX_GROUP_SHIFT) * e.segs_per_group + (int)((k & ((1ull << LVO_VX_GROUP_SHIFT) - 1ull)) >> vb);
+}
 __global__ void k_vx_keys(VoxelEngine e) {
   const int n = *e.d_n;
   const int vb = *e.d_vbits;
-  if (blockIdx.x == 0 && threadIdx.x == 0) {
-    const int nsegs = *e.d_nsegs;
-    *e.d_bits = vb + bitlen64((unsigned long long)(nsegs > 0 ? nsegs - 1 : 0));
-  }
+  if (blockIdx.x == 0 && threadIdx.x == 0) *e.d_bits = vb + bitlen64((unsigned long long)(e.segs_per_group - 1));
   for (int i = blockIdx.x * blockDim.x + threadIdx.x; i < n; i += gridDim.x * blockDim.x) {
     const int s = e.in_seg[i];
     const int mode = e.seg_mode[s];
@@ -124,7 +153,8 @@
       const int d0 = e.seg_div[s], d1 = e.seg_div[e.cap_segs + s];
       idx = (unsigned)(ijk0 + ijk1 * d0 + ijk2 * d0 * d1);
     }
-    e.sort.keys[0][i] = ((unsigned long long)(unsigned)s << vb) | (unsigned long long)idx;
+    e.sort.keys[0][i] = ((unsigned long long)(unsigned)(s / e.segs_per_group) << LVO_VX_GROUP_SHIFT) |
+                        ((unsigned long long)(unsigned)(s % e.segs_per_group) << vb) | (unsigned long long)idx;
     e.sort.vals[0][i] = (unsigned)i;
   }
 }
@@ -137,7 +167,7 @@
   for (int t = blockIdx.x * blockDim.x + threadIdx.x; t < n; t += gridDim.x * blockDim.x) {
     const unsigned long long k = keys[t];
     bool head = (t == 0) || (k != keys[t - 1]);
-    if (!head && e.seg_mode[(int)(k >> vb)] == 2) head = true;
+    if (!head && e.seg_mode[vx_key_seg(e, k, vb)] == 2) head = true;
     e.outpos[t] = head ? 1u : 0u;
   }
 }
@@ -158,7 +188,7 @@
     if (in) q = e.in_pts[v];
     unsigned long long kprev = __shfl_up_sync(0xffffffffu, k, 1);
     if (lane == 0 && in && t > 0) kprev = keys[t - 1];
-    const int seg = (int)(k >> vb);
+    const int seg = vx_key_seg(e, k, vb);
     const bool pseudo = in && e.seg_mode[seg] == 2;
     const bool head = in && (t == 0 || k != kprev || pseudo);
     const unsigned stops = __ballot_sync(0xffffffffu, head || !in);
@@ -207,14 +237,17 @@
   }
 }
 
-static inline void lvo_voxel_run(cudaStream_t st, const VoxelEngine& e, int n_items_cap, int n_segs_cap, int max_seg_bits, long long* launches) {
+static inline void lvo_voxel_run(cudaStream_t st, const VoxelEngine& eng, int n_items_cap, int n_segs_cap, int ngroups, int segs_per_group, long long* launches) {
+  VoxelEngine e = eng;
+  e.ngroups = ngroups; e.segs_per_group = segs_per_group;
+  int seg_bits = 0; while ((1 << seg_bits) < segs_per_group) seg_bits++;
   const int gi = max(1, min(lvo_div_up(n_items_cap, 256), 1184));
   const int gs = max(1, min(lvo_div_up(n_segs_cap, 256), 148));
   k_vx_reset<<<gs, 256, 0, st>>>(e);
   k_vx_bbox<<<gi, 256, 0, st>>>(e);
   k_vx_prepare<<<gs, 256, 0, st>>>(e);
   k_vx_keys<<<gi, 256, 0, st>>>(e);
-  lvo_sort_pairs(st, e.sort, e.d_n, n_items_cap, e.d_bits, 32 + max_seg_bits, launches);
+  lvo_sort_pairs(st, e.sort, e.grp_off, ngroups, n_items_cap, e.d_bits, 32 + seg_bits, launches);
   k_vx_heads<<<gi, 256, 0, st>>>(e);
   lvo_scan_exclusive(st, e.outpos, e.d_n, n_items_cap, e.d_n_out, e.scan, launches);
   k_vx_centroid<<<gi, 256, 0, st>>>(e);
diff --git a/profiles/voxel_engine.py b/profiles/voxel_engine.py
--- /dev/null
+++ b/profiles/voxel_engine.py
@@ -0,0 +1,110 @@
+import argparse
+import json
+import os
+import statistics
+import subprocess
+import sys
+
+HERE = os.path.dirname(os.path.abspath(__file__))
+sys.path.insert(0, HERE)
+from lane_lifecycle import ROOT, gpu_identity, load_pkg
+
+ENGINE = ("k_vx_", "k_sort_", "k_scan")
+
+
+def bench_line(lib):
+    env = dict(os.environ)
+    if lib:
+        env["LVO_LIB_PATH"] = lib
+    else:
+        env.pop("LVO_LIB_PATH", None)
+    r = subprocess.run([sys.executable, os.path.join(ROOT, "bench.py")], cwd=ROOT, env=env, capture_output=True, text=True, check=True)
+    d = json.loads(r.stdout.strip().splitlines()[-1])
+    st = d.get("single_trajectory") or {}
+    return {"value": d["value"], "e2e": d["e2e"]["value"], "full_schedule": (d.get("full_schedule") or {}).get("value"),
+            "single_trajectory": {k: v for k, v in st.items() if k != "what"}, "gpu_launches": d.get("gpu_launches"),
+            "stage_ms_per_frame_batched": d["roofline"].get("stage_ms_per_frame_batched"),
+            "config3_voxel_downsample": d["other_configs"].get("config3_voxel_downsample")}
+
+
+def kernel_table(frames):
+    import torch
+    from concurrent.futures import ThreadPoolExecutor
+    from torch.profiler import ProfilerActivity, profile
+    from oracle_py import Synth
+    L = load_pkg()
+    lanes, per_seq = 128, 8
+    plan = [(l // per_seq, l % per_seq) for l in range(lanes)]
+    synth = Synth()
+    jobs = sorted({(s, f + k) for s, f in plan for k in range(frames + 1)})
+    dev = {}
+    with ThreadPoolExecutor(max_workers=os.cpu_count() or 1) as ex:
+        for j, h in zip(jobs, ex.map(lambda j: synth.sweep(64, j[0], j[1])[0], jobs)):
+            dev[j] = torch.from_numpy(h).cuda()
+    torch.cuda.synchronize()
+    ctx = L.Lvo(lanes=lanes, max_points=131072, max_map_corner=1 << 18, max_map_surf=1 << 19, debug_probes=0)
+    ctx.set_option(L.LVO_OPT_GRAPHS, 0)
+    step = lambda k: ctx.step_batch_dev([dev[(s, f + k)].data_ptr() for s, f in plan], [dev[(s, f + k)].shape[0] for s, f in plan])
+    for k in range(frames):
+        step(k)
+    torch.cuda.synchronize()
+    with profile(activities=[ProfilerActivity.CUDA]) as prof:
+        step(frames)
+        torch.cuda.synchronize()
+    launches = int(ctx.timings().kernel_launches)
+    ctx.close()
+    table = {}
+    for e in prof.key_averages():
+        if e.device_type.name == "CUDA" or getattr(e, "self_device_time_total", 0) > 0:
+            us = float(getattr(e, "self_device_time_total", getattr(e, "self_cuda_time_total", 0.0)))
+            if us > 0:
+                table[e.key] = [int(e.count), us]
+    print(json.dumps({"kernel_launches": launches, "kernels": table}))
+
+
+def main():
+    ap = argparse.ArgumentParser()
+    ap.add_argument("--base", help="liblvo.so of the build to compare against")
+    ap.add_argument("--runs", type=int, default=3)
+    ap.add_argument("--frames", type=int, default=100)
+    ap.add_argument("--out", default=None)
+    ap.add_argument("--kernel-table", action="store_true", help=argparse.SUPPRESS)
+    args = ap.parse_args()
+    if args.kernel_table:
+        kernel_table(args.frames)
+        return
+    import torch
+    out = {"config": {"runs_per_build": args.runs, "bench": "python bench.py (defaults)", "kernel_table_frames_before": args.frames}}
+    out.update(gpu_identity(torch))
+    builds = {"base": os.path.abspath(args.base), "this": None}
+    out["bench"] = {b: [] for b in builds}
+    for i in range(args.runs):
+        for b, lib in builds.items():
+            r = bench_line(lib)
+            out["bench"][b].append(r)
+            print(b, json.dumps({k: r[k] for k in ("value", "e2e", "full_schedule", "gpu_launches")}), flush=True)
+    out["bench_value_median"] = {b: statistics.median(x["value"] for x in out["bench"][b]) for b in builds}
+    out["kernel_table"] = {}
+    for b, lib in builds.items():
+        env = dict(os.environ)
+        if lib:
+            env["LVO_LIB_PATH"] = lib
+        else:
+            env.pop("LVO_LIB_PATH", None)
+        r = subprocess.run([sys.executable, os.path.abspath(__file__), "--kernel-table", "--frames", str(args.frames)], cwd=ROOT, env=env,
+                           capture_output=True, text=True, check=True)
+        t = json.loads(r.stdout.strip().splitlines()[-1])
+        eng = {k: v for k, v in t["kernels"].items() if k.startswith(ENGINE) or "Memset" in k}
+        t["engine_us"] = sum(v[1] for v in eng.values())
+        t["engine_launches"] = sum(v[0] for v in eng.values())
+        out["kernel_table"][b] = t
+        print(b, "engine kernels us / frame", round(t["engine_us"], 1), "launches / frame", t["kernel_launches"], flush=True)
+    s = json.dumps(out, indent=1)
+    if args.out:
+        with open(args.out, "w") as f:
+            f.write(s)
+    print(s)
+
+
+if __name__ == "__main__":
+    main()
```

After: 24240 (median of 6 runs). +2.5%, better.
